# DataArcTech/RAG-ARC

Measured on AMD Instinct MI355X. Metric: queries/sec at fixed (N_corpus, d), exact top-k (ids bit-exact vs CPU oracle), higher is better.
Workload: dtype f16; 1 GPU; 100000000x768 fp16 corpus of N(0,1) directions resident in HBM, row-sharded over 1 GPU(s), batch 256 queries, cosine top-100, exact (canonical fp32 rescore); n_corpus=100000000, d=768, batch=256, k=100, rows_per_gpu=100000000, exchange=none (one shard), repaired_queries_last_step=0

## Files before the change

### include/rarc.h

```cpp
#ifndef RARC_H
#define RARC_H

#include <stddef.h>
#include <stdint.h>

#ifdef __cplusplus
extern "C" {
#endif

#define RARC_VERSION 600

#define RARC_OK 0
#define RARC_E_INVALID -1
#define RARC_E_HIP -2
#define RARC_E_WORKSPACE -3
#define RARC_E_UNSUPPORTED -4
#define RARC_E_IO -5

#define RARC_MAX_QUERIES 256
#define RARC_MAX_K 1024
#define RARC_DIM_ALIGN 128

#define RARC_Q_OK 0u
#define RARC_Q_UNCERTAIN 1u
#define RARC_Q_OVERFLOW 2u
#define RARC_Q_WHY_SEGMENT 0x100u
#define RARC_Q_WHY_G1 0x200u
#define RARC_Q_WHY_G2 0x400u
#define RARC_Q_WHY_BAND_TIES 0x800u
#define RARC_Q_WHY_BAND_GUARD 0x1000u

int rarc_version(void);
const char* rarc_last_error(void);

int rarc_padded_dim(int d);

int rarc_l2norm_rows_f32(const float* d_in, int64_t ld_in, float* d_out, int64_t ld_out,
                         int64_t n_rows, int d, void* stream);

int rarc_cosine_matrix_f32(const float* d_x, int64_t ld_x, int nx, const float* d_y, int64_t ld_y, int ny, int d,
                           double* d_out, void* stream);
int rarc_adjacent_cosine_distance_f32(const float* d_x, int64_t ld_x, int n_rows, int d, double* d_out, void* stream);

int rarc_ingest_f16(const float* d_in, int64_t ld_in, uint16_t* d_corpus_f16, int d_pad,
                    float* d_row_norm2, int64_t n_rows, int d, int normalize, void* stream);

size_t rarc_quant_meta_floats(int64_t n_rows);
int rarc_quant_meta_f16(const uint16_t* d_corpus_f16, int64_t n_rows, int d_pad, int64_t first_row,
                        float* d_qmeta, void* stream);

int rarc_debug_q8_scores(const uint16_t* d_corpus_f16, int64_t n_rows, int d_pad, const float* d_qmeta,
                         const void* d_qblock, int nq, float* d_out, void* stream);
int rarc_debug_q8_scores_f8(const uint8_t* d_corpus_f8, int64_t n_rows, int d_pad, const float* d_qmeta,
                            const void* d_qblock, int nq, float* d_out, void* stream);

size_t rarc_query_block_bytes(int d_pad);
int rarc_prep_queries(const float* d_in, int64_t ld_in, int nq, int d, int d_pad, int normalize,
                      float corpus_max_norm, const float* d_qmeta, void* d_qblock, void* stream);

int rarc_qblock_set_floor(void* d_qblock, int d_pad, const int64_t* d_prev_ids, const float* d_prev_scores, int k,
                          int nq, void* stream);

#define RARC_WS_ANYFLAG_OFFSET 5124
size_t rarc_search_workspace_bytes(int cand_cap);

int rarc_search_f16(const uint16_t* d_corpus_f16, int64_t n_rows, int d_pad, const float* d_qmeta,
                    const void* d_qblock, int nq, int k, int kprime, int64_t id_base, float bin_lo,
                    float bin_hi, int64_t* d_out_ids, float* d_out_scores, uint32_t* d_status,
                    void* d_workspace, size_t workspace_bytes, int cand_cap, void* stream);

int rarc_repair_f16(const uint16_t* d_corpus_f16, int64_t n_rows, int d_pad, const void* d_qblock,
                    int q, int k, int64_t id_base, int64_t* d_out_ids, float* d_out_scores,
                    uint32_t* d_found, void* d_workspace, size_t workspace_bytes, void* stream);

int rarc_verify_batch(const void* d_rows, const float* d_row_scale, int row_format, int64_t n_rows, int d_pad,
                      const void* d_qblock, int q_first, int nq, int k, int64_t id_base, const int64_t* d_ids,
                      const float* d_scores, uint32_t* d_counts, void* stream);

int rarc_quant_shadow_f16(const uint16_t* d_corpus_f16, int64_t n_rows, int d_pad, int64_t first_row,
                          float* d_qmeta, int8_t* d_shadow8, void* stream);
int rarc_search_f16_shadow(const uint16_t* d_corpus_f16, const int8_t* d_shadow8, int64_t n_rows, int d_pad,
                           const float* d_qmeta, const void* d_qblock, int nq, int k, int kprime,
                           int64_t id_base, float bin_lo, float bin_hi, int64_t* d_out_ids,
                           float* d_out_scores, uint32_t* d_status, void* d_workspace, size_t workspace_bytes,
                           int cand_cap, void* stream);

int rarc_padded_dim_f8(int d);
int rarc_ingest_f8(const float* d_in, int64_t ld_in, uint8_t* d_corpus_f8, int d_pad, float* d_row_scale,
                   float* d_row_norm2, int64_t n_rows, int d, int normalize, void* stream);
size_t rarc_quant_meta_floats_f8(int64_t n_rows);
int rarc_quant_meta_f8(const uint8_t* d_corpus_f8, const float* d_row_scale, int64_t n_rows, int d_pad,
                       int64_t first_row, float* d_qmeta, void* stream);
int rarc_search_f8(const uint8_t* d_corpus_f8, const float* d_row_scale, int64_t n_rows, int d_pad,
                   const float* d_qmeta, const void* d_qblock, int nq, int k, int kprime, int64_t id_base,
                   float bin_lo, float bin_hi, int64_t* d_out_ids, float* d_out_scores, uint32_t* d_status,
                   void* d_workspace, size_t workspace_bytes, int cand_cap, void* stream);
int rarc_repair_f8(const uint8_t* d_corpus_f8, const float* d_row_scale, int64_t n_rows, int d_pad,
                   const void* d_qblock, int q, int k, int64_t id_base, int64_t* d_out_ids, float* d_out_scores,
                   uint32_t* d_found, void* d_workspace, size_t workspace_bytes, void* stream);

int rarc_ingest_f32(const float* d_in, int64_t ld_in, float* d_corpus_f32, uint16_t* d_image_f16, int d_pad,
                    float* d_row_norm2, int64_t n_rows, int d, int normalize, void* stream);
int rarc_search_f32(const float* d_corpus_f32, const uint16_t* d_image_f16, int64_t n_rows, int d_pad,
                    const float* d_qmeta, const void* d_qblock, int nq, int k, int kprime, int64_t id_base,
                    float bin_lo, float bin_hi, int64_t* d_out_ids, float* d_out_scores, uint32_t* d_status,
                    void* d_workspace, size_t workspace_bytes, int cand_cap, void* stream);
typedef struct RarcSearchBatch {
  const void* d_rows; const void* d_aux; int row_format; int64_t n_rows; int d_pad; const float* d_qmeta;
  const float* d_queries; int64_t ld_queries; int nq; int d; int normalize; float corpus_max_norm; void* d_qblock;
  int k, kprime; int64_t id_base; float bin_lo, bin_hi;
  int64_t* d_out_ids; float* d_out_scores; uint32_t* d_status; uint32_t* flag_host;
  void* d_workspace; size_t workspace_bytes; int cand_cap;
  void* gate_event;
} RarcSearchBatch;
int rarc_search_batch(const RarcSearchBatch* batch, void* stream);

int rarc_stream_read(const void* d_src, size_t n_bytes, void* d_sink, void* stream);

size_t rarc_bm25_workspace_bytes(int nq, int64_t n_query_tokens, int64_t n_docs, int k);
int rarc_bm25_topk(const int64_t* d_post_off, const int32_t* d_post_doc, const double* d_post_w, int64_t n_terms,
                   int64_t n_docs, const int32_t* d_q_off, const int32_t* d_q_term, const double* d_q_idf, int nq,
                   int64_t n_query_tokens, int k, void* d_workspace, size_t workspace_bytes, int64_t* d_out_ids,
                   double* d_out_scores, void* stream);
int rarc_bm25_scores(const int64_t* d_post_off, const int32_t* d_post_doc, const double* d_post_w, int64_t n_terms,
                     int64_t n_docs, const int32_t* d_q_off, const int32_t* d_q_term, const double* d_q_idf, int nq,
                     int64_t n_query_tokens, void* d_workspace, size_t workspace_bytes, double* d_out_scores,
                     void* stream);

int rarc_repair_f32(const float* d_corpus_f32, int64_t n_rows, int d_pad, const void* d_qblock, int q, int k,
                    int64_t id_base, int64_t* d_out_ids, float* d_out_scores, uint32_t* d_found, void* d_workspace,
                    size_t workspace_bytes, void* stream);

int rarc_topk_merge(const int64_t* d_ids, const float* d_scores, int n_lists, int nq, int k,
                    int64_t* d_out_ids, float* d_out_scores, void* stream);
int rarc_pack_results(const int64_t* d_ids, const float* d_scores, int nq, int k, int32_t* d_packed, void* stream);
int rarc_topk_merge_packed(const int32_t* d_packed, int n_lists, int nq, int k, int64_t* d_out_ids,
                           float* d_out_scores, void* stream);

int rarc_rrf_fuse(const int64_t* d_keys, const int32_t* d_len, int nq, int n_lists, int max_len,
                  double rrf_k, int top_k, int64_t* d_out_keys, double* d_out_scores,
                  int32_t* d_out_n, void* stream);

int rarc_rerank_order(const uint16_t* d_z_no, const uint16_t* d_z_yes, int nq, int n,
                      uint16_t* d_out_scores_f16, int32_t* d_out_perm, void* stream);

size_t rarc_mmr_workspace_doubles(int n, int d);
int rarc_mmr_select(const float* d_cand, int64_t ld, const double* d_query, int n, int d, int normalize, int k,
                    double lambda, double* d_work, int32_t* d_out, void* stream);

size_t rarc_mmr_rows_workspace_bytes(int nq, int n, int d);
int rarc_mmr_select_rows(const void* d_rows, int fmt, const float* d_rowscale, int64_t n_rows, int d_pad, int d,
                         const double* d_queries, int64_t ldq, int nq, const int64_t* d_cand_ids, int n, int64_t id_base,
                         int normalize, int k, double lambda, int64_t* d_out_ids, void* d_ws, size_t ws_bytes, void* stream);

int rarc_synth_rows_f16(uint16_t* d_out_f16, int d_pad, int d, int64_t first_row, int64_t n_rows,
                        uint64_t seed, void* stream);
int rarc_synth_rows_f32(float* d_out_f32, int64_t ld_out, int d, int64_t first_row,
                        int64_t n_rows, uint64_t seed, void* stream);

int rarc_enc_embed_ln(const int32_t* d_ids, const uint16_t* d_word, const uint16_t* d_pos,
                      const uint16_t* d_type0, const uint16_t* d_gamma, const uint16_t* d_beta, float eps,
                      int n_tokens, int seq_len, int hidden, int vocab, uint16_t* d_out, void* stream);
int rarc_enc_gemm(const uint16_t* d_a, const uint16_t* d_w, const uint16_t* d_bias, uint16_t* d_c, int m,
                  int n, int k, int act, void* stream);
int rarc_enc_gemm_zero_bias(const uint16_t* d_a, const uint16_t* d_w, const uint16_t* d_zero_bias, uint16_t* d_c, int m,
                            int n, int k, int act, void* stream);
int rarc_enc_attention(const uint16_t* d_qkv, const int32_t* d_lens, int n_seq, int seq_len, int hidden,
                       int n_heads, uint16_t* d_ctx, void* stream);
int rarc_enc_add_ln(const uint16_t* d_x, const uint16_t* d_resid, const uint16_t* d_gamma,
                    const uint16_t* d_beta, float eps, int n_rows, int hidden, uint16_t* d_out, void* stream);
int rarc_enc_pool(const uint16_t* d_hidden, int n_seq, int seq_len, int hidden, int normalize,
                  float* d_out, void* stream);
int rarc_enc_pool_mean(const uint16_t* d_hidden, const int32_t* d_lens, int n_seq, int seq_len, int hidden,
                       int normalize, float* d_out, void* stream);

typedef struct RarcEncLayer {
  const uint16_t *qkv_w, *qkv_b;
  const uint16_t *o_w, *o_b, *ln1_g, *ln1_b;
  const uint16_t *f1_w, *f1_b, *f2_w, *f2_b, *ln2_g, *ln2_b;
} RarcEncLayer;
typedef struct RarcEncModel {
  int hidden, heads, inter, n_layers;
  float ln_eps;
  const uint16_t *word, *pos, *type0, *emb_g, *emb_b;
  const RarcEncLayer* layers;
  int vocab;
  int max_pos;
  const float* rel_bias;
  int rel_span;
} RarcEncModel;
size_t rarc_enc_workspace_bytes(int hidden, int inter, int n_tokens);
int rarc_enc_forward(const RarcEncModel* model, const int32_t* d_ids, const int32_t* d_lens, int n_seq,
                     int seq_len, int normalize, void* d_ws, size_t ws_bytes, float* d_out, void* stream);

typedef struct RarcEnc32Layer {
  const uint16_t* qkv_w3; const float *qkv_rw, *qkv_b;
  const uint16_t* o_w3;   const float *o_rw, *o_b, *ln1_g, *ln1_b;
  const uint16_t* f1_w3;  const float *f1_rw, *f1_b;
  const uint16_t* f2_w3;  const float *f2_rw, *f2_b, *ln2_g, *ln2_b;
  const float* f1_colmax;
  const uint16_t *qkv_wq, *o_wq, *f1_wq, *f2_wq;
} RarcEnc32Layer;
typedef struct RarcEnc32Model {
  int hidden, heads, inter, n_layers;
  float ln_eps;
  const float *word, *pos, *type0, *emb_g, *emb_b;
  const RarcEnc32Layer* layers;
  int vocab, max_pos;
  const float* rel_bias;
  int rel_span;
} RarcEnc32Model;
int rarc_enc32_split_weight(const float* d_w, int n, int k, uint16_t* d_w3, float* d_rw, void* stream);
int rarc_enc32_pack_query_weight(const uint16_t* d_w3, int n, int k, uint16_t* d_wq, void* stream);
int rarc_enc32_split_rows(const float* d_x, int m, int k, uint16_t* d_a3, float* d_ra, void* stream);
int rarc_enc32_gemm(const uint16_t* d_a3, const float* d_ra, const uint16_t* d_w3, const float* d_rw,
                    const float* d_bias, float* d_c, int m, int n, int k, void* stream);
size_t rarc_enc32_workspace_bytes(int hidden, int inter, int n_tokens);
int rarc_enc32_forward(const RarcEnc32Model* model, const int32_t* d_ids, const int32_t* d_lens, int n_seq,
                       int seq_len, int normalize, void* d_ws, size_t ws_bytes, float* d_out, void* stream);

typedef struct RarcLmLayer {
  const uint16_t *in_norm, *qkv_w, *q_norm, *k_norm, *o_w, *post_norm, *gate_up_w, *down_w;
  const uint16_t *qkv_w_folded, *gate_up_w_folded;
} RarcLmLayer;
typedef struct RarcLmModel {
  int hidden, n_layers, n_q_heads, n_kv_heads, head_dim, inter, vocab;
  float rms_eps, rope_theta;
  const uint16_t *embed, *lm_head, *final_norm, *zero_bias;
  const RarcLmLayer* layers;
} RarcLmModel;
size_t rarc_lm_workspace_bytes(const RarcLmModel* model, int n_tokens);
int rarc_lm_yes_no_logits(const RarcLmModel* model, const int32_t* d_ids, const int32_t* d_start, int n_seq,
                          int seq_len, int no_id, int yes_id, void* d_ws, size_t ws_bytes, uint16_t* d_out_f16,
                          void* stream);

size_t rarc_lm_prefix_cache_bytes(const RarcLmModel* model, int n_prefix_tokens);
int rarc_lm_prefix_kv(const RarcLmModel* model, const int32_t* d_ids, const int32_t* d_start, int n_prefix, int prefix_len,
                      void* d_ws, size_t ws_bytes, void* d_cache, size_t cache_bytes, void* stream);
int rarc_lm_yes_no_logits_prefixed(const RarcLmModel* model, const int32_t* d_ids, const int32_t* d_start, int n_seq,
                                   int seq_len, const int32_t* d_prefix_of, const void* d_cache, int n_prefix,
                                   int prefix_len, const int32_t* d_prefix_start, int no_id, int yes_id, void* d_ws,
                                   size_t ws_bytes, uint16_t* d_out_f16, void* stream);

int rarc_lm_embed_last(const RarcLmModel* model, const int32_t* d_ids, const int32_t* d_start, int n_seq, int seq_len,
                       int out_dim, int normalize, void* d_ws, size_t ws_bytes, float* d_out, int64_t ld_out, void* stream);
int rarc_lm_embed_last_prefixed(const RarcLmModel* model, const int32_t* d_ids, const int32_t* d_start, int n_seq,
                                int seq_len, const int32_t* d_prefix_of, const void* d_cache, int n_prefix,
                                int prefix_len, const int32_t* d_prefix_start, int out_dim, int normalize, void* d_ws,
                                size_t ws_bytes, float* d_out, int64_t ld_out, void* stream);

int rarc_lm_rope_table(int n_rows, int head_dim, float theta, uint16_t* d_table, void* stream);
int rarc_lm_rmsnorm(uint16_t* d_x, const uint16_t* d_delta, const uint16_t* d_w, float eps, int n_rows, int hidden, uint16_t* d_y,
                    void* stream);
int rarc_lm_rowscale_parts(const float* d_ssq, int n_parts, float eps, int n_rows, int hidden, float* d_r, void* stream);
int rarc_lm_swiglu(const uint16_t* d_gate_up, int n_rows, int inter, uint16_t* d_out, void* stream);
int rarc_lm_attention(const uint16_t* d_qkv, const int32_t* d_start, int n_seq, int seq_len, int n_q, int n_kv, int head_dim,
                      const uint16_t* d_q_norm, const uint16_t* d_k_norm, float eps, const uint16_t* d_rope, int rope_rows,
                      const uint16_t* d_prefix_kv, const int32_t* d_prefix_of, const int32_t* d_prefix_start, int n_prefix,
                      int prefix_len, int kernel, uint16_t* d_ctx, void* stream);
int rarc_lm_last_logits(const uint16_t* d_x, const uint16_t* d_final_norm, const uint16_t* d_lm_head, float eps, int n_seq,
                        int row_stride, int row_off, int hidden, int vocab, int no_id, int yes_id, uint16_t* d_out, void* stream);
int rarc_lm_last_embed(const uint16_t* d_x, const uint16_t* d_final_norm, float eps, int n_seq, int row_stride, int row_off,
                       int hidden, int out_dim, int normalize, float* d_out, int64_t ld_out, void* stream);
int rarc_lm_gather_last(const uint16_t* d_src, int seq_len, int width, int n_seq, int n_rows, uint16_t* d_dst, void* stream);

typedef struct RarcWordPiece RarcWordPiece;
int rarc_wordpiece_create(const char* vocab_blob, size_t blob_bytes, int do_lower_case, const char* unk_token,
                          const char* cls_token, const char* sep_token, const char* pad_token, const char* never_split_blob,
                          size_t never_split_bytes, int max_input_chars_per_word, RarcWordPiece** out);
void rarc_wordpiece_destroy(RarcWordPiece* wp);
int rarc_wordpiece_encode(const RarcWordPiece* wp, const char* text_blob, const int64_t* text_offsets, int n_texts,
                          int max_length, int32_t* h_ids, int64_t ld_ids, int32_t* h_lens, int n_threads);

#define RARC_IO_DIRECT 1
#define RARC_IO_FSYNC 2
#define RARC_IO_TRUNCATE 4
typedef struct RarcIoStats {
  int64_t bytes;
  double seconds;
  double file_seconds;
  double copy_wait_seconds;
  int64_t direct_bytes;
  int64_t n_chunks, slot_bytes;
  int n_threads, direct;
} RarcIoStats;
int rarc_file_to_device(const char* path, int n_seg, const int64_t* h_file_off, const int64_t* h_bytes,
                        const int64_t* h_dev_off, void* d_base, int64_t d_capacity_bytes, void* h_staging,
                        size_t staging_bytes, int n_threads, int flags, void* stream, RarcIoStats* stats);
int rarc_device_to_file(const char* path, int n_seg, const int64_t* h_file_off, const int64_t* h_bytes,
                        const int64_t* h_dev_off, const void* d_base, int64_t d_capacity_bytes, void* h_staging,
                        size_t staging_bytes, int n_threads, int flags, void* stream, RarcIoStats* stats);

size_t rarc_wide_workspace_bytes(int d_pad, int cand_cap);
int rarc_search_wide(const void* d_rows, const uint16_t* d_image16, int fmt, int64_t n_rows, int d_pad, float max_norm,
                     float rho, const void* d_qblock, int nq, int k, int64_t id_base, int64_t* d_out_ids,
                     float* d_out_scores, uint32_t* d_status, void* d_ws, size_t ws_bytes, int cand_cap, void* stream);

int rarc_row_sqnorms(const void* d_rows, int fmt, int64_t n_rows, int d_pad, int64_t first_row, float* d_xn, void* stream);
int rarc_search_wide_l2(const void* d_rows, const uint16_t* d_image16, int fmt, int64_t n_rows, int d_pad, float max_norm,
                        float rho, const float* d_xn, const void* d_qblock, int nq, int k, int64_t id_base, int64_t* d_out_ids,
                        float* d_out_scores, uint32_t* d_status, void* d_ws, size_t ws_bytes, int cand_cap, void* stream);
int rarc_debug_wide_bounds(const void* d_ws, size_t ws_bytes, int d_pad, int cand_cap, float* d_out, void* stream);
int rarc_debug_query_scale8(float mx, float* sq, float* qi);
int rarc_debug_q8_tail_plan(uint32_t t_begin, uint32_t n_tiles, uint32_t grid, int d_pad, int fmt, int pct, int min_mib,
                            uint32_t* t_dyn, uint32_t* r0, uint32_t* unit);
int rarc_debug_q8_tail_chunks(uint32_t k_first, uint32_t n, uint32_t stride, uint32_t unit, uint32_t t_dyn, uint32_t r0,
                              uint32_t n_tiles, uint32_t* t0, uint32_t* t_end);
int64_t rarc_debug_q8_tail_counter_offset(int launch);

size_t rarc_search_rows_workspace_bytes(int nq, int k);
int rarc_search_rows(const void* d_rows, int fmt, int64_t n_rows, int d_pad, const void* d_qblock, int nq, const int64_t* d_list,
                     int64_t m, int k, int64_t id_base, const float* d_xn, int l2, int64_t* d_out_ids, float* d_out_scores,
                     uint32_t* d_status, void* d_ws, size_t ws_bytes, void* stream);
int rarc_strike_rows(const int64_t* d_ids, const float* d_scores, int nq, int kprime, const uint32_t* d_bits, int64_t n_rows,
                     int64_t id_base, int k, int l2, int64_t* d_out_ids, float* d_out_scores, uint32_t* d_count, void* stream);

size_t rarc_search_rows_grouped_workspace_bytes(int nq, int k);
int rarc_search_rows_grouped(const void* d_rows, int fmt, int64_t n_rows, int d_pad, const void* d_qblock, int nq,
                             const int64_t* d_lists, const int64_t* d_tiles, int n_tiles, int64_t m_max, int k, int64_t id_base,
                             const float* d_xn, int l2, int64_t* d_out_ids, float* d_out_scores, uint32_t* d_status, void* d_ws,
                             size_t ws_bytes, void* stream);
int rarc_strike_rows_grouped(const int64_t* d_ids, const float* d_scores, int nq, int kprime, const uint32_t* d_bits,
                             const int64_t* d_bits_off, int64_t n_rows, int64_t id_base, int k, int l2, int64_t* d_out_ids,
                             float* d_out_scores, uint32_t* d_count, void* stream);

size_t rarc_similar_pairs_workspace_bytes(int64_t n_rows, int d, int cand_cap);
int rarc_similar_pairs(const float* d_rows, int64_t ld, int64_t n_rows, int d, double threshold, void* d_ws, size_t ws_bytes,
                       int cand_cap, int64_t* d_out_pairs, double* d_out_scores, int64_t out_cap,
                       unsigned long long* d_out_count, uint32_t* d_flags, void* stream);

size_t rarc_knn_graph_workspace_bytes(int64_t n_rows, int d, int top_k, int cand_cap);
int rarc_knn_graph(const float* d_rows, int64_t ld, int64_t n_rows, int d, int top_k, double cutoff, void* d_ws, size_t ws_bytes,
                   int cand_cap, int64_t* d_out_ids, double* d_out_scores, int32_t* d_out_count, uint32_t* d_flags, void* stream);

size_t rarc_graph_csr_workspace_bytes(int64_t n, int64_t m);
int rarc_graph_csr(const int64_t* d_pairs, const uint32_t* d_weights, const uint32_t* d_loops, int64_t n, int64_t m, void* d_graph,
                   size_t graph_bytes, void* stream);
size_t rarc_louvain_workspace_bytes(int64_t n, int64_t m);
int rarc_louvain_init(const void* d_graph, size_t graph_bytes, int64_t n, int64_t m, void* d_state, size_t state_bytes, int64_t* d_out3,
                      void* stream);
int rarc_louvain_sweep(const void* d_graph, size_t graph_bytes, int64_t n, int64_t m, void* d_state, size_t state_bytes, int cur, int sweep,
                       int64_t* d_out3, void* stream);
int rarc_louvain_aggregate(const void* d_graph, size_t graph_bytes, int64_t n, int64_t m, void* d_state, size_t state_bytes, int cur,
                           int64_t* d_labels, int64_t n0, int64_t* d_out_pairs, uint32_t* d_out_weights, uint32_t* d_out_loops,
                           int64_t* d_out_counts, void* stream);
size_t rarc_louvain_labels_workspace_bytes(int64_t n0);
int rarc_louvain_labels(int64_t* d_labels, int64_t n0, void* d_ws, size_t ws_bytes, void* stream);
int rarc_louvain_limits(int* out4);

size_t rarc_ppr_workspace_bytes(int64_t n, int64_t m, int nq);
int rarc_ppr_seed(const void* d_graph, size_t graph_bytes, int64_t n, int64_t m, const int64_t* d_seeds, const uint32_t* d_seed_weights,
                  int nq, int n_slots, void* d_ws, size_t ws_bytes, void* stream);
int rarc_ppr_step(const void* d_graph, size_t graph_bytes, int64_t n, int64_t m, int nq, int damping_q16, int64_t tolerance, int cur,
                  void* d_ws, size_t ws_bytes, uint32_t* d_done_out, void* stream);
int rarc_ppr_scores(int64_t n, int64_t m, int nq, const void* d_ws, size_t ws_bytes, double* d_out_scores, void* stream);
int rarc_ppr_topk(int64_t n, int64_t m, int nq, int top_k, int cur, void* d_ws, size_t ws_bytes, int64_t* d_out_ids,
                  double* d_out_scores, int32_t* d_out_count, void* stream);
int rarc_ppr_limits(int* out6);

size_t rarc_ppr_chunks_workspace_bytes(int64_t n_chunks, int nq);
int rarc_ppr_chunks(int64_t n, int64_t m, int nq, int cur, const void* d_ws, size_t ws_bytes, const int64_t* d_row_ptr,
                    const int32_t* d_ent, const uint32_t* d_w, int64_t n_chunks, int64_t nnz, const int32_t* d_split, int64_t n_split,
                    void* d_cws, size_t cws_bytes, void* stream);
int rarc_ppr_chunks_scores(int64_t n_chunks, int nq, const void* d_cws, size_t cws_bytes, double* d_out_scores, void* stream);
int rarc_ppr_chunks_topk(int64_t n_chunks, int nq, int top_k, void* d_cws, size_t cws_bytes, int64_t* d_out_ids, double* d_out_scores,
                         int32_t* d_out_count, void* stream);
int rarc_ppr_chunks_limits(int* out4);

size_t rarc_khop_workspace_bytes(int64_t n, int64_t m, int nq, int hops);
int rarc_khop_seed(int64_t n, int64_t m, const int64_t* d_seeds, int nq, int n_slots, int hops, void* d_ws, size_t ws_bytes, void* stream);
int rarc_khop_step(const void* d_graph, size_t graph_bytes, int64_t n, int64_t m, int nq, int hops, int hop, void* d_ws, size_t ws_bytes,
                   uint32_t* d_grew_out, void* stream);
int rarc_khop_counts(int64_t n, int64_t m, int nq, int hops, void* d_ws, size_t ws_bytes, int32_t* d_out_counts, void* stream);
int rarc_khop_levels(int64_t n, int64_t m, int nq, int hops, const void* d_ws, size_t ws_bytes, uint8_t* d_out_levels, void* stream);
int rarc_khop_list(int64_t n, int64_t m, int nq, int hops, int max_vertices, void* d_ws, size_t ws_bytes, int64_t* d_out_ids,
                   int32_t* d_out_hops, int32_t* d_out_count, void* stream);
int rarc_khop_chunks(int64_t n, int64_t m, int nq, int hops, const uint32_t* decay, const void* d_ws, size_t ws_bytes,
                     const int64_t* d_row_ptr, const int32_t* d_ent, const uint32_t* d_w, int64_t n_chunks, int64_t nnz,
                     const int32_t* d_split, int64_t n_split, void* d_cws, size_t cws_bytes, void* stream);
int rarc_khop_limits(int* out5);

size_t rarc_khop_edges_workspace_bytes(int64_t r, int nq, int hops);
int rarc_khop_edges(int64_t n, int64_t m, int nq, int hops, const void* d_ws, size_t ws_bytes, const int64_t* d_rel, int64_t r, int max_edges,
                    void* d_ews, size_t ews_bytes, int64_t* d_out_ids, int32_t* d_out_levels, int32_t* d_out_count,
                    int32_t* d_out_level_counts, void* stream);
int rarc_khop_edges_limits(int* out2);

int rarc_khop_paths(int64_t n, int64_t m, int ns, int np, int max_length, const void* d_ws, size_t ws_bytes, const int32_t* d_pairs,
                    void* d_pws, size_t pws_bytes, int32_t* d_out_dist, void* stream);
int rarc_khop_path_edges(int64_t n, int64_t m, int nq, int hops, const void* d_ws, size_t ws_bytes, const int64_t* d_rel, int64_t r,
                         int max_edges, void* d_ews, size_t ews_bytes, int64_t* d_out_ids, int32_t* d_out_levels, int32_t* d_out_count,
                         int32_t* d_out_level_counts, void* stream);
int rarc_khop_paths_limits(int* out3);

size_t rarc_graph_types_workspace_bytes(int64_t n, int64_t m);
int rarc_graph_types(const void* d_graph, size_t graph_bytes, int64_t n, int64_t m, const int64_t* d_pairs, const uint32_t* d_masks,
                     void* d_out, size_t out_bytes, void* stream);
int rarc_khop_step_typed(const void* d_graph, size_t graph_bytes, const void* d_types, size_t types_bytes, const uint32_t* d_filters,
                         int64_t n, int64_t m, int nq, int hops, int hop, void* d_ws, size_t ws_bytes, uint32_t* d_grew_out, void* stream);
int rarc_khop_edges_typed(int64_t n, int64_t m, int nq, int hops, const void* d_ws, size_t ws_bytes, const int64_t* d_rel, int64_t r,
                          const int32_t* d_rel_types, int rel_masks, const uint32_t* d_filters, int max_edges, void* d_ews, size_t ews_bytes,
                          int64_t* d_out_ids, int32_t* d_out_levels, int32_t* d_out_count, int32_t* d_out_level_counts, void* stream);
int rarc_khop_path_edges_typed(int64_t n, int64_t m, int nq, int hops, const void* d_ws, size_t ws_bytes, const int64_t* d_rel, int64_t r,
                               const int32_t* d_rel_types, int rel_masks, const uint32_t* d_filters, int max_edges, void* d_ews,
                               size_t ews_bytes, int64_t* d_out_ids, int32_t* d_out_levels, int32_t* d_out_count,
                               int32_t* d_out_level_counts, void* stream);

size_t rarc_graph_types_weighted_workspace_bytes(int64_t n, int64_t m);
int rarc_graph_types_weighted(const void* d_graph, size_t graph_bytes, int64_t n, int64_t m, const int64_t* d_pairs, const uint32_t* d_masks,
                              const uint32_t* d_weights, void* d_out, size_t out_bytes, void* stream);
int rarc_ppr_seed_typed(const void* d_graph, size_t graph_bytes, const void* d_types, size_t types_bytes, const uint32_t* d_filters, int64_t n,
                        int64_t m, const int64_t* d_seeds, const uint32_t* d_seed_weights, int nq, int n_slots, void* d_ws, size_t ws_bytes,
                        void* stream);
int rarc_ppr_step_typed(const void* d_graph, size_t graph_bytes, const void* d_types, size_t types_bytes, const uint32_t* d_filters, int64_t n,
                        int64_t m, int nq, int damping_q16, int64_t tolerance, int cur, void* d_ws, size_t ws_bytes, uint32_t* d_done_out,
                        void* stream);

size_t rarc_sort_reduce_workspace_bytes(int64_t count);
int rarc_sort_reduce(const uint64_t* d_keys, const uint32_t* d_values, int64_t count, int key_bits, void* d_ws, size_t ws_bytes,
                     uint64_t* d_out_keys, uint64_t* d_out_sums, int64_t* d_out2, void* stream);
int rarc_sort_reduce_limits(int* out4);
size_t rarc_merge_plan_workspace_bytes(int64_t n);
int rarc_merge_plan(const int64_t* d_labels, const uint32_t* d_richness, int64_t n, void* d_ws, size_t ws_bytes, int64_t* d_primary,
                    int64_t* d_new_id, int64_t* d_kept, int64_t* d_removed, int64_t* d_out_count, void* stream);
size_t rarc_merge_pairs_workspace_bytes(int64_t m);
int rarc_merge_pairs(const int64_t* d_pairs, const uint32_t* d_weights, int64_t m, const int64_t* d_new_id, int64_t n, void* d_ws,
                     size_t ws_bytes, int64_t* d_out_pairs, uint32_t* d_out_weights, int64_t* d_out5, void* stream);
size_t rarc_merge_mentions_workspace_bytes(int64_t n_chunks, int64_t nnz);
int rarc_merge_mentions(const int64_t* d_row_ptr, const int32_t* d_ent, const uint32_t* d_w, int64_t n_chunks, int64_t nnz,
                        const int64_t* d_new_id, int64_t n, void* d_ws, size_t ws_bytes, int64_t* d_out_row_ptr, int32_t* d_out_ent,
                        uint32_t* d_out_w, int32_t* d_out_split, int64_t* d_out6, void* stream);
size_t rarc_merge_relations_workspace_bytes(int64_t r);
int rarc_merge_relations(const int64_t* d_rel, int64_t r, const int64_t* d_new_id, int64_t n, void* d_ws, size_t ws_bytes,
                         int64_t* d_out_rel, int64_t* d_out_rows, int64_t* d_out3, void* stream);

size_t rarc_ingest_pairs_workspace_bytes(int64_t m0, int64_t r);
int rarc_ingest_pairs(const int64_t* d_rows, const uint32_t* d_row_weights, const int32_t* d_row_types, int64_t r,
                      const int64_t* d_base_pairs, const uint32_t* d_base_weights, const uint32_t* d_base_masks, int64_t m0, int64_t n,
                      void* d_ws, size_t ws_bytes, int64_t* d_out_pairs, uint32_t* d_out_weights, uint32_t* d_out_masks, int64_t* d_out8,
                      void* stream);
size_t rarc_ingest_mentions_workspace_bytes(int64_t n_chunks, int64_t nnz0, int64_t r);
int rarc_ingest_mentions(const int64_t* d_rows, const uint32_t* d_row_weights, int64_t r, const int64_t* d_base_row_ptr,
                         const int32_t* d_base_ent, const uint32_t* d_base_w, int64_t base_chunks, int64_t nnz0, int64_t n_chunks,
                         int64_t n_entities, void* d_ws, size_t ws_bytes, int64_t* d_out_row_ptr, int32_t* d_out_ent, uint32_t* d_out_w,
                         int32_t* d_out_split, int64_t* d_out8, void* stream);
int rarc_ingest_limits(int* out4);

size_t rarc_components_workspace_bytes(int64_t n, int64_t m);
int rarc_components_init(int64_t n, int64_t m, void* d_ws, size_t ws_bytes, void* stream);
int rarc_components_round(const void* d_graph, size_t graph_bytes, int64_t n, int64_t m, void* d_ws, size_t ws_bytes, int32_t* d_changed,
                          void* stream);
int rarc_components_finish(int64_t n, int64_t m, void* d_ws, size_t ws_bytes, int64_t* d_labels, int32_t* d_dense, int64_t* d_sizes,
                           int64_t* d_out3, void* stream);
int rarc_components_limits(int* out4);

size_t rarc_cooccur_workspace_bytes(int64_t n_chunks, int64_t nnz);
int rarc_cooccur_count(const int64_t* d_row_ptr, const int32_t* d_ent, const uint32_t* d_w, int64_t n_chunks, int64_t nnz, int64_t n,
                       int max_mentions, void* d_ws, size_t ws_bytes, int64_t* d_out4, void* stream);
int rarc_cooccur_emit(const int64_t* d_row_ptr, const int32_t* d_ent, const uint32_t* d_w, int64_t n_chunks, int64_t nnz, int64_t n,
                      int mode, const void* d_ws, size_t ws_bytes, uint64_t* d_keys, uint32_t* d_values, int64_t total, void* stream);
size_t rarc_cooccur_edges_workspace_bytes(int64_t distinct);
int rarc_cooccur_edges(const uint64_t* d_keys, const uint64_t* d_sums, int64_t distinct, int64_t n, int64_t min_weight, void* d_ws,
                       size_t ws_bytes, int64_t* d_out_pairs, uint32_t* d_out_weights, int64_t* d_out3, void* stream);
int rarc_cooccur_limits(int* out4);

int rarc_compact_rows(void* d_rows, int64_t row_bytes, int64_t n_rows, const int64_t* d_adj, int64_t n_holes,
                      int64_t first_hole, void* d_tmp, size_t tmp_bytes, void* stream);

#define RARC_VMEM_DEFAULT_SLAB (16u << 20)
typedef struct RarcVmem RarcVmem;
int rarc_vmem_create(int device, size_t reserve_bytes, size_t min_reserve_bytes, size_t slab_bytes, RarcVmem** out);
int rarc_vmem_grow(RarcVmem* arena, size_t min_bytes);
void* rarc_vmem_base(const RarcVmem* arena);
size_t rarc_vmem_mapped(const RarcVmem* arena);
size_t rarc_vmem_reserved(const RarcVmem* arena);
size_t rarc_vmem_slab(const RarcVmem* arena);
size_t rarc_vmem_granularity(const RarcVmem* arena);
int rarc_vmem_destroy(RarcVmem* arena);

int rarc_profile_begin(int max_launches);
int rarc_profile_end(double* total_scan_ms, int* n_launches);

#ifdef __cplusplus
}
#endif
#endif
```

### rag-arc_amd/csrc/finalize.hip

```cpp
#include "rarc_common.h"
#include <type_traits>

constexpr int FIN_THREADS = 256;

__device__ __forceinline__ float canon_dot_f16(const float* __restrict__ q,
                                               const half_t* __restrict__ row, int d) {
  float a[8] = {0.f, 0.f, 0.f, 0.f, 0.f, 0.f, 0.f, 0.f};
#pragma unroll 16
  for (int m = 0; m < d; m += 8) {
    const half8 x = *(const half8*)(row + m);
    const float4 q0 = *(const float4*)(q + m);
    const float4 q1 = *(const float4*)(q + m + 4);
    a[0] = __builtin_fmaf(q0.x, (float)x[0], a[0]);
    a[1] = __builtin_fmaf(q0.y, (float)x[1], a[1]);
    a[2] = __builtin_fmaf(q0.z, (float)x[2], a[2]);
    a[3] = __builtin_fmaf(q0.w, (float)x[3], a[3]);
    a[4] = __builtin_fmaf(q1.x, (float)x[4], a[4]);
    a[5] = __builtin_fmaf(q1.y, (float)x[5], a[5]);
    a[6] = __builtin_fmaf(q1.z, (float)x[6], a[6]);
    a[7] = __builtin_fmaf(q1.w, (float)x[7], a[7]);
  }
  return rarc_canon_tree(a);
}

__device__ __forceinline__ float canon_dot_f32(const float* __restrict__ q, const float* __restrict__ row, int d) {
  float a[8] = {0.f, 0.f, 0.f, 0.f, 0.f, 0.f, 0.f, 0.f};
#pragma unroll 8
  for (int m = 0; m < d; m += 8) {
    const float4 x0 = *(const float4*)(row + m), x1 = *(const float4*)(row + m + 4);
    const float4 q0 = *(const float4*)(q + m), q1 = *(const float4*)(q + m + 4);
    a[0] = __builtin_fmaf(q0.x, x0.x, a[0]);
    a[1] = __builtin_fmaf(q0.y, x0.y, a[1]);
    a[2] = __builtin_fmaf(q0.z, x0.z, a[2]);
    a[3] = __builtin_fmaf(q0.w, x0.w, a[3]);
    a[4] = __builtin_fmaf(q1.x, x1.x, a[4]);
    a[5] = __builtin_fmaf(q1.y, x1.y, a[5]);
    a[6] = __builtin_fmaf(q1.z, x1.z, a[6]);
    a[7] = __builtin_fmaf(q1.w, x1.w, a[7]);
  }
  return rarc_canon_tree(a);
}

__device__ __forceinline__ void bitonic_desc(uint64_t* a, int n) {
  for (int k = 2; k <= n; k <<= 1) {
    for (int j = k >> 1; j > 0; j >>= 1) {
      for (int i = threadIdx.x; i < n; i += blockDim.x) {
        const int ixj = i ^ j;
        if (ixj > i) {
          const uint64_t x = a[i], y = a[ixj];
          const bool up = ((i & k) == 0);
          if (up ? (x < y) : (x > y)) {
            a[i] = y;
            a[ixj] = x;
          }
        }
      }
      __syncthreads();
    }
  }
}

struct FinParams {
  const half_t* corpus;
  const float* q32;
  const float* eps;
  const uint32_t* cnt2;
  const uint64_t* cand;
  const uint32_t* hist;
  const float* binlo;
  const float* bininv;
  uint32_t* flags;
  uint32_t seg;
  uint32_t n_wg;
  int d;
  int k, kprime;
  int64_t id_base;
  int64_t* out_ids;
  float* out_scores;
  uint32_t* status;
  uint32_t* flag_host;
};

constexpr int FIN_SURV = 4096;

__global__ __launch_bounds__(FIN_THREADS) void rarc_finalize_kernel(const FinParams p) {
  __shared__ uint64_t keys[FIN_SURV];
  __shared__ uint64_t sel[RARC_MAX_K];
  __shared__ uint64_t fin[RARC_MAX_K];
  __shared__ uint32_t s_hist[RARC_NB];
  __shared__ __attribute__((aligned(16))) float s_q[768];
  __shared__ float s_thr;
  __shared__ uint32_t s_ns, s_total, s_over, s_maxn;
  const int q = blockIdx.x, tid = threadIdx.x;

  for (int i = tid; i < RARC_NB; i += blockDim.x) s_hist[i] = p.hist[(size_t)q * RARC_NB + i];
  for (int i = tid; i < p.d; i += blockDim.x) s_q[i] = p.q32[(size_t)q * p.d + i];
  if (tid == 0) { s_ns = 0; s_total = 0; s_over = 0; s_maxn = 0; }
  __syncthreads();
  if (tid < 64) {
    uint32_t above;
    const int b = rarc_wave_find_from_top(s_hist, RARC_NB, (uint32_t)p.kprime, &above);
    if (tid == 0) s_thr = rarc_bin_threshold(b, p.binlo[q], p.bininv[q]);
  }
  __syncthreads();
  const float thr = s_thr;

  {
    uint32_t n = 0;
    const uint64_t* src = p.cand;
    if ((uint32_t)tid < p.n_wg) {
      const uint32_t c = p.cnt2[(size_t)tid * RARC_MAX_QUERIES + q];
      n = c < p.seg ? c : p.seg;
      if (c > p.seg) atomicOr(&s_over, 1u);
      atomicAdd(&s_total, c);
      src = p.cand + ((size_t)q * RARC_MAX_WG + tid) * p.seg;
    }
    uint64_t first[16];
#pragma unroll
    for (int i = 0; i < 8; ++i) {
      const ulonglong2 v = ((const ulonglong2*)src)[i];
      first[2 * i] = v.x;
      first[2 * i + 1] = v.y;
    }
#pragma unroll
    for (uint32_t i = 0; i < 16; ++i) {
      if (i < n && rarc_candscore(first[i]) >= thr) {
        const uint32_t pos = atomicAdd(&s_ns, 1u);
        if (pos < FIN_SURV) keys[pos] = first[i];
      }
    }
    for (uint32_t i = 16; i < n; ++i) {
      const uint64_t key = src[i];
      if (rarc_candscore(key) >= thr) {
        const uint32_t pos = atomicAdd(&s_ns, 1u);
        if (pos < FIN_SURV) keys[pos] = key;
      }
    }
  }
  __syncthreads();
  const uint32_t ns_all = s_ns, total = s_total;
  const int ns = ns_all < FIN_SURV ? (int)ns_all : FIN_SURV;

  const int kp = ns < p.kprime ? ns : p.kprime;
  for (int i = tid; i < ns; i += blockDim.x) {
    const uint64_t mine = keys[i];
    int rank = 0;
    for (int j = 0; j < ns; ++j) rank += (keys[j] > mine);
    if (rank < kp) sel[rank] = mine;
  }
  __syncthreads();

  const float* qv = s_q;
  for (int i = tid; i < kp; i += blockDim.x) {
    const uint32_t row = rarc_candrow(sel[i]);
    fin[i] = rarc_candkey(canon_dot_f16(qv, p.corpus + (size_t)row * p.d, p.d), row);
  }
  __syncthreads();
  for (int i = tid; i < p.k; i += blockDim.x) {
    if (i >= kp) {
      p.out_ids[(size_t)q * p.k + i] = -1;
      p.out_scores[(size_t)q * p.k + i] = -INFINITY;
    }
  }
  __shared__ float s_sk;
  for (int i = tid; i < kp; i += blockDim.x) {
    const uint64_t mine = fin[i];
    int rank = 0;
    for (int j = 0; j < kp; ++j) rank += (fin[j] > mine);
    if (rank < p.k) {
      p.out_ids[(size_t)q * p.k + rank] = p.id_base + (int64_t)rarc_candrow(mine);
      p.out_scores[(size_t)q * p.k + rank] = rarc_candscore(mine);
    }
    if (rank == (p.k < kp ? p.k : kp) - 1) s_sk = rarc_candscore(mine);
  }
  __syncthreads();

  if (tid == 0) {
    uint32_t st = RARC_Q_OK;
    if (s_over || ns_all > (uint32_t)FIN_SURV) st |= RARC_Q_OVERFLOW;
    if (total >= (uint32_t)p.kprime && kp >= 1) {
      const float tmin = rarc_candscore(sel[kp - 1]);
      if (!(tmin + p.eps[q] < s_sk)) st |= RARC_Q_UNCERTAIN;
    }
    p.status[q] = st;
    if (st) {
      atomicOr(&p.flags[1], st);
      atomicOr(&p.status[RARC_MAX_QUERIES], st);
      if (p.flag_host) __hip_atomic_store(p.flag_host, 1u, __ATOMIC_RELAXED, __HIP_MEMORY_SCOPE_SYSTEM);
    }
  }
}

int rarc_finalize_launch(const uint16_t* corpus, int d_pad, const float* q32, const float* eps, int nq,
                         int k, int kprime, int64_t id_base, const RarcWs& ws, int cap, int n_wg,
                         int64_t* out_ids, float* out_scores, uint32_t* status, hipStream_t s) {
  FinParams p;
  p.corpus = (const half_t*)corpus;
  p.q32 = q32;
  p.eps = eps;
  p.cnt2 = ws.cnt2;
  p.cand = ws.cand;
  p.hist = ws.hist;
  p.binlo = ws.binlo;
  p.bininv = ws.bininv;
  p.flags = ws.flags;
  p.seg = (uint32_t)(cap / RARC_MAX_WG);
  p.n_wg = (uint32_t)n_wg;
  p.d = d_pad;
  p.k = k;
  p.kprime = kprime;
  p.id_base = id_base;
  p.out_ids = out_ids;
  p.out_scores = out_scores;
  p.status = status;
  p.flag_host = rarc_launch_extras().flag_host;
  hipLaunchKernelGGL(rarc_finalize_kernel, dim3(nq), dim3(FIN_THREADS), 0, s, p);
  RARC_HIP_CHECK(hipGetLastError());
  return RARC_OK;
}

constexpr int FIN8_THREADS = 512;
constexpr int FIN8_RS = 6144;
constexpr int FIN8_MAXD = 1024;
#ifndef FIN8_COLLECT_U
#define FIN8_COLLECT_U 8
#endif

struct Fin8Params {
  const void* corpus;
  const float* rowscale;
  int fmt;
  const float* q32;
  const float* eps8;
  const uint32_t* cnt2;
  const uint64_t* cand;
  const uint32_t* hist;
  const float* binlo;
  const float* bininv;
  uint32_t* flags;
  uint32_t seg;
  uint32_t n_wg;
  int d;
  int k;
  int64_t id_base;
  int64_t* out_ids;
  float* out_scores;
  uint32_t* status;
  const float* tmeta;
  int mstride;
  const float* hq;
  unsigned long long* dbg;
  uint32_t* tighten_thr;
  int tighten_mode;
  const float* eps16;
  uint32_t* flag_host;
};

__global__ __launch_bounds__(FIN8_THREADS) void rarc_finalize_q8_kernel(const Fin8Params p) {
  extern __shared__ __attribute__((aligned(16))) char fsm[];
  __shared__ uint64_t ex[FIN8_RS];
  __shared__ __attribute__((aligned(16))) float s_q[FIN8_MAXD];
  __shared__ uint32_t s_hist[RARC_NB];
  __shared__ uint32_t s_cnt[RARC_MAX_WG];
  __shared__ float s_t1, s_L;
  __shared__ uint32_t s_ne, s_over, s_cmp;
  __shared__ int s_selb;
  __shared__ uint32_t s_selabove;
  const int q = blockIdx.x, tid = threadIdx.x;
  const float eps = p.eps8[q];
#define FIN8_STAMP(i) if (p.dbg && q == 0 && tid == 0) p.dbg[i] = __builtin_amdgcn_s_memrealtime();
  FIN8_STAMP(0)

  for (int i = tid; i < RARC_NB; i += blockDim.x) s_hist[i] = p.hist[(size_t)q * RARC_NB + i];
  for (int i = tid; i < p.d; i += blockDim.x) s_q[i] = p.q32[(size_t)q * p.d + i];
  if (tid == 0) { s_ne = 0; s_over = 0; s_L = -INFINITY; }
  __syncthreads();
  for (int i = tid; i < RARC_MAX_WG; i += blockDim.x) {
    const uint32_t c = (uint32_t)i < p.n_wg ? p.cnt2[(size_t)i * RARC_MAX_QUERIES + q] : 0u;
    s_cnt[i] = c;
    if (c > p.seg) atomicOr(&s_over, 1u);
  }
  if (tid < 64) {
    uint32_t above;
    const int b = rarc_wave_find_from_top(s_hist, RARC_NB, (uint32_t)p.k, &above);
    if (tid == 0) s_t1 = rarc_bin_threshold(b, p.binlo[q], p.bininv[q]);
  }
  __syncthreads();
  float t1 = s_t1;

  auto collect = [&](auto want) {
    constexpr int U = FIN8_COLLECT_U;
    const int lane = tid & 63, wv = tid >> 6, nwv = blockDim.x >> 6;
    for (uint32_t wg0 = wv * U; wg0 < p.n_wg; wg0 += nwv * U) {
      uint32_t n[U];
      uint32_t nmax = 0;
#pragma unroll
      for (int u = 0; u < U; ++u) {
        const uint32_t wg = wg0 + u;
        const uint32_t c = wg < p.n_wg ? s_cnt[wg] : 0u;
        n[u] = c < p.seg ? c : p.seg;
        nmax = n[u] > nmax ? n[u] : nmax;
      }
      for (uint32_t base = 0; base < nmax; base += 64) {
        uint64_t key[U];
#pragma unroll
        for (int u = 0; u < U; ++u) {
          const uint32_t i = base + lane;
          key[u] = i < n[u] ? p.cand[((size_t)q * RARC_MAX_WG + wg0 + u) * p.seg + i] : 0ull;
        }
#pragma unroll
        for (int u = 0; u < U; ++u) {
          if (base + lane < n[u] && want(rarc_candscore(key[u]), rarc_candrow(key[u]))) {
            const uint32_t e = atomicAdd(&s_ne, 1u);
            if (e < FIN8_RS) ex[e] = key[u];
          }
        }
      }
    }
  };
  auto rescore_n = [&](auto nt_c, int from, int to) __attribute__((always_inline)) {
    constexpr int NT = decltype(nt_c)::value;
    const int lane = tid & 63, wv = tid >> 6, j = lane & 7, rr = lane >> 3;
    constexpr int rbytes = NT * 128;
    constexpr int rstride = rbytes + 16;
    char* stage = fsm + (size_t)wv * 8 * rstride;
    typedef uint32_t u32x4 __attribute__((ext_vector_type(4)));
    u32x4 pre[NT];
    auto issue = [&](int i) {
      if (i < to) {
        const u32x4* src = (const u32x4*)((const char*)p.corpus + (size_t)rarc_candrow(ex[i]) * rbytes) + j;
#pragma unroll
        for (int t = 0; t < NT; ++t) pre[t] = src[t * 8];
      }
    };
    int i = from + wv * 8 + rr;
    issue(i);
    for (; i - rr - wv * 8 < to; i += (blockDim.x >> 6) * 8) {
#pragma unroll
      for (int t = 0; t < NT; ++t) *(u32x4*)(stage + rr * rstride + (t * 8 + j) * 16) = pre[t];
      const int cur = i;
      issue(i + (blockDim.x >> 6) * 8);
      __builtin_amdgcn_wave_barrier();
      float acc = 0.f;
      if (cur < to) {
        if (p.fmt == 2) {
          const char* rowp = stage + rr * rstride + 4 * j;
          for (int m0 = 0; m0 < NT * 4; m0 += 16) {
            float xs[16], qs[16];
#pragma unroll
            for (int u = 0; u < 16; ++u) {
              xs[u] = *(const float*)(rowp + 32 * (m0 + u));
              qs[u] = s_q[8 * (m0 + u) + j];
            }
#pragma unroll
            for (int u = 0; u < 16; ++u) acc = __builtin_fmaf(qs[u], xs[u], acc);
          }
        } else if (p.fmt) {
          const char* rowp = stage + rr * rstride + j;
          for (int m0 = 0; m0 < NT * 16; m0 += 16) {
            float xs[16], qs[16];
#pragma unroll
            for (int u = 0; u < 16; ++u) {
              xs[u] = __builtin_amdgcn_cvt_f32_fp8((uint32_t) * (const uint8_t*)(rowp + 8 * (m0 + u)), 0);
              qs[u] = s_q[8 * (m0 + u) + j];
            }
#pragma unroll
            for (int u = 0; u < 16; ++u) acc = __builtin_fmaf(qs[u], xs[u], acc);
          }
        } else {
          const char* rowp = stage + rr * rstride + 2 * j;
          for (int m0 = 0; m0 < NT * 8; m0 += 16) {
            float xs[16], qs[16];
#pragma unroll
            for (int u = 0; u < 16; ++u) {
              xs[u] = (float)*(const half_t*)(rowp + 16 * (m0 + u));
              qs[u] = s_q[8 * (m0 + u) + j];
            }
#pragma unroll
            for (int u = 0; u < 16; ++u) acc = __builtin_fmaf(qs[u], xs[u], acc);
          }
        }
      }
      float a8[8];
#pragma unroll
      for (int u = 0; u < 8; ++u) a8[u] = __shfl(acc, (lane & ~7) + u, 64);
      if (cur < to && j == 0) {
        const uint32_t row = rarc_candrow(ex[cur]);
        float sc = rarc_canon_tree(a8);
        if (p.fmt == 1) sc = p.rowscale[row] * sc;
        ex[cur] = rarc_candkey(sc, row);
      }
      __builtin_amdgcn_wave_barrier();
    }
  };
  auto rescore = [&](int from, int to) __attribute__((always_inline)) {
    switch ((p.fmt == 2 ? p.d * 4 : (p.fmt ? p.d : p.d * 2)) / 128) {
#define FIN8_NT(N) case N: rescore_n(std::integral_constant<int, N>{}, from, to); break;
      FIN8_NT(2) FIN8_NT(4) FIN8_NT(6) FIN8_NT(8) FIN8_NT(10) FIN8_NT(12) FIN8_NT(14) FIN8_NT(16)
      FIN8_NT(20) FIN8_NT(24) FIN8_NT(28) FIN8_NT(32)
#undef FIN8_NT
      default: break;
    }
  };

  constexpr int FIN8_SMALL = 1024;
  auto select_kth = [&](int n, int kth) __attribute__((always_inline)) -> uint64_t {
    if (n <= FIN8_SMALL) {
      __syncthreads();
      for (int i = tid; i < n; i += blockDim.x) {
        const uint64_t mine = ex[i];
        int rank = 0;
        for (int j = 0; j < n; ++j) rank += (ex[j] > mine);
        if (rank == kth - 1) { s_selb = (int)(mine >> 32); s_selabove = (uint32_t)mine; }
      }
      __syncthreads();
      const uint64_t r = ((uint64_t)(uint32_t)s_selb << 32) | s_selabove;
      __syncthreads();
      return r;
    }
    uint64_t prefix = 0, mask = 0;
    uint32_t need = (uint32_t)kth;
    for (int shift = 56; shift >= 0; shift -= 8) {
      __syncthreads();
      for (int i = tid; i < RARC_NB; i += blockDim.x) s_hist[i] = 0;
      __syncthreads();
      for (int i = tid; i < n; i += blockDim.x) {
        const uint64_t key = ex[i];
        if ((key & mask) == prefix) atomicAdd(&s_hist[(uint32_t)(key >> shift) & 255u], 1u);
      }
      __syncthreads();
      if (tid < 64) {
        uint32_t above = 0;
        const int b = rarc_wave_find_from_top(s_hist, RARC_NB, need, &above);
        if (tid == 0) { s_selb = b; s_selabove = above; }
      }
      __syncthreads();
      prefix |= (uint64_t)(uint32_t)s_selb << shift;
      mask |= 0xFFull << shift;
      need -= s_selabove;
    }
    __syncthreads();
    return prefix;
  };
  static_assert(RARC_NB == 256, "the radix select counts one byte per pass in s_hist");

  FIN8_STAMP(1)
  collect([&](float a, uint32_t) { return a >= t1; });
  __syncthreads();
  if (s_ne > (uint32_t)FIN8_RS && t1 > -INFINITY) {
    __syncthreads();
    if (tid == 0) s_cmp = 0;
    __syncthreads();
    collect([&](float a, uint32_t) { atomicMax(&s_cmp, rarc_ordkey(a)); return false; });
    __syncthreads();
    float a_lo = t1, a_hi = rarc_unordkey(s_cmp + 1u);
    __syncthreads();
    for (int probe = 0; probe < 40 && a_hi > a_lo; ++probe) {
      const float mid = a_lo + 0.5f * (a_hi - a_lo);
      if (!(mid > a_lo && mid < a_hi)) break;
      __syncthreads();
      if (tid == 0) s_ne = 0;
      __syncthreads();
      collect([&](float a, uint32_t) { return a >= mid; });
      __syncthreads();
      const uint32_t c = s_ne;
      if (c > (uint32_t)FIN8_RS) a_lo = mid;
      else if (c < (uint32_t)p.k) a_hi = mid;
      else { t1 = mid; break; }
    }
    if (s_ne > (uint32_t)FIN8_RS || s_ne < (uint32_t)p.k) {
      __syncthreads();
      if (tid == 0) s_ne = 0;
      __syncthreads();
      collect([&](float a, uint32_t) { return a >= t1; });
      __syncthreads();
    }
  }
  FIN8_STAMP(2)
  const uint32_t ne1_all = s_ne;
  const int ne1 = ne1_all < FIN8_RS ? (int)ne1_all : FIN8_RS;
  rescore(0, ne1);
  __syncthreads();
  FIN8_STAMP(3)
  if (ne1 >= p.k) {
    const uint64_t kth = select_kth(ne1, p.k);
    if (tid == 0) s_L = rarc_candscore(kth);
  }
  __syncthreads();
  const float L = s_L;
  FIN8_STAMP(4)
  if (p.tighten_thr) {
    if (tid == 0 && L > -INFINITY) {
      const float t = L - (1.0002f * eps + 1e-7f);
      if (p.tighten_mode == 2 || t > __uint_as_float(p.tighten_thr[q])) p.tighten_thr[q] = __float_as_uint(t);
    } else if (tid == 0 && p.tighten_mode == 2) {
      const float e16 = p.eps16 ? p.eps16[q] : 0.f;
      const float cur = __uint_as_float(p.tighten_thr[q]);
      if (cur > -INFINITY && cur < INFINITY) p.tighten_thr[q] = __float_as_uint(cur - (1.0002f * fmaxf(eps - e16, 0.f) + 1e-7f));
    }
    return;
  }

  const float hqv = p.hq ? p.hq[q] : 0.f;
  const float e16 = p.eps16 ? p.eps16[q] : 0.f;
  const float r_max = p.tmeta ? p.tmeta[0 - RARC_QMETA_HDR] : 0.f;
  auto reaches = [&](float a, uint32_t row, float ref) {
    if (!(a + eps * 1.0001f >= ref)) return false;
    if (!p.tmeta) return true;
    const uint32_t w = __float_as_uint(p.tmeta[(size_t)(row >> 5) * p.mstride]);
    const float rt = (float)__builtin_bit_cast(half_t, (uint16_t)(w >> 16));
    return a + fmaxf(eps - hqv * fmaxf(r_max - rt, 0.f), e16) * 1.0001f >= ref;
  };
  if (ne1_all <= (uint32_t)FIN8_RS && t1 > -INFINITY) collect([&](float a, uint32_t row) { return a < t1 && reaches(a, row, L); });
  __syncthreads();
  FIN8_STAMP(5)
  uint32_t ne_all = s_ne;
  int ne = ne_all < FIN8_RS ? (int)ne_all : FIN8_RS;
  bool band_fail = false;
  uint32_t why = 0;
  if (ne1_all > (uint32_t)FIN8_RS) why |= RARC_Q_WHY_G1;
  if (ne_all > (uint32_t)FIN8_RS && ne1_all <= (uint32_t)FIN8_RS && ne1 >= p.k && L > -INFINITY) {
    uint64_t* tmp = (uint64_t*)fsm;
    auto keep_top_k = [&](int n) {
      const uint64_t kth = select_kth(n, p.k);
      if (tid == 0) { s_cmp = 0; s_L = rarc_candscore(kth); }
      __syncthreads();
      for (int i = tid; i < n; i += blockDim.x) {
        const uint64_t mine = ex[i];
        if (mine >= kth) tmp[atomicAdd(&s_cmp, 1u)] = mine;
      }
      __syncthreads();
      for (int i = tid; i < p.k; i += blockDim.x) ex[i] = tmp[i];
      __syncthreads();
    };
    keep_top_k(ne1);
    float hi = t1, lo_try = -INFINITY;
    bool reached_floor = false;
    for (int guard = 0; guard < 512; ++guard) {
      const float floor_a = s_L - eps * 1.0001f;
      if (!(hi > floor_a)) { reached_floor = true; break; }
      const float lo = lo_try > floor_a ? lo_try : floor_a;
      __syncthreads();
      if (tid == 0) s_ne = (uint32_t)p.k;
      __syncthreads();
      const float lc = s_L;
      collect([&](float a, uint32_t row) { return a >= lo && a < hi && reaches(a, row, lc); });
      __syncthreads();
      const uint32_t cnt = s_ne;
      if (cnt > (uint32_t)FIN8_RS) {
        const float mid = lo + 0.5f * (hi - lo);
        if (!(mid > lo && mid < hi)) { band_fail = true; why |= RARC_Q_WHY_BAND_TIES; break; }
        lo_try = mid;
        continue;
      }
      rescore(p.k, (int)cnt);
      __syncthreads();
      keep_top_k((int)cnt);
      const float width = hi - lo;
      hi = lo;
      lo_try = (cnt > (uint32_t)(FIN8_RS / 2)) ? hi - width : hi - 2.0f * width;
    }
    if (!reached_floor && !band_fail) why |= RARC_Q_WHY_BAND_GUARD;
    if (!reached_floor) band_fail = true;
    ne = p.k;
    ne_all = band_fail ? (uint32_t)FIN8_RS + 1u : (uint32_t)p.k;
  } else {
    rescore(ne1, ne);
    __syncthreads();
  }
  FIN8_STAMP(6)

  const int kk = ne < p.k ? ne : p.k;
  for (int i = tid; i < p.k; i += blockDim.x) {
    if (i >= kk) {
      p.out_ids[(size_t)q * p.k + i] = -1;
      p.out_scores[(size_t)q * p.k + i] = -INFINITY;
    }
  }
  if (ne <= FIN8_SMALL) {
    for (int i = tid; i < ne; i += blockDim.x) {
      const uint64_t mine = ex[i];
      if (rarc_candscore(mine) < L) continue;
      int rank = 0;
      for (int j = 0; j < ne; ++j) rank += (ex[j] > mine);
      if (rank < p.k) {
        p.out_ids[(size_t)q * p.k + rank] = p.id_base + (int64_t)rarc_candrow(mine);
        p.out_scores[(size_t)q * p.k + rank] = rarc_candscore(mine);
      }
    }
  } else {
    uint64_t* top = (uint64_t*)fsm;
    const uint64_t kth = select_kth(ne, kk);
    if (tid == 0) s_cmp = 0;
    __syncthreads();
    for (int i = tid; i < ne; i += blockDim.x) {
      const uint64_t mine = ex[i];
      if (mine >= kth) top[atomicAdd(&s_cmp, 1u)] = mine;
    }
    __syncthreads();
    for (int i = tid; i < kk; i += blockDim.x) {
      const uint64_t mine = top[i];
      int rank = 0;
      for (int j = 0; j < kk; ++j) rank += (top[j] > mine);
      p.out_ids[(size_t)q * p.k + rank] = p.id_base + (int64_t)rarc_candrow(mine);
      p.out_scores[(size_t)q * p.k + rank] = rarc_candscore(mine);
    }
  }
  FIN8_STAMP(7)
  if (p.dbg && q == 0 && tid == 0) { p.dbg[8] = ne1_all; p.dbg[9] = ne_all; }
  if (p.dbg && tid == 0) { p.dbg[16 + 4 * q] = ne1_all; p.dbg[17 + 4 * q] = ne_all; p.dbg[18 + 4 * q] = __builtin_amdgcn_s_memrealtime(); p.dbg[19 + 4 * q] = ((unsigned long long)__float_as_uint(t1) << 32) | __float_as_uint(L); }
  if (tid == 0) {
    uint32_t st = RARC_Q_OK;
    if (s_over || ne_all > (uint32_t)FIN8_RS) st |= RARC_Q_OVERFLOW;
    if (st) st |= why | (s_over ? RARC_Q_WHY_SEGMENT : 0u) | ((ne_all > (uint32_t)FIN8_RS && !why) ? RARC_Q_WHY_G2 : 0u);
    p.status[q] = st;
    if (st) {
      atomicOr(&p.flags[1], st);
      atomicOr(&p.status[RARC_MAX_QUERIES], st);
      if (p.flag_host) __hip_atomic_store(p.flag_host, 1u, __ATOMIC_RELAXED, __HIP_MEMORY_SCOPE_SYSTEM);
    }
  }
}

unsigned long long* g_fin8_dbg = nullptr;
int rarc_finalize_q8_launch(const void* corpus, const float* rowscale, int fmt, int d_pad, const float* q32,
                            const float* eps8, int nq, int k, int64_t id_base, const RarcWs& ws, int cap, int n_wg,
                            int64_t* out_ids, float* out_scores, uint32_t* status, hipStream_t s, int tighten,
                            const float* qmeta, const float* hq, const float* eps16) {
  RARC_REQUIRE(d_pad <= FIN8_MAXD, RARC_E_UNSUPPORTED, "rarc_finalize_q8: d_pad %d > %d", d_pad, FIN8_MAXD);
  Fin8Params p;
  p.corpus = corpus;
  p.rowscale = rowscale;
  p.fmt = fmt;
  p.q32 = q32;
  p.eps8 = eps8;
  p.cnt2 = ws.cnt2;
  p.cand = ws.cand;
  p.hist = ws.hist;
  p.binlo = ws.binlo;
  p.bininv = ws.bininv;
  p.flags = ws.flags;
  p.seg = (uint32_t)(cap / RARC_MAX_WG);
  p.n_wg = (uint32_t)n_wg;
  p.d = d_pad;
  p.k = k;
  p.id_base = id_base;
  p.out_ids = out_ids;
  p.out_scores = out_scores;
  p.status = status;
  p.tmeta = qmeta ? qmeta + RARC_QMETA_HDR : nullptr;
  p.mstride = fmt == 1 ? RARC_QMETA_F8_STRIDE : RARC_QMETA_STRIDE;
  p.hq = hq;
  p.dbg = tighten ? nullptr : g_fin8_dbg;
  p.tighten_thr = tighten ? (uint32_t*)ws.thr : nullptr;
  p.tighten_mode = tighten;
  p.eps16 = eps16;
  p.flag_host = tighten ? nullptr : rarc_launch_extras().flag_host;
  const size_t rbytes = (size_t)d_pad * (fmt == 2 ? 4 : (fmt ? 1 : 2));
  const int threads = rbytes <= 1536 ? FIN8_THREADS : (rbytes <= 3072 ? FIN8_THREADS / 2 : FIN8_THREADS / 4);
  const size_t lds = (size_t)(threads / 64) * 8 * (rbytes + 16);
  static RarcPerDevice lds_attr_dev;
  size_t& lds_attr = lds_attr_dev.cur();
  if (lds > lds_attr) {
    RARC_HIP_CHECK(hipFuncSetAttribute((const void*)rarc_finalize_q8_kernel,
                                       hipFuncAttributeMaxDynamicSharedMemorySize, (int)lds));
    lds_attr = lds;
  }
  hipLaunchKernelGGL(rarc_finalize_q8_kernel, dim3(nq), dim3(threads), lds, s, p);
  RARC_HIP_CHECK(hipGetLastError());
  return RARC_OK;
}

__device__ __forceinline__ float canon_dot_f8(const float* __restrict__ q, const uint8_t* __restrict__ row, int d,
                                              float scale) {
  float a[8] = {0.f, 0.f, 0.f, 0.f, 0.f, 0.f, 0.f, 0.f};
#pragma unroll 8
  for (int m = 0; m < d; m += 16) {
    const uint4 v = *(const uint4*)(row + m);
    const uint32_t w[4] = {v.x, v.y, v.z, v.w};
#pragma unroll
    for (int i = 0; i < 4; ++i) {
      float f[4];
      rarc_f8x4_to_f32(w[i], f);
      const int e0 = 4 * i;
#pragma unroll
      for (int e = 0; e < 4; ++e) a[(e0 + e) & 7] = __builtin_fmaf(q[m + e0 + e], f[e], a[(e0 + e) & 7]);
    }
  }
  return scale * rarc_canon_tree(a);
}

struct RepairParams {
  const half_t* corpus;
  const uint8_t* corpus8;
  const float* corpus32;
  const float* rowscale;
  const float* qv;
  uint32_t n_rows;
  int d, k;
  int64_t id_base;
  int64_t* ids;
  float* scores;
  uint64_t* list;
  uint32_t* count;
  uint32_t cap;
};

__global__ __launch_bounds__(256) void rarc_repair_scan_kernel(const RepairParams p) {
  const int64_t kid = p.ids[p.k - 1];
  const float ks = p.scores[p.k - 1];
  const uint64_t kth = (kid < 0) ? 0ull : rarc_candkey(ks, (uint32_t)(kid - p.id_base));
  for (uint32_t r = blockIdx.x * blockDim.x + threadIdx.x; r < p.n_rows; r += gridDim.x * blockDim.x) {
    const float c = p.corpus32 ? canon_dot_f32(p.qv, p.corpus32 + (size_t)r * p.d, p.d)
                  : p.corpus8 ? canon_dot_f8(p.qv, p.corpus8 + (size_t)r * p.d, p.d, p.rowscale[r])
                              : canon_dot_f16(p.qv, p.corpus + (size_t)r * p.d, p.d);
    const uint64_t key = rarc_candkey(c, r);
    if (key > kth) {
      const uint32_t pos = atomicAdd(p.count, 1u);
      if (pos < p.cap) p.list[pos] = key;
    }
  }
}

__global__ __launch_bounds__(256) void rarc_repair_merge_kernel(const RepairParams p, uint32_t* found) {
  extern __shared__ __attribute__((aligned(16))) char smem[];
  uint64_t* keys = (uint64_t*)smem;
  const uint32_t total = *p.count;
  const uint32_t n = total < p.cap ? total : p.cap;
  int np2 = 2;
  while (np2 < (int)n + 1) np2 <<= 1;
  const int64_t kid = p.ids[p.k - 1];
  const uint64_t kth = (kid < 0) ? 0ull : rarc_candkey(p.scores[p.k - 1], (uint32_t)(kid - p.id_base));
  for (int i = threadIdx.x; i < np2; i += blockDim.x)
    keys[i] = (i < (int)n) ? p.list[i] : (i == (int)n ? kth : 0ull);
  __syncthreads();
  bitonic_desc(keys, np2);
  if (threadIdx.x == 0) {
    uint32_t old_better = 0;
    for (int i = 0; i < p.k - 1; ++i) old_better += (p.ids[i] >= 0);
    *found = (total > old_better) ? (total - old_better) : 0u;
    if (total > p.cap) *found |= 0x80000000u;
  }
  __syncthreads();
  for (int i = threadIdx.x; i < p.k; i += blockDim.x) {
    const uint64_t key = keys[i];
    if (key != 0ull) {
      p.ids[i] = p.id_base + (int64_t)rarc_candrow(key);
      p.scores[i] = rarc_candscore(key);
    } else {
      p.ids[i] = -1;
      p.scores[i] = -INFINITY;
    }
  }
}

constexpr int VERIFY_NQ = 8;
struct VerifyParams {
  const void* corpus;
  const float* rowscale;
  int fmt;
  const float* q32;
  int q_first, nq;
  uint32_t n_rows;
  int d, k;
  int64_t id_base;
  const int64_t* ids;
  const float* scores;
  uint32_t* counts;
};

__global__ __launch_bounds__(256) void rarc_verify_kernel(const VerifyParams p) {
  __shared__ __attribute__((aligned(16))) float s_q[VERIFY_NQ][1024];
  __shared__ uint64_t s_kth[VERIFY_NQ];
  __shared__ uint32_t s_cnt[3 * VERIFY_NQ];
  const int tid = threadIdx.x;
  for (int i = tid; i < VERIFY_NQ * p.d; i += blockDim.x) {
    const int qi = i / p.d, m = i % p.d;
    s_q[qi][m] = qi < p.nq ? p.q32[(size_t)(p.q_first + qi) * p.d + m] : 0.f;
  }
  if (tid < VERIFY_NQ) {
    uint64_t kth = ~0ull;
    if (tid < p.nq) {
      const int64_t kid = p.ids[(size_t)(p.q_first + tid) * p.k + p.k - 1];
      kth = kid < 0 ? 0ull : rarc_candkey(p.scores[(size_t)(p.q_first + tid) * p.k + p.k - 1], (uint32_t)(kid - p.id_base));
    }
    s_kth[tid] = kth;
    s_cnt[tid] = 0;
    s_cnt[VERIFY_NQ + tid] = 0;
    s_cnt[2 * VERIFY_NQ + tid] = 0;
  }
  __syncthreads();
  uint32_t mine[VERIFY_NQ];
#pragma unroll
  for (int qi = 0; qi < VERIFY_NQ; ++qi) mine[qi] = 0;
  uint8_t lookups[VERIFY_NQ];
#pragma unroll
  for (int qi = 0; qi < VERIFY_NQ; ++qi) lookups[qi] = 0;
  for (uint32_t r = blockIdx.x * blockDim.x + tid; r < p.n_rows; r += gridDim.x * blockDim.x) {
    float a[VERIFY_NQ][8];
#pragma unroll
    for (int qi = 0; qi < VERIFY_NQ; ++qi)
#pragma unroll
      for (int j = 0; j < 8; ++j) a[qi][j] = 0.f;
    float scale = 1.f;
    if (p.fmt == 0) {
      const half_t* row = (const half_t*)p.corpus + (size_t)r * p.d;
      for (int m = 0; m < p.d; m += 8) {
        const half8 x = *(const half8*)(row + m);
#pragma unroll
        for (int qi = 0; qi < VERIFY_NQ; ++qi) {
          const float4 q0 = *(const float4*)(&s_q[qi][m]), q1 = *(const float4*)(&s_q[qi][m + 4]);
          a[qi][0] = __builtin_fmaf(q0.x, (float)x[0], a[qi][0]);
          a[qi][1] = __builtin_fmaf(q0.y, (float)x[1], a[qi][1]);
          a[qi][2] = __builtin_fmaf(q0.z, (float)x[2], a[qi][2]);
          a[qi][3] = __builtin_fmaf(q0.w, (float)x[3], a[qi][3]);
          a[qi][4] = __builtin_fmaf(q1.x, (float)x[4], a[qi][4]);
          a[qi][5] = __builtin_fmaf(q1.y, (float)x[5], a[qi][5]);
          a[qi][6] = __builtin_fmaf(q1.z, (float)x[6], a[qi][6]);
          a[qi][7] = __builtin_fmaf(q1.w, (float)x[7], a[qi][7]);
        }
      }
    } else if (p.fmt == 2) {
      const float* row = (const float*)p.corpus + (size_t)r * p.d;
      for (int m = 0; m < p.d; m += 8) {
        const float4 x0 = *(const float4*)(row + m), x1 = *(const float4*)(row + m + 4);
#pragma unroll
        for (int qi = 0; qi < VERIFY_NQ; ++qi) {
          const float4 q0 = *(const float4*)(&s_q[qi][m]), q1 = *(const float4*)(&s_q[qi][m + 4]);
          a[qi][0] = __builtin_fmaf(q0.x, x0.x, a[qi][0]);
          a[qi][1] = __builtin_fmaf(q0.y, x0.y, a[qi][1]);
          a[qi][2] = __builtin_fmaf(q0.z, x0.z, a[qi][2]);
          a[qi][3] = __builtin_fmaf(q0.w, x0.w, a[qi][3]);
          a[qi][4] = __builtin_fmaf(q1.x, x1.x, a[qi][4]);
          a[qi][5] = __builtin_fmaf(q1.y, x1.y, a[qi][5]);
          a[qi][6] = __builtin_fmaf(q1.z, x1.z, a[qi][6]);
          a[qi][7] = __builtin_fmaf(q1.w, x1.w, a[qi][7]);
        }
      }
    } else {
      const uint8_t* row = (const uint8_t*)p.corpus + (size_t)r * p.d;
      scale = p.rowscale[r];
      for (int m = 0; m < p.d; m += 8) {
        const uint2 v = *(const uint2*)(row + m);
        float xa[4], xb[4];
        rarc_f8x4_to_f32(v.x, xa);
        rarc_f8x4_to_f32(v.y, xb);
        const float x[8] = {xa[0], xa[1], xa[2], xa[3], xb[0], xb[1], xb[2], xb[3]};
#pragma unroll
        for (int qi = 0; qi < VERIFY_NQ; ++qi) {
          const float4 q0 = *(const float4*)(&s_q[qi][m]), q1 = *(const float4*)(&s_q[qi][m + 4]);
          a[qi][0] = __builtin_fmaf(q0.x, x[0], a[qi][0]);
          a[qi][1] = __builtin_fmaf(q0.y, x[1], a[qi][1]);
          a[qi][2] = __builtin_fmaf(q0.z, x[2], a[qi][2]);
          a[qi][3] = __builtin_fmaf(q0.w, x[3], a[qi][3]);
          a[qi][4] = __builtin_fmaf(q1.x, x[4], a[qi][4]);
          a[qi][5] = __builtin_fmaf(q1.y, x[5], a[qi][5]);
          a[qi][6] = __builtin_fmaf(q1.z, x[6], a[qi][6]);
          a[qi][7] = __builtin_fmaf(q1.w, x[7], a[qi][7]);
        }
      }
    }
#pragma unroll
    for (int qi = 0; qi < VERIFY_NQ; ++qi) {
      float c = rarc_canon_tree(a[qi]);
      if (p.fmt == 1) c = scale * c;
      const uint64_t key = rarc_candkey(c, r);
      mine[qi] += key > s_kth[qi] ? 1u : 0u;
      if (qi < p.nq && key >= s_kth[qi] && s_kth[qi] != 0ull && lookups[qi] >= 64) atomicAdd(&s_cnt[2 * VERIFY_NQ + qi], 1u);
      if (qi < p.nq && key >= s_kth[qi] && s_kth[qi] != 0ull && lookups[qi] < 64) {
        ++lookups[qi];
        const int64_t* ai = p.ids + (size_t)(p.q_first + qi) * p.k;
        const float* as = p.scores + (size_t)(p.q_first + qi) * p.k;
        const int64_t want = (int64_t)r + p.id_base;
        for (int j = 0; j < p.k; ++j)
          if (ai[j] == want) {
            if (__builtin_bit_cast(uint32_t, as[j]) == __builtin_bit_cast(uint32_t, c)) atomicAdd(&s_cnt[VERIFY_NQ + qi], 1u);
            break;
          }
      }
    }
  }
#pragma unroll
  for (int qi = 0; qi < VERIFY_NQ; ++qi)
    if (mine[qi]) atomicAdd(&s_cnt[qi], mine[qi]);
  __syncthreads();
  if (tid < p.nq && s_cnt[tid]) atomicAdd(&p.counts[tid], s_cnt[tid]);
  if (tid < p.nq && s_cnt[VERIFY_NQ + tid]) atomicAdd(&p.counts[VERIFY_NQ + tid], s_cnt[VERIFY_NQ + tid]);
  if (tid < p.nq && s_cnt[2 * VERIFY_NQ + tid]) atomicAdd(&p.counts[2 * VERIFY_NQ + tid], s_cnt[2 * VERIFY_NQ + tid]);
}

int rarc_verify_launch(const void* corpus, const float* rowscale, int fmt, int64_t n_rows, int d_pad, const float* q32,
                       int q_first, int nq, int k, int64_t id_base, const int64_t* ids, const float* scores,
                       uint32_t* counts, hipStream_t s) {
  VerifyParams p{corpus, rowscale, fmt, q32, q_first, nq, (uint32_t)n_rows, d_pad, k, id_base, ids, scores, counts};
  RARC_HIP_CHECK(hipMemsetAsync(counts, 0, sizeof(uint32_t) * 3 * VERIFY_NQ, s));
  hipLaunchKernelGGL(rarc_verify_kernel, dim3(2048), dim3(256), 0, s, p);
  RARC_HIP_CHECK(hipGetLastError());
  return RARC_OK;
}

int rarc_repair_launch(const void* corpus, const float* rowscale, int fmt, int64_t n_rows, int d_pad,
                       const float* qv, int k, int64_t id_base, int64_t* ids, float* scores, uint32_t* found,
                       const RarcWs& ws, int cap, hipStream_t s) {
  RepairParams p;
  p.corpus = fmt ? nullptr : (const half_t*)corpus;
  p.corpus8 = fmt == 1 ? (const uint8_t*)corpus : nullptr;
  p.corpus32 = fmt == 2 ? (const float*)corpus : nullptr;
  p.rowscale = rowscale;
  p.qv = qv;
  p.n_rows = (uint32_t)n_rows;
  p.d = d_pad;
  p.k = k;
  p.id_base = id_base;
  p.ids = ids;
  p.scores = scores;
  p.list = ws.cand;
  p.count = ws.cnt;
  p.cap = (uint32_t)(cap < 8192 ? cap : 8192);
  RARC_HIP_CHECK(hipMemsetAsync(p.count, 0, 4, s));
  const int grid = 2048;
  hipLaunchKernelGGL(rarc_repair_scan_kernel, dim3(grid), dim3(256), 0, s, p);
  RARC_HIP_CHECK(hipGetLastError());
  int np2 = 2;
  while (np2 < (int)p.cap + 1) np2 <<= 1;
  const size_t lds = (size_t)np2 * 8;
  static RarcPerDevice lds_attr_dev;
  size_t& lds_attr = lds_attr_dev.cur();
  if (lds > lds_attr) {
    RARC_HIP_CHECK(hipFuncSetAttribute((const void*)rarc_repair_merge_kernel,
                                       hipFuncAttributeMaxDynamicSharedMemorySize, (int)lds));
    lds_attr = lds;
  }
  hipLaunchKernelGGL(rarc_repair_merge_kernel, dim3(1), dim3(256), lds, s, p, found);
  RARC_HIP_CHECK(hipGetLastError());
  return RARC_OK;
}

template <bool PACKED>
__global__ __launch_bounds__(256) void rarc_merge_kernel(const int64_t* ids, const float* scores, int G,
                                                         int nq, int k, int64_t* out_ids,
                                                         float* out_scores) {
  extern __shared__ __attribute__((aligned(16))) char smem[];
  uint32_t* sk = (uint32_t*)smem;
  const int q = blockIdx.x;
  const int n = G * k;
  int np2 = 2;
  while (np2 < n) np2 <<= 1;
  int64_t* sid = (int64_t*)(smem + (size_t)np2 * 4);
  for (int i = threadIdx.x; i < np2; i += blockDim.x) {
    uint32_t key = 0;
    int64_t id = INT64_MAX;
    if (i < n) {
      const int g = i / k, j = i % k;
      const size_t o = ((size_t)g * nq + q) * k + j;
      float sc;
      if (PACKED) {
        const uint32_t* pk = (const uint32_t*)ids + o * 3;
        id = (int64_t)((uint64_t)pk[0] | ((uint64_t)pk[1] << 32));
        sc = __uint_as_float(pk[2]);
      } else {
        id = ids[o];
        sc = scores[o];
      }
      if (id >= 0) key = rarc_ordkey(sc);
      else id = INT64_MAX;
    }
    sk[i] = key;
    sid[i] = id;
  }
  __syncthreads();
  for (int kk = 2; kk <= np2; kk <<= 1) {
    for (int j = kk >> 1; j > 0; j >>= 1) {
      for (int i = threadIdx.x; i < np2; i += blockDim.x) {
        const int ixj = i ^ j;
        if (ixj > i) {
          const uint32_t ka = sk[i], kb = sk[ixj];
          const int64_t ia = sid[i], ib = sid[ixj];
          const bool a_better = (ka > kb) || (ka == kb && ia < ib);
          const bool b_better = (kb > ka) || (ka == kb && ib < ia);
          const bool up = ((i & kk) == 0);
          if (up ? b_better : a_better) {
            sk[i] = kb; sk[ixj] = ka;
            sid[i] = ib; sid[ixj] = ia;
          }
        }
      }
      __syncthreads();
    }
  }
  for (int i = threadIdx.x; i < k; i += blockDim.x) {
    const bool valid = (i < n) && sid[i] != INT64_MAX;
    out_ids[(size_t)q * k + i] = valid ? sid[i] : -1;
    out_scores[(size_t)q * k + i] = valid ? rarc_unordkey(sk[i]) : -INFINITY;
  }
}

int rarc_merge_launch(const int64_t* ids, const float* scores, int G, int nq, int k, int64_t* out_ids,
                      float* out_scores, hipStream_t s, bool packed) {
  int np2 = 2;
  while (np2 < G * k) np2 <<= 1;
  const size_t lds = (size_t)np2 * 12;
  RARC_REQUIRE(lds <= 160 * 1024, RARC_E_UNSUPPORTED, "rarc_topk_merge: %d lists x k=%d too large", G, k);
  static RarcPerDevice lds_attr_dev;
  size_t& lds_attr = lds_attr_dev.cur();
  if (lds > lds_attr) {
    RARC_HIP_CHECK(hipFuncSetAttribute((const void*)rarc_merge_kernel<false>,
                                       hipFuncAttributeMaxDynamicSharedMemorySize, (int)lds));
    RARC_HIP_CHECK(hipFuncSetAttribute((const void*)rarc_merge_kernel<true>,
                                       hipFuncAttributeMaxDynamicSharedMemorySize, (int)lds));
    lds_attr = lds;
  }
  if (packed)
    hipLaunchKernelGGL(rarc_merge_kernel<true>, dim3(nq), dim3(256), lds, s, ids, scores, G, nq, k, out_ids, out_scores);
  else
    hipLaunchKernelGGL(rarc_merge_kernel<false>, dim3(nq), dim3(256), lds, s, ids, scores, G, nq, k, out_ids, out_scores);
  RARC_HIP_CHECK(hipGetLastError());
  return RARC_OK;
}

__global__ __launch_bounds__(256) void rarc_pack_kernel(const int64_t* ids, const float* scores, int n, uint32_t* out) {
  const int i = blockIdx.x * 256 + threadIdx.x;
  if (i >= n) return;
  const uint64_t id = (uint64_t)ids[i];
  out[3 * i] = (uint32_t)id;
  out[3 * i + 1] = (uint32_t)(id >> 32);
  out[3 * i + 2] = __float_as_uint(scores[i]);
}

int rarc_pack_launch(const int64_t* ids, const float* scores, int n, uint32_t* out, hipStream_t s) {
  hipLaunchKernelGGL(rarc_pack_kernel, dim3((n + 255) / 256), dim3(256), 0, s, ids, scores, n, out);
  RARC_HIP_CHECK(hipGetLastError());
  return RARC_OK;
}
```

### rag-arc_amd/csrc/rarc_api.hip

```cpp
#include <stdarg.h>
#include <stdio.h>
#include "rarc_common.h"

int rarc_scan_f16_launch(const uint16_t* corpus, int64_t n_rows, int d_pad, const uint16_t* q16, int nq,
                         int kprime, float bin_lo, float bin_hi, const RarcWs& ws, int cap, int* grid_out,
                         hipStream_t s, const float* floor, const float* floor_eps);
int rarc_finalize_launch(const uint16_t* corpus, int d_pad, const float* q32, const float* eps, int nq,
                         int k, int kprime, int64_t id_base, const RarcWs& ws, int cap, int n_wg,
                         int64_t* out_ids, float* out_scores, uint32_t* status, hipStream_t s);
int rarc_scan_q8_launch(const void* corpus, const float* rowscale, int fmt, int64_t n_rows, int d_pad,
                        const float* qmeta, const uint16_t* q16, const int8_t* q8, const float* qinv,
                        const float* eps16, const float* eps8, int nq, int kprime, float bin_lo, float bin_hi,
                        const RarcWs& ws, int cap, int* grid_out, hipStream_t s, const int8_t* shadow8,
                        int (*tighten)(void* ctx, int n_wg, int mode), void* tighten_ctx, const float* hq, const float* floor,
                        int* hybrid_out);
int rarc_finalize_q8_launch(const void* corpus, const float* rowscale, int fmt, int d_pad, const float* q32,
                            const float* eps8, int nq, int k, int64_t id_base, const RarcWs& ws, int cap, int n_wg,
                            int64_t* out_ids, float* out_scores, uint32_t* status, hipStream_t s, int tighten,
                            const float* qmeta, const float* hq, const float* eps16);

struct Q8Search {
  const void* rows;
  const float* rowscale;
  int fin_fmt;
  int d_pad, nq, k, cap;
  int64_t id_base;
  const float *q32, *eps8;
  const float *qmeta, *hq;
  const float* eps16;
  const RarcWs* ws;
  int64_t* out_ids;
  float* out_scores;
  uint32_t* status;
  hipStream_t s;
};
static int q8_tighten(void* ctx, int n_wg, int mode) {
  const Q8Search& a = *(const Q8Search*)ctx;
  return rarc_finalize_q8_launch(a.rows, a.rowscale, a.fin_fmt, a.d_pad, a.q32, a.eps8, a.nq, a.k, a.id_base, *a.ws, a.cap,
                                 n_wg, a.out_ids, a.out_scores, a.status, a.s, mode, a.qmeta, a.hq, a.eps16);
}
int rarc_repair_launch(const void* corpus, const float* rowscale, int fmt, int64_t n_rows, int d_pad,
                       const float* qv, int k, int64_t id_base, int64_t* ids, float* scores, uint32_t* found,
                       const RarcWs& ws, int cap, hipStream_t s);
int rarc_verify_launch(const void* corpus, const float* rowscale, int fmt, int64_t n_rows, int d_pad, const float* q32,
                       int q_first, int nq, int k, int64_t id_base, const int64_t* ids, const float* scores,
                       uint32_t* counts, hipStream_t s);
int rarc_merge_launch(const int64_t* ids, const float* scores, int G, int nq, int k, int64_t* out_ids,
                      float* out_scores, hipStream_t s, bool packed);
int rarc_pack_launch(const int64_t* ids, const float* scores, int n, uint32_t* out, hipStream_t s);

static thread_local char g_err[512] = "";

#include <atomic>
#include <mutex>
#include <vector>
static std::mutex g_prof_mu;
static std::vector<hipEvent_t> g_prof_ev;
static int g_prof_n = 0;
static std::atomic<bool> g_prof_on{false};
bool rarc_prof_next(hipEvent_t* start, hipEvent_t* stop) {
  if (!g_prof_on.load(std::memory_order_acquire)) return false;
  std::lock_guard<std::mutex> lk(g_prof_mu);
  if (!g_prof_on || (size_t)(2 * g_prof_n + 1) >= g_prof_ev.size()) return false;
  *start = g_prof_ev[2 * g_prof_n];
  *stop = g_prof_ev[2 * g_prof_n + 1];
  ++g_prof_n;
  return true;
}
extern "C" int rarc_profile_begin(int max_launches) {
  std::lock_guard<std::mutex> lk(g_prof_mu);
  RARC_REQUIRE(max_launches > 0 && max_launches <= 65536 && !g_prof_on, RARC_E_INVALID, "rarc_profile_begin: bad state");
  g_prof_ev.resize((size_t)2 * max_launches);
  for (auto& e : g_prof_ev) RARC_HIP_CHECK(hipEventCreate(&e));
  g_prof_n = 0;
  g_prof_on = true;
  return RARC_OK;
}
extern "C" int rarc_profile_end(double* total_scan_ms, int* n_launches) {
  std::lock_guard<std::mutex> lk(g_prof_mu);
  RARC_REQUIRE(g_prof_on && total_scan_ms && n_launches, RARC_E_INVALID, "rarc_profile_end: not profiling");
  double tot = 0;
  for (int i = 0; i < g_prof_n; ++i) {
    RARC_HIP_CHECK(hipEventSynchronize(g_prof_ev[2 * i + 1]));
    float ms = 0;
    RARC_HIP_CHECK(hipEventElapsedTime(&ms, g_prof_ev[2 * i], g_prof_ev[2 * i + 1]));
    tot += ms;
  }
  *total_scan_ms = tot;
  *n_launches = g_prof_n;
  for (auto& e : g_prof_ev) (void)hipEventDestroy(e);
  g_prof_ev.clear();
  g_prof_on = false;
  return RARC_OK;
}

void rarc_set_error(const char* fmt, ...) {
  va_list ap;
  va_start(ap, fmt);
  vsnprintf(g_err, sizeof(g_err), fmt, ap);
  va_end(ap);
}

#include <dlfcn.h>
static int (*g_roctx_push)(const char*) = nullptr;
static int (*g_roctx_pop)() = nullptr;
static bool roctx_ready() {
  static const bool ok = [] {
    const char* e = getenv("RARC_ROCTX");
    if (!e || atoi(e) == 0) return false;
    void* h = dlopen("librocprofiler-sdk-roctx.so", RTLD_NOW | RTLD_GLOBAL);
    if (!h) h = dlopen("libroctx64.so", RTLD_NOW | RTLD_GLOBAL);
    if (!h) return false;
    g_roctx_push = (int (*)(const char*))dlsym(h, "roctxRangePushA");
    g_roctx_pop = (int (*)())dlsym(h, "roctxRangePop");
    return g_roctx_push && g_roctx_pop;
  }();
  return ok;
}
void rarc_roctx_push(const char* name) { if (roctx_ready()) g_roctx_push(name); }
void rarc_roctx_pop() { if (roctx_ready()) g_roctx_pop(); }

RarcLaunchExtras& rarc_launch_extras() {
  static thread_local RarcLaunchExtras x;
  return x;
}

extern "C" int rarc_version(void) { return RARC_BUILD_VERSION; }
extern "C" const char* rarc_last_error(void) { return g_err; }
extern "C" int rarc_padded_dim(int d) {
  return d <= 0 ? 0 : ((d + RARC_DIM_ALIGN - 1) / RARC_DIM_ALIGN) * RARC_DIM_ALIGN;
}

extern "C" size_t rarc_search_workspace_bytes(int cand_cap) {
  if (cand_cap < 4096) cand_cap = 4096;
  return RARC_WS_CAND + (size_t)RARC_MAX_QUERIES * (size_t)cand_cap * 8;
}

static int check_ws(void* ws, size_t bytes, int cap, const char* who) {
  RARC_REQUIRE(ws != nullptr && ((uintptr_t)ws % 256) == 0, RARC_E_WORKSPACE,
               "%s: workspace must be a 256-byte aligned device pointer", who);
  RARC_REQUIRE(cap >= 4096 && cap % RARC_MAX_WG == 0 && bytes >= rarc_search_workspace_bytes(cap), RARC_E_WORKSPACE,
               "%s: workspace of %zu bytes too small for cand_cap=%d (need %zu)", who, bytes, cap,
               rarc_search_workspace_bytes(cap));
  return RARC_OK;
}

extern "C" int rarc_search_f16(const uint16_t* d_corpus_f16, int64_t n_rows, int d_pad, const float* d_qmeta,
                               const void* d_qblock, int nq, int k, int kprime, int64_t id_base, float bin_lo,
                               float bin_hi, int64_t* d_out_ids, float* d_out_scores, uint32_t* d_status,
                               void* d_workspace, size_t workspace_bytes, int cand_cap, void* stream) {
  RARC_RANGE();
  RARC_REQUIRE(d_qblock && d_out_ids && d_out_scores && d_status, RARC_E_INVALID, "rarc_search_f16: null pointer");
  RARC_REQUIRE(n_rows >= 0 && n_rows < (int64_t)0xffffffe0ll, RARC_E_INVALID,
               "rarc_search_f16: n_rows=%lld outside [0, 2^32-32)", (long long)n_rows);
  RARC_REQUIRE(d_corpus_f16 || n_rows == 0, RARC_E_INVALID, "rarc_search_f16: null corpus");
  RARC_REQUIRE(d_pad > 0 && d_pad % RARC_DIM_ALIGN == 0, RARC_E_INVALID, "rarc_search_f16: d_pad=%d", d_pad);
  RARC_REQUIRE(nq >= 0 && nq <= RARC_MAX_QUERIES, RARC_E_INVALID, "rarc_search_f16: nq=%d outside [0,%d]", nq,
               RARC_MAX_QUERIES);
  RARC_REQUIRE(k >= 1 && k <= kprime && kprime <= RARC_MAX_K, RARC_E_INVALID,
               "rarc_search_f16: need 1 <= k (%d) <= kprime (%d) <= %d", k, kprime, RARC_MAX_K);
  RARC_REQUIRE(bin_hi > bin_lo, RARC_E_INVALID, "rarc_search_f16: empty histogram range");
  int rc = check_ws(d_workspace, workspace_bytes, cand_cap, "rarc_search_f16");
  if (rc) return rc;
  if (nq == 0) return RARC_OK;
  const RarcWs ws = rarc_ws_carve(d_workspace);
  const RarcQb qb = rarc_qb_carve(d_qblock, d_pad);
  hipStream_t s = (hipStream_t)stream;
  int n_wg = 0, hybrid = 0;
  if (d_qmeta) {
    Q8Search a{d_corpus_f16, nullptr, 0, d_pad, nq, k, cand_cap, id_base, qb.q32, qb.eps8, d_qmeta, qb.hq, qb.eps16, &ws, d_out_ids, d_out_scores,
               d_status, s};
    rc = rarc_scan_q8_launch(d_corpus_f16, nullptr, 0, n_rows, d_pad, d_qmeta, qb.q16, qb.q8, qb.qinv, qb.eps16,
                             qb.eps8, nq, kprime, bin_lo, bin_hi, ws, cand_cap, &n_wg, s, nullptr, q8_tighten, &a, qb.hq, qb.floor, &hybrid);
    if (rc) return rc;
    return rarc_finalize_q8_launch(d_corpus_f16, nullptr, 0, d_pad, qb.q32, qb.eps8, nq, k, id_base, ws, cand_cap,
                                   n_wg, d_out_ids, d_out_scores, d_status, s, 0, d_qmeta, qb.hq, hybrid ? qb.eps16 : nullptr);
  }
  rc = rarc_scan_f16_launch(d_corpus_f16, n_rows, d_pad, qb.q16, nq, kprime, bin_lo, bin_hi, ws, cand_cap, &n_wg, s,
                            qb.floor, qb.eps16);
  if (rc) return rc;
  return rarc_finalize_launch(d_corpus_f16, d_pad, qb.q32, qb.eps16, nq, k, kprime, id_base, ws, cand_cap, n_wg,
                              d_out_ids, d_out_scores, d_status, s);
}

extern "C" int rarc_repair_f16(const uint16_t* d_corpus_f16, int64_t n_rows, int d_pad, const void* d_qblock,
                               int q, int k, int64_t id_base, int64_t* d_out_ids, float* d_out_scores,
                               uint32_t* d_found, void* d_workspace, size_t workspace_bytes, void* stream) {
  RARC_RANGE();
  RARC_REQUIRE(d_corpus_f16 && d_qblock && d_out_ids && d_out_scores && d_found, RARC_E_INVALID,
               "rarc_repair_f16: null pointer");
  RARC_REQUIRE(q >= 0 && q < RARC_MAX_QUERIES && k >= 1 && k <= RARC_MAX_K && d_pad > 0 &&
                   d_pad % RARC_DIM_ALIGN == 0 && n_rows >= 0 && n_rows < (int64_t)0xffffffe0ll,
               RARC_E_INVALID, "rarc_repair_f16: bad arguments (q=%d k=%d)", q, k);
  int rc = check_ws(d_workspace, workspace_bytes, 4096, "rarc_repair_f16");
  if (rc) return rc;
  const int cap = (int)((workspace_bytes - RARC_WS_CAND) / 8);
  const RarcWs ws = rarc_ws_carve(d_workspace);
  const RarcQb qb = rarc_qb_carve(d_qblock, d_pad);
  return rarc_repair_launch(d_corpus_f16, nullptr, 0, n_rows, d_pad, qb.q32 + (size_t)q * d_pad, k, id_base,
                            d_out_ids + (size_t)q * k, d_out_scores + (size_t)q * k, d_found, ws, cap,
                            (hipStream_t)stream);
}

extern "C" int rarc_search_f16_shadow(const uint16_t* d_corpus_f16, const int8_t* d_shadow8, int64_t n_rows,
                                      int d_pad, const float* d_qmeta, const void* d_qblock, int nq, int k,
                                      int kprime, int64_t id_base, float bin_lo, float bin_hi, int64_t* d_out_ids,
                                      float* d_out_scores, uint32_t* d_status, void* d_workspace,
                                      size_t workspace_bytes, int cand_cap, void* stream) {
  RARC_RANGE();
  RARC_REQUIRE(d_qblock && d_qmeta && d_out_ids && d_out_scores && d_status, RARC_E_INVALID,
               "rarc_search_f16_shadow: null pointer");
  RARC_REQUIRE(n_rows >= 0 && n_rows < (int64_t)0xffffffe0ll, RARC_E_INVALID,
               "rarc_search_f16_shadow: n_rows=%lld outside [0, 2^32-32)", (long long)n_rows);
  RARC_REQUIRE((d_corpus_f16 && d_shadow8) || n_rows == 0, RARC_E_INVALID, "rarc_search_f16_shadow: null corpus");
  RARC_REQUIRE(d_pad > 0 && d_pad % 256 == 0, RARC_E_INVALID, "rarc_search_f16_shadow: d_pad=%d (multiple of 256)", d_pad);
  RARC_REQUIRE(nq >= 0 && nq <= RARC_MAX_QUERIES, RARC_E_INVALID, "rarc_search_f16_shadow: nq=%d outside [0,%d]", nq,
               RARC_MAX_QUERIES);
  RARC_REQUIRE(k >= 1 && k <= kprime && kprime <= RARC_MAX_K, RARC_E_INVALID,
               "rarc_search_f16_shadow: need 1 <= k (%d) <= kprime (%d) <= %d", k, kprime, RARC_MAX_K);
  RARC_REQUIRE(bin_hi > bin_lo, RARC_E_INVALID, "rarc_search_f16_shadow: empty histogram range");
  int rc = check_ws(d_workspace, workspace_bytes, cand_cap, "rarc_search_f16_shadow");
  if (rc) return rc;
  if (nq == 0) return RARC_OK;
  const RarcWs ws = rarc_ws_carve(d_workspace);
  const RarcQb qb = rarc_qb_carve(d_qblock, d_pad);
  hipStream_t s = (hipStream_t)stream;
  int n_wg = 0, hybrid = 0;
  Q8Search a{d_corpus_f16, nullptr, 0, d_pad, nq, k, cand_cap, id_base, qb.q32, qb.eps8, d_qmeta, qb.hq, qb.eps16, &ws, d_out_ids, d_out_scores,
             d_status, s};
  rc = rarc_scan_q8_launch(d_corpus_f16, nullptr, 2, n_rows, d_pad, d_qmeta, qb.q16, qb.q8, qb.qinv, qb.eps16, qb.eps8,
                           nq, kprime, bin_lo, bin_hi, ws, cand_cap, &n_wg, s, d_shadow8, q8_tighten, &a, qb.hq, qb.floor, nullptr);
  if (rc) return rc;
  return rarc_finalize_q8_launch(d_corpus_f16, nullptr, 0, d_pad, qb.q32, qb.eps8, nq, k, id_base, ws, cand_cap,
                                 n_wg, d_out_ids, d_out_scores, d_status, s, 0, d_qmeta, qb.hq, hybrid ? qb.eps16 : nullptr);
}

extern "C" int rarc_search_f32(const float* d_corpus_f32, const uint16_t* d_image_f16, int64_t n_rows, int d_pad,
                               const float* d_qmeta, const void* d_qblock, int nq, int k, int kprime, int64_t id_base,
                               float bin_lo, float bin_hi, int64_t* d_out_ids, float* d_out_scores,
                               uint32_t* d_status, void* d_workspace, size_t workspace_bytes, int cand_cap,
                               void* stream) {
  RARC_RANGE();
  RARC_REQUIRE(d_qblock && d_qmeta && d_out_ids && d_out_scores && d_status, RARC_E_INVALID,
               "rarc_search_f32: null pointer");
  RARC_REQUIRE(n_rows >= 0 && n_rows < (int64_t)0xffffffe0ll, RARC_E_INVALID,
               "rarc_search_f32: n_rows=%lld outside [0, 2^32-32)", (long long)n_rows);
  RARC_REQUIRE((d_corpus_f32 && d_image_f16) || n_rows == 0, RARC_E_INVALID, "rarc_search_f32: null corpus");
  RARC_REQUIRE(d_pad > 0 && d_pad % RARC_DIM_ALIGN == 0, RARC_E_INVALID, "rarc_search_f32: d_pad=%d", d_pad);
  RARC_REQUIRE(nq >= 0 && nq <= RARC_MAX_QUERIES, RARC_E_INVALID, "rarc_search_f32: nq=%d outside [0,%d]", nq,
               RARC_MAX_QUERIES);
  RARC_REQUIRE(k >= 1 && k <= kprime && kprime <= RARC_MAX_K, RARC_E_INVALID,
               "rarc_search_f32: need 1 <= k (%d) <= kprime (%d) <= %d", k, kprime, RARC_MAX_K);
  RARC_REQUIRE(bin_hi > bin_lo, RARC_E_INVALID, "rarc_search_f32: empty histogram range");
  int rc = check_ws(d_workspace, workspace_bytes, cand_cap, "rarc_search_f32");
  if (rc) return rc;
  if (nq == 0) return RARC_OK;
  const RarcWs ws = rarc_ws_carve(d_workspace);
  const RarcQb qb = rarc_qb_carve(d_qblock, d_pad);
  hipStream_t s = (hipStream_t)stream;
  int n_wg = 0, hybrid = 0;
  Q8Search a{d_corpus_f32, nullptr, 2, d_pad, nq, k, cand_cap, id_base, qb.q32, qb.eps8, d_qmeta, qb.hq, qb.eps16, &ws, d_out_ids, d_out_scores,
             d_status, s};
  rc = rarc_scan_q8_launch(d_image_f16, nullptr, 0, n_rows, d_pad, d_qmeta, qb.q16, qb.q8, qb.qinv, qb.eps16, qb.eps8,
                           nq, kprime, bin_lo, bin_hi, ws, cand_cap, &n_wg, s, nullptr, q8_tighten, &a, qb.hq, qb.floor, nullptr);
  if (rc) return rc;
  return rarc_finalize_q8_launch(d_corpus_f32, nullptr, 2, d_pad, qb.q32, qb.eps8, nq, k, id_base, ws, cand_cap, n_wg,
                                 d_out_ids, d_out_scores, d_status, s, 0, d_qmeta, qb.hq, hybrid ? qb.eps16 : nullptr);
}

extern "C" int rarc_repair_f32(const float* d_corpus_f32, int64_t n_rows, int d_pad, const void* d_qblock, int q, int k,
                               int64_t id_base, int64_t* d_out_ids, float* d_out_scores, uint32_t* d_found,
                               void* d_workspace, size_t workspace_bytes, void* stream) {
  RARC_RANGE();
  RARC_REQUIRE(d_corpus_f32 && d_qblock && d_out_ids && d_out_scores && d_found, RARC_E_INVALID,
               "rarc_repair_f32: null pointer");
  RARC_REQUIRE(q >= 0 && q < RARC_MAX_QUERIES && k >= 1 && k <= RARC_MAX_K && d_pad > 0 &&
                   d_pad % RARC_DIM_ALIGN == 0 && n_rows >= 0 && n_rows < (int64_t)0xffffffe0ll,
               RARC_E_INVALID, "rarc_repair_f32: bad arguments (q=%d k=%d)", q, k);
  int rc = check_ws(d_workspace, workspace_bytes, 4096, "rarc_repair_f32");
  if (rc) return rc;
  const int cap = (int)((workspace_bytes - RARC_WS_CAND) / 8);
  const RarcWs ws = rarc_ws_carve(d_workspace);
  const RarcQb qb = rarc_qb_carve(d_qblock, d_pad);
  return rarc_repair_launch(d_corpus_f32, nullptr, 2, n_rows, d_pad, qb.q32 + (size_t)q * d_pad, k, id_base,
                            d_out_ids + (size_t)q * k, d_out_scores + (size_t)q * k, d_found, ws, cap,
                            (hipStream_t)stream);
}

extern "C" int rarc_search_f8(const uint8_t* d_corpus_f8, const float* d_row_scale, int64_t n_rows, int d_pad,
                              const float* d_qmeta, const void* d_qblock, int nq, int k, int kprime,
                              int64_t id_base, float bin_lo, float bin_hi, int64_t* d_out_ids,
                              float* d_out_scores, uint32_t* d_status, void* d_workspace, size_t workspace_bytes,
                              int cand_cap, void* stream) {
  RARC_RANGE();
  RARC_REQUIRE(d_qblock && d_qmeta && d_out_ids && d_out_scores && d_status, RARC_E_INVALID,
               "rarc_search_f8: null pointer");
  RARC_REQUIRE(n_rows >= 0 && n_rows < (int64_t)0xffffffe0ll, RARC_E_INVALID,
               "rarc_search_f8: n_rows=%lld outside [0, 2^32-32)", (long long)n_rows);
  RARC_REQUIRE((d_corpus_f8 && d_row_scale) || n_rows == 0, RARC_E_INVALID, "rarc_search_f8: null corpus");
  RARC_REQUIRE(d_pad > 0 && d_pad % RARC_DIM_ALIGN_F8 == 0, RARC_E_INVALID, "rarc_search_f8: d_pad=%d", d_pad);
  RARC_REQUIRE(nq >= 0 && nq <= RARC_MAX_QUERIES, RARC_E_INVALID, "rarc_search_f8: nq=%d outside [0,%d]", nq,
               RARC_MAX_QUERIES);
  RARC_REQUIRE(k >= 1 && k <= kprime && kprime <= RARC_MAX_K, RARC_E_INVALID,
               "rarc_search_f8: need 1 <= k (%d) <= kprime (%d) <= %d", k, kprime, RARC_MAX_K);
  RARC_REQUIRE(bin_hi > bin_lo, RARC_E_INVALID, "rarc_search_f8: empty histogram range");
  int rc = check_ws(d_workspace, workspace_bytes, cand_cap, "rarc_search_f8");
  if (rc) return rc;
  if (nq == 0) return RARC_OK;
  const RarcWs ws = rarc_ws_carve(d_workspace);
  const RarcQb qb = rarc_qb_carve(d_qblock, d_pad);
  hipStream_t s = (hipStream_t)stream;
  int n_wg = 0, hybrid = 0;
  Q8Search a{d_corpus_f8, d_row_scale, 1, d_pad, nq, k, cand_cap, id_base, qb.q32, qb.eps8, d_qmeta, qb.hq, qb.eps16, &ws, d_out_ids, d_out_scores,
             d_status, s};
  rc = rarc_scan_q8_launch(d_corpus_f8, d_row_scale, 1, n_rows, d_pad, d_qmeta, qb.q16, qb.q8, qb.qinv, qb.eps16,
                           qb.eps8, nq, kprime, bin_lo, bin_hi, ws, cand_cap, &n_wg, s, nullptr, q8_tighten, &a, qb.hq, qb.floor, nullptr);
  if (rc) return rc;
  return rarc_finalize_q8_launch(d_corpus_f8, d_row_scale, 1, d_pad, qb.q32, qb.eps8, nq, k, id_base, ws, cand_cap,
                                 n_wg, d_out_ids, d_out_scores, d_status, s, 0, d_qmeta, qb.hq, hybrid ? qb.eps16 : nullptr);
}

extern "C" int rarc_repair_f8(const uint8_t* d_corpus_f8, const float* d_row_scale, int64_t n_rows, int d_pad,
                              const void* d_qblock, int q, int k, int64_t id_base, int64_t* d_out_ids,
                              float* d_out_scores, uint32_t* d_found, void* d_workspace, size_t workspace_bytes,
                              void* stream) {
  RARC_RANGE();
  RARC_REQUIRE(d_corpus_f8 && d_row_scale && d_qblock && d_out_ids && d_out_scores && d_found, RARC_E_INVALID,
               "rarc_repair_f8: null pointer");
  RARC_REQUIRE(q >= 0 && q < RARC_MAX_QUERIES && k >= 1 && k <= RARC_MAX_K && d_pad > 0 &&
                   d_pad % RARC_DIM_ALIGN_F8 == 0 && n_rows >= 0 && n_rows < (int64_t)0xffffffe0ll,
               RARC_E_INVALID, "rarc_repair_f8: bad arguments (q=%d k=%d)", q, k);
  int rc = check_ws(d_workspace, workspace_bytes, 4096, "rarc_repair_f8");
  if (rc) return rc;
  const int cap = (int)((workspace_bytes - RARC_WS_CAND) / 8);
  const RarcWs ws = rarc_ws_carve(d_workspace);
  const RarcQb qb = rarc_qb_carve(d_qblock, d_pad);
  return rarc_repair_launch(d_corpus_f8, d_row_scale, 1, n_rows, d_pad, qb.q32 + (size_t)q * d_pad, k, id_base,
                            d_out_ids + (size_t)q * k, d_out_scores + (size_t)q * k, d_found, ws, cap,
                            (hipStream_t)stream);
}

extern "C" int rarc_verify_batch(const void* d_rows, const float* d_row_scale, int row_format, int64_t n_rows, int d_pad,
                                 const void* d_qblock, int q_first, int nq, int k, int64_t id_base, const int64_t* d_ids,
                                 const float* d_scores, uint32_t* d_counts, void* stream) {
  RARC_RANGE();
  RARC_REQUIRE(d_rows && d_qblock && d_ids && d_scores && d_counts, RARC_E_INVALID, "rarc_verify_batch: null pointer");
  RARC_REQUIRE(row_format >= 0 && row_format <= 2 && (row_format != 1 || d_row_scale), RARC_E_INVALID,
               "rarc_verify_batch: row_format %d (0 fp16, 1 fp8 + scales, 2 fp32)", row_format);
  RARC_REQUIRE(nq >= 1 && nq <= 8 && q_first >= 0 && q_first + nq <= RARC_MAX_QUERIES && k >= 1 && k <= RARC_MAX_K &&
                   d_pad > 0 && d_pad % RARC_DIM_ALIGN == 0 && d_pad <= 1024 && n_rows >= 0 && n_rows < (int64_t)0xffffffe0ll,
               RARC_E_INVALID, "rarc_verify_batch: bad arguments (q_first=%d nq=%d k=%d d_pad=%d)", q_first, nq, k, d_pad);
  const RarcQb qb = rarc_qb_carve(d_qblock, d_pad);
  return rarc_verify_launch(d_rows, d_row_scale, row_format, n_rows, d_pad, qb.q32, q_first, nq, k, id_base, d_ids,
                            d_scores, d_counts, (hipStream_t)stream);
}

extern "C" int rarc_topk_merge(const int64_t* d_ids, const float* d_scores, int n_lists, int nq, int k,
                               int64_t* d_out_ids, float* d_out_scores, void* stream) {
  RARC_RANGE();
  RARC_REQUIRE(d_ids && d_scores && d_out_ids && d_out_scores, RARC_E_INVALID, "rarc_topk_merge: null pointer");
  RARC_REQUIRE(n_lists >= 1 && nq >= 0 && k >= 1, RARC_E_INVALID, "rarc_topk_merge: bad sizes");
  if (nq == 0) return RARC_OK;
  return rarc_merge_launch(d_ids, d_scores, n_lists, nq, k, d_out_ids, d_out_scores, (hipStream_t)stream, false);
}

extern "C" int rarc_pack_results(const int64_t* d_ids, const float* d_scores, int nq, int k, int32_t* d_packed, void* stream) {
  RARC_REQUIRE(d_ids && d_scores && d_packed && nq >= 0 && k >= 1, RARC_E_INVALID, "rarc_pack_results: bad arguments");
  if (nq == 0) return RARC_OK;
  return rarc_pack_launch(d_ids, d_scores, nq * k, (uint32_t*)d_packed, (hipStream_t)stream);
}

extern "C" int rarc_topk_merge_packed(const int32_t* d_packed, int n_lists, int nq, int k, int64_t* d_out_ids,
                                      float* d_out_scores, void* stream) {
  RARC_RANGE();
  RARC_REQUIRE(d_packed && d_out_ids && d_out_scores, RARC_E_INVALID, "rarc_topk_merge_packed: null pointer");
  RARC_REQUIRE(n_lists >= 1 && nq >= 0 && k >= 1, RARC_E_INVALID, "rarc_topk_merge_packed: bad sizes");
  if (nq == 0) return RARC_OK;
  return rarc_merge_launch((const int64_t*)d_packed, nullptr, n_lists, nq, k, d_out_ids, d_out_scores, (hipStream_t)stream, true);
}


extern "C" int rarc_search_batch(const RarcSearchBatch* b, void* stream) {
  RARC_RANGE();
  RARC_REQUIRE(b != nullptr, RARC_E_INVALID, "rarc_search_batch: null descriptor");
  RARC_REQUIRE(b->row_format >= 0 && b->row_format <= 3, RARC_E_INVALID, "rarc_search_batch: row_format %d", b->row_format);
  RARC_REQUIRE(b->d_status != nullptr, RARC_E_INVALID, "rarc_search_batch: null status");
  RarcLaunchExtras& x = rarc_launch_extras();
  struct Clear {
    RarcLaunchExtras& x;
    ~Clear() { x = RarcLaunchExtras(); }
  } clear{x};
  x.status_zero = b->d_status;
  x.flag_host = b->flag_host;
  x.gate = (hipEvent_t)b->gate_event;
  int rc = rarc_prep_queries(b->d_queries, b->ld_queries, b->nq, b->d, b->d_pad, b->normalize, b->corpus_max_norm, b->d_qmeta,
                             b->d_qblock, stream);
  if (rc) return rc;
  switch (b->row_format) {
    case 0:
      return rarc_search_f16((const uint16_t*)b->d_rows, b->n_rows, b->d_pad, b->d_qmeta, b->d_qblock, b->nq, b->k, b->kprime,
                             b->id_base, b->bin_lo, b->bin_hi, b->d_out_ids, b->d_out_scores, b->d_status, b->d_workspace,
                             b->workspace_bytes, b->cand_cap, stream);
    case 1:
      return rarc_search_f8((const uint8_t*)b->d_rows, (const float*)b->d_aux, b->n_rows, b->d_pad, b->d_qmeta, b->d_qblock, b->nq,
                            b->k, b->kprime, b->id_base, b->bin_lo, b->bin_hi, b->d_out_ids, b->d_out_scores, b->d_status,
                            b->d_workspace, b->workspace_bytes, b->cand_cap, stream);
    case 2:
      return rarc_search_f32((const float*)b->d_rows, (const uint16_t*)b->d_aux, b->n_rows, b->d_pad, b->d_qmeta, b->d_qblock, b->nq,
                             b->k, b->kprime, b->id_base, b->bin_lo, b->bin_hi, b->d_out_ids, b->d_out_scores, b->d_status,
                             b->d_workspace, b->workspace_bytes, b->cand_cap, stream);
    default:
      return rarc_search_f16_shadow((const uint16_t*)b->d_rows, (const int8_t*)b->d_aux, b->n_rows, b->d_pad, b->d_qmeta, b->d_qblock,
                                    b->nq, b->k, b->kprime, b->id_base, b->bin_lo, b->bin_hi, b->d_out_ids, b->d_out_scores,
                                    b->d_status, b->d_workspace, b->workspace_bytes, b->cand_cap, stream);
  }
}
```

### rag-arc_amd/csrc/rarc_common.h

```cpp
#pragma once
#include <hip/hip_runtime.h>
#include <stdint.h>
#include <stddef.h>
#include "../../include/rarc.h"

#if (defined(SCAN_HALFREAD) || defined(RARC_Q8_ABLATIONS) || defined(G256_SKIP_A1)) && !defined(RARC_EXPERIMENT)
#error "SCAN_HALFREAD / RARC_Q8_ABLATIONS / G256_SKIP_A1 build kernels with wrong results: measurement builds only, add -DRARC_EXPERIMENT"
#endif
#ifdef RARC_EXPERIMENT
#define RARC_BUILD_VERSION (RARC_VERSION + 100000)
#else
#define RARC_BUILD_VERSION RARC_VERSION
#endif

typedef _Float16 half_t;
typedef _Float16 half8 __attribute__((ext_vector_type(8)));
typedef float f32x16 __attribute__((ext_vector_type(16)));

#define RARC_GPTR(p) ((const __attribute__((address_space(1))) void*)(p))
#define RARC_LPTR(p) ((__attribute__((address_space(3))) void*)(p))

constexpr int RARC_NB = 256;
constexpr int RARC_MAX_WG = 256;
constexpr int RARC_SEED_TILES = 128;
constexpr int RARC_SEED_MAX_TILES = 2048;
constexpr size_t RARC_WS_THR = 0;
constexpr size_t RARC_WS_BINLO = 1024;
constexpr size_t RARC_WS_BINSCALE = 2048;
constexpr size_t RARC_WS_BININV = 3072;
constexpr size_t RARC_WS_CNT = 4096;
constexpr size_t RARC_WS_FLAGS = 5120;
constexpr int RARC_WS_TAIL_FLAG = 32;
static_assert(RARC_WS_FLAGS + 4 == RARC_WS_ANYFLAG_OFFSET, "include/rarc.h out of sync");
constexpr size_t RARC_WS_HIST = 8192;
constexpr size_t RARC_WS_CNT2 = RARC_WS_HIST + (size_t)RARC_MAX_QUERIES * RARC_NB * 4;
constexpr size_t RARC_WS_SEED = RARC_WS_CNT2 + (size_t)RARC_MAX_WG * RARC_MAX_QUERIES * 4;
constexpr size_t RARC_WS_CAND = RARC_WS_SEED + (size_t)RARC_MAX_QUERIES * RARC_SEED_MAX_TILES * 32 * 4;

struct RarcWs {
  float* thr;
  float* binlo;
  float* binscale;
  float* bininv;
  uint32_t* cnt;
  uint32_t* flags;
  uint32_t* hist;
  uint32_t* cnt2;
  float* seed;
  uint64_t* cand;
};
static inline RarcWs rarc_ws_carve(void* base) {
  char* b = (char*)base;
  RarcWs w;
  w.thr = (float*)(b + RARC_WS_THR);
  w.binlo = (float*)(b + RARC_WS_BINLO);
  w.binscale = (float*)(b + RARC_WS_BINSCALE);
  w.bininv = (float*)(b + RARC_WS_BININV);
  w.cnt = (uint32_t*)(b + RARC_WS_CNT);
  w.flags = (uint32_t*)(b + RARC_WS_FLAGS);
  w.hist = (uint32_t*)(b + RARC_WS_HIST);
  w.cnt2 = (uint32_t*)(b + RARC_WS_CNT2);
  w.seed = (float*)(b + RARC_WS_SEED);
  w.cand = (uint64_t*)(b + RARC_WS_CAND);
  return w;
}


struct RarcQb {
  float* q32;
  uint16_t* q16;
  int8_t* q8;
  float* eps16;
  float* eps8;
  float* qinv;
  float* hq;
  float* floor;
};
static inline size_t rarc_qb_bytes(int d_pad) { return (size_t)RARC_MAX_QUERIES * (size_t)d_pad * 7 + 5 * 1024; }
static inline RarcQb rarc_qb_carve(const void* base, int d_pad) {
  char* b = (char*)base;
  const size_t n = (size_t)RARC_MAX_QUERIES * (size_t)d_pad;
  RarcQb q;
  q.q32 = (float*)b;
  q.q16 = (uint16_t*)(b + n * 4);
  q.q8 = (int8_t*)(b + n * 6);
  q.eps16 = (float*)(b + n * 7);
  q.eps8 = (float*)(b + n * 7 + 1024);
  q.qinv = (float*)(b + n * 7 + 2048);
  q.hq = (float*)(b + n * 7 + 3072);
  q.floor = (float*)(b + n * 7 + 4096);
  return q;
}

__host__ __device__ static inline float rarc_bin_threshold(int b, float lo, float width) {
  return (b >= 2) ? lo + (float)(b - 1) * width : -__builtin_inff();
}
__host__ __device__ static inline int rarc_bin_of(float s, float lo, float scale) {
  const float x = (s - lo) * scale;
  int b = (x >= (float)(RARC_NB - 1)) ? RARC_NB - 1 : (x > 0.f ? (int)x : 0);
  return b;
}

#ifdef __HIPCC__
__device__ __forceinline__ int rarc_fresh_lane() {
  int l;
  asm volatile("v_mbcnt_lo_u32_b32 %0, -1, 0\n\tv_mbcnt_hi_u32_b32 %0, -1, %0" : "=v"(l));
  return l;
}
__device__ __forceinline__ uint32_t rarc_lds_add_rtn(uint32_t byte_addr, uint32_t v) {
  uint32_t old;
  asm volatile("ds_add_rtn_u32 %0, %1, %2\n\ts_waitcnt lgkmcnt(0)" : "=v"(old) : "v"(byte_addr), "v"(v) : "memory");
  return old;
}
__device__ __forceinline__ float rarc_lds_read_f32(uint32_t byte_addr) {
  float x;
  asm volatile("ds_read_b32 %0, %1\n\ts_waitcnt lgkmcnt(0)" : "=v"(x) : "v"(byte_addr) : "memory");
  return x;
}
__device__ __forceinline__ void rarc_lds_read_u32x4(uint32_t byte_addr, uint32_t& a, uint32_t& b, uint32_t& c,
                                                    uint32_t& d) {
  typedef uint32_t u32x4 __attribute__((ext_vector_type(4)));
  u32x4 v;
  asm volatile("ds_read_b128 %0, %1\n\ts_waitcnt lgkmcnt(0)" : "=v"(v) : "v"(byte_addr) : "memory");
  a = v[0]; b = v[1]; c = v[2]; d = v[3];
}
__device__ static inline int rarc_wave_find_from_top_256(uint32_t c0, uint32_t c1, uint32_t c2, uint32_t c3,
                                                         uint32_t need) {
  const int lane = rarc_fresh_lane();
  const uint32_t mine = c0 + c1 + c2 + c3;
  uint32_t suf = mine;
#pragma unroll
  for (int d = 1; d < 64; d <<= 1) {
    const uint32_t o = (uint32_t)__builtin_amdgcn_ds_bpermute(((lane + d) & 63) << 2, (int)suf);
    if (lane + d < 64) suf += o;
  }
  const unsigned long long ge = __builtin_amdgcn_ballot_w64(suf >= need);
  if (!ge) return -1;
  const int hl = 63 - __builtin_clzll(ge);
  const uint32_t above = __shfl(suf - mine, hl, 64);
  const uint32_t h3 = __shfl(c3, hl, 64), h2 = __shfl(c2, hl, 64), h1 = __shfl(c1, hl, 64);
  int b = 4 * hl;
  if (above + h3 >= need) b += 3;
  else if (above + h3 + h2 >= need) b += 2;
  else if (above + h3 + h2 + h1 >= need) b += 1;
  return b;
}
__device__ static inline int rarc_wave_find_from_top(const uint32_t* cnt, int nbins, uint32_t need,
                                                     uint32_t* above_out) {
  const int lane = rarc_fresh_lane();
  const int per = nbins / 64;
  const uint32_t* mine = cnt + lane * per;
  uint32_t tot = 0;
  for (int i = 0; i < per; ++i) tot += mine[i];
  uint32_t suf = tot;
#pragma unroll
  for (int d = 1; d < 64; d <<= 1) {
    const uint32_t o = __shfl_down(suf, d, 64);
    if (lane + d < 64) suf += o;
  }
  const unsigned long long ge = __builtin_amdgcn_ballot_w64(suf >= need);
  if (!ge) return -1;
  const int hl = 63 - __builtin_clzll(ge);
  uint32_t above = __shfl(suf - tot, hl, 64);
  int b = -1;
  if (lane == hl) {
    for (int i = per - 1; i >= 0; --i) {
      const uint32_t c = mine[i];
      if (above + c >= need) { b = lane * per + i; break; }
      above += c;
    }
  }
  b = __shfl(b, hl, 64);
  *above_out = __shfl(above, hl, 64);
  return b;
}
#endif

__host__ __device__ static inline uint32_t rarc_ordkey(float f) {
  union { float f; uint32_t u; } x; x.f = f;
  return (x.u & 0x80000000u) ? ~x.u : (x.u | 0x80000000u);
}
__host__ __device__ static inline float rarc_unordkey(uint32_t k) {
  union { float f; uint32_t u; } x;
  x.u = (k & 0x80000000u) ? (k & 0x7fffffffu) : ~k;
  return x.f;
}
__host__ __device__ static inline uint64_t rarc_candkey(float score, uint32_t row) {
  return ((uint64_t)rarc_ordkey(score) << 32) | (uint64_t)(~row);
}
__host__ __device__ static inline uint32_t rarc_candrow(uint64_t key) { return ~(uint32_t)key; }
__host__ __device__ static inline float rarc_candscore(uint64_t key) {
  return rarc_unordkey((uint32_t)(key >> 32));
}

__host__ __device__ static inline float rarc_canon_tree(const float a[8]) {
  return ((a[0] + a[4]) + (a[2] + a[6])) + ((a[1] + a[5]) + (a[3] + a[7]));
}


#define RARC_MFMA_SETTLE(acc)                  \
  do {                                         \
    __builtin_amdgcn_sched_barrier(0);         \
    asm volatile("s_nop 4");                   \
    __builtin_amdgcn_sched_barrier(0);         \
  } while (0)

struct RarcLaunchExtras {
  uint32_t* status_zero = nullptr;
  uint32_t* flag_host = nullptr;
  hipEvent_t gate = nullptr;
};
RarcLaunchExtras& rarc_launch_extras();
inline int rarc_gate_scan(hipStream_t s) {
  RarcLaunchExtras& x = rarc_launch_extras();
  if (x.gate) {
    hipEvent_t g = x.gate;
    x.gate = nullptr;
    if (hipStreamWaitEvent(s, g, 0) != hipSuccess) return -2;
  }
  return 0;
}

typedef _Float16 half2_t __attribute__((ext_vector_type(2)));
typedef int i32x4 __attribute__((ext_vector_type(4)));
typedef int i32x16 __attribute__((ext_vector_type(16)));
#ifdef __HIPCC__
__device__ __forceinline__ uint2 rarc_quant8_chunk(const uint4 v, const half_t s) {
  const half2_t s2 = {s, s}, c2 = {(half_t)1536.f, (half_t)1536.f};
  const half2_t y0 = __builtin_elementwise_fma(__builtin_bit_cast(half2_t, v.x), s2, c2);
  const half2_t y1 = __builtin_elementwise_fma(__builtin_bit_cast(half2_t, v.y), s2, c2);
  const half2_t y2 = __builtin_elementwise_fma(__builtin_bit_cast(half2_t, v.z), s2, c2);
  const half2_t y3 = __builtin_elementwise_fma(__builtin_bit_cast(half2_t, v.w), s2, c2);
  uint2 o;
  o.x = __builtin_amdgcn_perm(__builtin_bit_cast(uint32_t, y1), __builtin_bit_cast(uint32_t, y0), 0x06040200u);
  o.y = __builtin_amdgcn_perm(__builtin_bit_cast(uint32_t, y3), __builtin_bit_cast(uint32_t, y2), 0x06040200u);
  return o;
}
#endif
__host__ __device__ static inline uint8_t rarc_f8_encode(float x) {
  union { float f; uint32_t u; } c; c.f = x;
  uint32_t u = c.u;
  const uint8_t sign = (uint8_t)((u >> 24) & 0x80);
  u &= 0x7fffffffu;
  c.u = u;
  const float a = c.f;
  if (!(a == a)) return sign;
  if (a >= 448.0f) return sign | 0x7e;
  if (a < 0.015625f) return sign | (uint8_t)(int)__builtin_rintf(a * 512.0f);
  uint32_t r = u + 0x0007ffffu + ((u >> 20) & 1u);
  r >>= 20;
  uint32_t code = r - ((127u - 7u) << 3);
  if (code > 0x7eu) code = 0x7eu;
  return sign | (uint8_t)code;
}
#ifdef __HIPCC__
typedef float float2_t __attribute__((ext_vector_type(2)));
__device__ __forceinline__ void rarc_f8x4_to_f32(uint32_t w, float (&o)[4]) {
  const float2_t lo = __builtin_amdgcn_cvt_pk_f32_fp8(w, false), hi = __builtin_amdgcn_cvt_pk_f32_fp8(w, true);
  o[0] = lo.x; o[1] = lo.y; o[2] = hi.x; o[3] = hi.y;
}
__device__ __forceinline__ uint4 rarc_quant8_chunk_f8(const uint4 v, const half_t mul) {
  const half2_t m2 = {mul, mul}, c2 = {(half_t)1536.f, (half_t)1536.f};
  const uint32_t w[4] = {v.x, v.y, v.z, v.w};
  uint32_t o[4];
#pragma unroll
  for (int i = 0; i < 4; ++i) {
    const half2_t lo = __builtin_amdgcn_cvt_scalef32_pk_f16_fp8(w[i], 1.0f, false);
    const half2_t hi = __builtin_amdgcn_cvt_scalef32_pk_f16_fp8(w[i], 1.0f, true);
    const half2_t ylo = __builtin_elementwise_fma(lo, m2, c2), yhi = __builtin_elementwise_fma(hi, m2, c2);
    o[i] = __builtin_amdgcn_perm(__builtin_bit_cast(uint32_t, yhi), __builtin_bit_cast(uint32_t, ylo), 0x06040200u);
  }
  return make_uint4(o[0], o[1], o[2], o[3]);
}
#endif
constexpr int RARC_DIM_ALIGN_F8 = 256;
constexpr int RARC_QMETA_F8_STRIDE = 34;

constexpr int RARC_QMETA_HDR = 4;
constexpr int RARC_QMETA_STRIDE = 2;
static inline __host__ __device__ float rarc_tmeta_pack(uint16_t s_half_bits, uint16_t rt_half_bits) {
  const uint32_t w = ((uint32_t)rt_half_bits << 16) | (uint32_t)s_half_bits;
  return __builtin_bit_cast(float, w);
}

__host__ __device__ static inline void rarc_query_scale8(float mx, float* sq_out, float* qi_out) {
  float sq = (mx > 0.f && mx < __builtin_inff()) ? 127.f / mx : 1.f;
  if (!(sq < __builtin_inff())) sq = 1.f;
  *sq_out = sq;
  *qi_out = 1.0f / sq;
}

void rarc_set_error(const char* fmt, ...);
#define RARC_HIP_CHECK(expr)                                                              \
  do {                                                                                    \
    hipError_t _e = (expr);                                                               \
    if (_e != hipSuccess) {                                                               \
      rarc_set_error("%s failed: %s (%s:%d)", #expr, hipGetErrorString(_e), __FILE__,     \
                     __LINE__);                                                           \
      return RARC_E_HIP;                                                                  \
    }                                                                                     \
  } while (0)
struct RarcPerDevice {
  size_t v[64] = {};
  size_t& cur() {
    int d = 0;
    (void)hipGetDevice(&d);
    return v[(d < 0 ? 0 : d) & 63];
  }
};

#define RARC_REQUIRE(cond, code, ...)  \
  do {                                 \
    if (!(cond)) {                     \
      rarc_set_error(__VA_ARGS__);     \
      return (code);                   \
    }                                  \
  } while (0)

void rarc_roctx_push(const char* name);
void rarc_roctx_pop();
struct RarcRange {
  explicit RarcRange(const char* name) { rarc_roctx_push(name); }
  ~RarcRange() { rarc_roctx_pop(); }
  RarcRange(const RarcRange&) = delete;
  RarcRange& operator=(const RarcRange&) = delete;
};
#define RARC_RANGE() RarcRange rarc_range_guard_(__func__)
```

### rag-arc_amd/hip/binding.py

```python
from __future__ import annotations

import ctypes
import os
import threading
from ctypes import c_double, c_float, c_int, c_int64, c_size_t, c_uint64, c_void_p

_PKG = os.path.dirname(os.path.dirname(os.path.abspath(__file__)))
_LIB = os.environ.get("RARC_LIBRARY") or os.path.join(_PKG, "lib", "librarc_hip.so")

MAX_QUERIES = 256
MAX_K = 1024
WIDE_MAX_K = 8192
WIDE_MAX_DPAD = 4096
DIM_ALIGN = 128
Q_UNCERTAIN = 1
Q_OVERFLOW = 2
WS_ANYFLAG_OFFSET = 5124


class RarcError(RuntimeError):
    """Raised for every non-zero status returned by librarc_hip.so."""


class RarcUnsupported(RarcError, NotImplementedError):
    """A search the reference's `IndexFlatIP.search` would answer (any d, any k: VectorStore_Faiss.py:262) that this backend
    REFUSES — the storage x path matrix in INTEGRATION.md ("What the backend refuses").  A refusal is loud and happens before
    anything is launched; the message names the configuration that does answer the call.  Also a NotImplementedError, the
    type the reference's VectorStore base raises for what a store does not implement (VectorStoreBase.py:145-176)."""


class EncLayer(ctypes.Structure):
    _fields_ = [(n, c_void_p) for n in ("qkv_w", "qkv_b", "o_w", "o_b", "ln1_g", "ln1_b", "f1_w", "f1_b", "f2_w",
                                        "f2_b", "ln2_g", "ln2_b")]


class EncModel(ctypes.Structure):
    _fields_ = [("hidden", c_int), ("heads", c_int), ("inter", c_int), ("n_layers", c_int), ("ln_eps", c_float),
                ("word", c_void_p), ("pos", c_void_p), ("type0", c_void_p), ("emb_g", c_void_p), ("emb_b", c_void_p),
                ("layers", ctypes.POINTER(EncLayer)), ("vocab", c_int), ("max_pos", c_int),
                ("rel_bias", c_void_p), ("rel_span", c_int)]


class Enc32Layer(ctypes.Structure):
    _fields_ = [(n, c_void_p) for n in ("qkv_w3", "qkv_rw", "qkv_b", "o_w3", "o_rw", "o_b", "ln1_g", "ln1_b", "f1_w3", "f1_rw",
                                        "f1_b", "f2_w3", "f2_rw", "f2_b", "ln2_g", "ln2_b", "f1_colmax",
                                        "qkv_wq", "o_wq", "f1_wq", "f2_wq")]


class Enc32Model(ctypes.Structure):
    _fields_ = [("hidden", c_int), ("heads", c_int), ("inter", c_int), ("n_layers", c_int), ("ln_eps", c_float),
                ("word", c_void_p), ("pos", c_void_p), ("type0", c_void_p), ("emb_g", c_void_p), ("emb_b", c_void_p),
                ("layers", ctypes.POINTER(Enc32Layer)), ("vocab", c_int), ("max_pos", c_int),
                ("rel_bias", c_void_p), ("rel_span", c_int)]


class SearchBatch(ctypes.Structure):
    _fields_ = [("d_rows", c_void_p), ("d_aux", c_void_p), ("row_format", c_int), ("n_rows", c_int64), ("d_pad", c_int),
                ("d_qmeta", c_void_p),
                ("d_queries", c_void_p), ("ld_queries", c_int64), ("nq", c_int), ("d", c_int), ("normalize", c_int),
                ("corpus_max_norm", c_float), ("d_qblock", c_void_p),
                ("k", c_int), ("kprime", c_int), ("id_base", c_int64), ("bin_lo", c_float), ("bin_hi", c_float),
                ("d_out_ids", c_void_p), ("d_out_scores", c_void_p), ("d_status", c_void_p), ("flag_host", c_void_p),
                ("d_workspace", c_void_p), ("workspace_bytes", c_size_t), ("cand_cap", c_int),
                ("gate_event", c_void_p)]


class IoStats(ctypes.Structure):
    _fields_ = [("bytes", c_int64), ("seconds", c_double), ("file_seconds", c_double), ("copy_wait_seconds", c_double),
                ("direct_bytes", c_int64), ("n_chunks", c_int64), ("slot_bytes", c_int64), ("n_threads", c_int),
                ("direct", c_int)]


IO_DIRECT = 1
IO_FSYNC = 2
IO_TRUNCATE = 4


class LmLayer(ctypes.Structure):
    _fields_ = [(n, c_void_p) for n in ("in_norm", "qkv_w", "q_norm", "k_norm", "o_w", "post_norm", "gate_up_w", "down_w",
                                        "qkv_w_folded", "gate_up_w_folded")]


class LmModel(ctypes.Structure):
    _fields_ = [("hidden", c_int), ("n_layers", c_int), ("n_q_heads", c_int), ("n_kv_heads", c_int), ("head_dim", c_int),
                ("inter", c_int), ("vocab", c_int), ("rms_eps", c_float), ("rope_theta", c_float), ("embed", c_void_p),
                ("lm_head", c_void_p), ("final_norm", c_void_p), ("zero_bias", c_void_p), ("layers", ctypes.POINTER(LmLayer))]


_lock = threading.Lock()
_lib = None

SIGNATURES = {
    "rarc_version": (c_int, []),
    "rarc_last_error": (ctypes.c_char_p, []),
    "rarc_padded_dim": (c_int, [c_int]),
    "rarc_l2norm_rows_f32": (c_int, [c_void_p, c_int64, c_void_p, c_int64, c_int64, c_int, c_void_p]),
    "rarc_cosine_matrix_f32": (c_int, [c_void_p, c_int64, c_int, c_void_p, c_int64, c_int, c_int, c_void_p, c_void_p]),
    "rarc_adjacent_cosine_distance_f32": (c_int, [c_void_p, c_int64, c_int, c_int, c_void_p, c_void_p]),
    "rarc_ingest_f16": (c_int, [c_void_p, c_int64, c_void_p, c_int, c_void_p, c_int64, c_int, c_int, c_void_p]),
    "rarc_quant_meta_floats": (c_size_t, [c_int64]),
    "rarc_quant_meta_f16": (c_int, [c_void_p, c_int64, c_int, c_int64, c_void_p, c_void_p]),
    "rarc_debug_q8_scores": (c_int, [c_void_p, c_int64, c_int, c_void_p, c_void_p, c_int, c_void_p, c_void_p]),
    "rarc_debug_q8_scores_f8": (c_int, [c_void_p, c_int64, c_int, c_void_p, c_void_p, c_int, c_void_p, c_void_p]),
    "rarc_query_block_bytes": (c_size_t, [c_int]),
    "rarc_prep_queries": (c_int, [c_void_p, c_int64, c_int, c_int, c_int, c_int, c_float, c_void_p, c_void_p,
                                  c_void_p]),
    "rarc_qblock_set_floor": (c_int, [c_void_p, c_int, c_void_p, c_void_p, c_int, c_int, c_void_p]),
    "rarc_search_workspace_bytes": (c_size_t, [c_int]),
    "rarc_search_f16": (c_int, [c_void_p, c_int64, c_int, c_void_p, c_void_p, c_int, c_int, c_int,
                                c_int64, c_float, c_float, c_void_p, c_void_p, c_void_p, c_void_p, c_size_t,
                                c_int, c_void_p]),
    "rarc_repair_f16": (c_int, [c_void_p, c_int64, c_int, c_void_p, c_int, c_int, c_int64, c_void_p, c_void_p,
                                c_void_p, c_void_p, c_size_t, c_void_p]),
    "rarc_verify_batch": (c_int, [c_void_p, c_void_p, c_int, c_int64, c_int, c_void_p, c_int, c_int, c_int, c_int64, c_void_p,
                                  c_void_p, c_void_p, c_void_p]),
    "rarc_quant_shadow_f16": (c_int, [c_void_p, c_int64, c_int, c_int64, c_void_p, c_void_p, c_void_p]),
    "rarc_search_f16_shadow": (c_int, [c_void_p, c_void_p, c_int64, c_int, c_void_p, c_void_p, c_int, c_int, c_int,
                                       c_int64, c_float, c_float, c_void_p, c_void_p, c_void_p, c_void_p, c_size_t,
                                       c_int, c_void_p]),
    "rarc_ingest_f32": (c_int, [c_void_p, c_int64, c_void_p, c_void_p, c_int, c_void_p, c_int64, c_int, c_int, c_void_p]),
    "rarc_search_f32": (c_int, [c_void_p, c_void_p, c_int64, c_int, c_void_p, c_void_p, c_int, c_int, c_int,
                                c_int64, c_float, c_float, c_void_p, c_void_p, c_void_p, c_void_p, c_size_t,
                                c_int, c_void_p]),
    "rarc_repair_f32": (c_int, [c_void_p, c_int64, c_int, c_void_p, c_int, c_int, c_int64, c_void_p, c_void_p,
                                c_void_p, c_void_p, c_size_t, c_void_p]),
    "rarc_padded_dim_f8": (c_int, [c_int]),
    "rarc_ingest_f8": (c_int, [c_void_p, c_int64, c_void_p, c_int, c_void_p, c_void_p, c_int64, c_int, c_int, c_void_p]),
    "rarc_quant_meta_floats_f8": (c_size_t, [c_int64]),
    "rarc_quant_meta_f8": (c_int, [c_void_p, c_void_p, c_int64, c_int, c_int64, c_void_p, c_void_p]),
    "rarc_search_f8": (c_int, [c_void_p, c_void_p, c_int64, c_int, c_void_p, c_void_p, c_int, c_int, c_int,
                               c_int64, c_float, c_float, c_void_p, c_void_p, c_void_p, c_void_p, c_size_t,
                               c_int, c_void_p]),
    "rarc_repair_f8": (c_int, [c_void_p, c_void_p, c_int64, c_int, c_void_p, c_int, c_int, c_int64, c_void_p,
                               c_void_p, c_void_p, c_void_p, c_size_t, c_void_p]),
    "rarc_topk_merge": (c_int, [c_void_p, c_void_p, c_int, c_int, c_int, c_void_p, c_void_p, c_void_p]),
    "rarc_pack_results": (c_int, [c_void_p, c_void_p, c_int, c_int, c_void_p, c_void_p]),
    "rarc_topk_merge_packed": (c_int, [c_void_p, c_int, c_int, c_int, c_void_p, c_void_p, c_void_p]),
    "rarc_rrf_fuse": (c_int, [c_void_p, c_void_p, c_int, c_int, c_int, c_double, c_int, c_void_p, c_void_p,
                              c_void_p, c_void_p]),
    "rarc_rerank_order": (c_int, [c_void_p, c_void_p, c_int, c_int, c_void_p, c_void_p, c_void_p]),
    "rarc_mmr_workspace_doubles": (c_size_t, [c_int, c_int]),
    "rarc_mmr_select": (c_int, [c_void_p, c_int64, c_void_p, c_int, c_int, c_int, c_int, c_double, c_void_p, c_void_p,
                                c_void_p]),
    "rarc_mmr_rows_workspace_bytes": (c_size_t, [c_int, c_int, c_int]),
    "rarc_mmr_select_rows": (c_int, [c_void_p, c_int, c_void_p, c_int64, c_int, c_int, c_void_p, c_int64, c_int, c_void_p, c_int,
                                     c_int64, c_int, c_int, c_double, c_void_p, c_void_p, c_size_t, c_void_p]),
    "rarc_synth_rows_f16": (c_int, [c_void_p, c_int, c_int, c_int64, c_int64, c_uint64, c_void_p]),
    "rarc_synth_rows_f32": (c_int, [c_void_p, c_int64, c_int, c_int64, c_int64, c_uint64, c_void_p]),
    "rarc_enc_embed_ln": (c_int, [c_void_p, c_void_p, c_void_p, c_void_p, c_void_p, c_void_p, c_float, c_int, c_int,
                                  c_int, c_int, c_void_p, c_void_p]),
    "rarc_enc_gemm": (c_int, [c_void_p, c_void_p, c_void_p, c_void_p, c_int, c_int, c_int, c_int, c_void_p]),
    "rarc_enc_gemm_zero_bias": (c_int, [c_void_p, c_void_p, c_void_p, c_void_p, c_int, c_int, c_int, c_int, c_void_p]),
    "rarc_enc_attention": (c_int, [c_void_p, c_void_p, c_int, c_int, c_int, c_int, c_void_p, c_void_p]),
    "rarc_enc_add_ln": (c_int, [c_void_p, c_void_p, c_void_p, c_void_p, c_float, c_int, c_int, c_void_p, c_void_p]),
    "rarc_enc_pool": (c_int, [c_void_p, c_int, c_int, c_int, c_int, c_void_p, c_void_p]),
    "rarc_enc_pool_mean": (c_int, [c_void_p, c_void_p, c_int, c_int, c_int, c_int, c_void_p, c_void_p]),
    "rarc_enc_workspace_bytes": (c_size_t, [c_int, c_int, c_int]),
    "rarc_enc_forward": (c_int, [c_void_p, c_void_p, c_void_p, c_int, c_int, c_int, c_void_p, c_size_t, c_void_p,
                                 c_void_p]),
    "rarc_enc32_split_weight": (c_int, [c_void_p, c_int, c_int, c_void_p, c_void_p, c_void_p]),
    "rarc_search_batch": (c_int, [c_void_p, c_void_p]),
    "rarc_stream_read": (c_int, [c_void_p, c_size_t, c_void_p, c_void_p]),
    "rarc_enc32_pack_query_weight": (c_int, [c_void_p, c_int, c_int, c_void_p, c_void_p]),
    "rarc_enc32_split_rows": (c_int, [c_void_p, c_int, c_int, c_void_p, c_void_p, c_void_p]),
    "rarc_enc32_gemm": (c_int, [c_void_p, c_void_p, c_void_p, c_void_p, c_void_p, c_void_p, c_int, c_int, c_int, c_void_p]),
    "rarc_enc32_workspace_bytes": (c_size_t, [c_int, c_int, c_int]),
    "rarc_enc32_forward": (c_int, [c_void_p, c_void_p, c_void_p, c_int, c_int, c_int, c_void_p, c_size_t, c_void_p,
                                   c_void_p]),
    "rarc_lm_workspace_bytes": (c_size_t, [c_void_p, c_int]),
    "rarc_lm_yes_no_logits": (c_int, [c_void_p, c_void_p, c_void_p, c_int, c_int, c_int, c_int, c_void_p, c_size_t, c_void_p,
                                      c_void_p]),
    "rarc_lm_prefix_cache_bytes": (c_size_t, [c_void_p, c_int]),
    "rarc_lm_prefix_kv": (c_int, [c_void_p, c_void_p, c_void_p, c_int, c_int, c_void_p, c_size_t, c_void_p, c_size_t, c_void_p]),
    "rarc_lm_yes_no_logits_prefixed": (c_int, [c_void_p, c_void_p, c_void_p, c_int, c_int, c_void_p, c_void_p, c_int, c_int,
                                                c_void_p, c_int, c_int, c_void_p, c_size_t, c_void_p, c_void_p]),
    "rarc_lm_embed_last": (c_int, [c_void_p, c_void_p, c_void_p, c_int, c_int, c_int, c_int, c_void_p, c_size_t, c_void_p, c_int64,
                                   c_void_p]),
    "rarc_lm_embed_last_prefixed": (c_int, [c_void_p, c_void_p, c_void_p, c_int, c_int, c_void_p, c_void_p, c_int, c_int, c_void_p,
                                            c_int, c_int, c_void_p, c_size_t, c_void_p, c_int64, c_void_p]),
    "rarc_lm_rope_table": (c_int, [c_int, c_int, c_float, c_void_p, c_void_p]),
    "rarc_lm_rmsnorm": (c_int, [c_void_p, c_void_p, c_void_p, c_float, c_int, c_int, c_void_p, c_void_p]),
    "rarc_lm_rowscale_parts": (c_int, [c_void_p, c_int, c_float, c_int, c_int, c_void_p, c_void_p]),
    "rarc_lm_swiglu": (c_int, [c_void_p, c_int, c_int, c_void_p, c_void_p]),
    "rarc_lm_attention": (c_int, [c_void_p, c_void_p, c_int, c_int, c_int, c_int, c_int, c_void_p, c_void_p, c_float, c_void_p, c_int,
                                  c_void_p, c_void_p, c_void_p, c_int, c_int, c_int, c_void_p, c_void_p]),
    "rarc_lm_last_logits": (c_int, [c_void_p, c_void_p, c_void_p, c_float, c_int, c_int, c_int, c_int, c_int, c_int, c_int, c_void_p,
                                    c_void_p]),
    "rarc_lm_last_embed": (c_int, [c_void_p, c_void_p, c_float, c_int, c_int, c_int, c_int, c_int, c_int, c_void_p, c_int64,
                                   c_void_p]),
    "rarc_lm_gather_last": (c_int, [c_void_p, c_int, c_int, c_int, c_int, c_void_p, c_void_p]),
    "rarc_wordpiece_create": (c_int, [ctypes.c_char_p, c_size_t, c_int, ctypes.c_char_p, ctypes.c_char_p, ctypes.c_char_p,
                                      ctypes.c_char_p, ctypes.c_char_p, c_size_t, c_int, ctypes.POINTER(c_void_p)]),
    "rarc_wordpiece_destroy": (None, [c_void_p]),
    "rarc_wordpiece_encode": (c_int, [c_void_p, ctypes.c_char_p, c_void_p, c_int, c_int, c_void_p, c_int64, c_void_p, c_int]),
    "rarc_file_to_device": (c_int, [ctypes.c_char_p, c_int, ctypes.POINTER(c_int64), ctypes.POINTER(c_int64),
                                    ctypes.POINTER(c_int64), c_void_p, c_int64, c_void_p, c_size_t, c_int, c_int, c_void_p,
                                    ctypes.POINTER(IoStats)]),
    "rarc_device_to_file": (c_int, [ctypes.c_char_p, c_int, ctypes.POINTER(c_int64), ctypes.POINTER(c_int64),
                                    ctypes.POINTER(c_int64), c_void_p, c_int64, c_void_p, c_size_t, c_int, c_int, c_void_p,
                                    ctypes.POINTER(IoStats)]),
    "rarc_wide_workspace_bytes": (c_size_t, [c_int, c_int]),
    "rarc_search_wide": (c_int, [c_void_p, c_void_p, c_int, c_int64, c_int, c_float, c_float, c_void_p, c_int, c_int, c_int64,
                                 c_void_p, c_void_p, c_void_p, c_void_p, c_size_t, c_int, c_void_p]),
    "rarc_row_sqnorms": (c_int, [c_void_p, c_int, c_int64, c_int, c_int64, c_void_p, c_void_p]),
    "rarc_search_wide_l2": (c_int, [c_void_p, c_void_p, c_int, c_int64, c_int, c_float, c_float, c_void_p, c_void_p, c_int, c_int,
                                    c_int64, c_void_p, c_void_p, c_void_p, c_void_p, c_size_t, c_int, c_void_p]),
    "rarc_debug_wide_bounds": (c_int, [c_void_p, c_size_t, c_int, c_int, c_void_p, c_void_p]),
    "rarc_debug_query_scale8": (c_int, [c_float, ctypes.POINTER(c_float), ctypes.POINTER(c_float)]),
    "rarc_debug_q8_tail_plan": (c_int, [ctypes.c_uint32, ctypes.c_uint32, ctypes.c_uint32, c_int, c_int, c_int, c_int,
                                        ctypes.POINTER(ctypes.c_uint32), ctypes.POINTER(ctypes.c_uint32), ctypes.POINTER(ctypes.c_uint32)]),
    "rarc_debug_q8_tail_chunks": (c_int, [ctypes.c_uint32] * 7 + [c_void_p, c_void_p]),
    "rarc_debug_q8_tail_counter_offset": (c_int64, [c_int]),
    "rarc_search_rows_workspace_bytes": (c_size_t, [c_int, c_int]),
    "rarc_search_rows": (c_int, [c_void_p, c_int, c_int64, c_int, c_void_p, c_int, c_void_p, c_int64, c_int, c_int64, c_void_p, c_int,
                                 c_void_p, c_void_p, c_void_p, c_void_p, c_size_t, c_void_p]),
    "rarc_strike_rows": (c_int, [c_void_p, c_void_p, c_int, c_int, c_void_p, c_int64, c_int64, c_int, c_int, c_void_p, c_void_p,
                                 c_void_p, c_void_p]),
    "rarc_search_rows_grouped_workspace_bytes": (c_size_t, [c_int, c_int]),
    "rarc_search_rows_grouped": (c_int, [c_void_p, c_int, c_int64, c_int, c_void_p, c_int, c_void_p, c_void_p, c_int, c_int64, c_int,
                                         c_int64, c_void_p, c_int, c_void_p, c_void_p, c_void_p, c_void_p, c_size_t, c_void_p]),
    "rarc_strike_rows_grouped": (c_int, [c_void_p, c_void_p, c_int, c_int, c_void_p, c_void_p, c_int64, c_int64, c_int, c_int,
                                         c_void_p, c_void_p, c_void_p, c_void_p]),
    "rarc_similar_pairs_workspace_bytes": (c_size_t, [c_int64, c_int, c_int]),
    "rarc_similar_pairs": (c_int, [c_void_p, c_int64, c_int64, c_int, ctypes.c_double, c_void_p, c_size_t, c_int, c_void_p, c_void_p,
                                   c_int64, c_void_p, c_void_p, c_void_p]),
    "rarc_knn_graph_workspace_bytes": (c_size_t, [c_int64, c_int, c_int, c_int]),
    "rarc_knn_graph": (c_int, [c_void_p, c_int64, c_int64, c_int, c_int, ctypes.c_double, c_void_p, c_size_t, c_int, c_void_p, c_void_p,
                               c_void_p, c_void_p, c_void_p]),
    "rarc_graph_csr_workspace_bytes": (c_size_t, [c_int64, c_int64]),
    "rarc_graph_csr": (c_int, [c_void_p, c_void_p, c_void_p, c_int64, c_int64, c_void_p, c_size_t, c_void_p]),
    "rarc_louvain_workspace_bytes": (c_size_t, [c_int64, c_int64]),
    "rarc_louvain_init": (c_int, [c_void_p, c_size_t, c_int64, c_int64, c_void_p, c_size_t, c_void_p, c_void_p]),
    "rarc_louvain_sweep": (c_int, [c_void_p, c_size_t, c_int64, c_int64, c_void_p, c_size_t, c_int, c_int, c_void_p, c_void_p]),
    "rarc_louvain_aggregate": (c_int, [c_void_p, c_size_t, c_int64, c_int64, c_void_p, c_size_t, c_int, c_void_p, c_int64, c_void_p,
                                       c_void_p, c_void_p, c_void_p, c_void_p]),
    "rarc_louvain_labels_workspace_bytes": (c_size_t, [c_int64]),
    "rarc_louvain_labels": (c_int, [c_void_p, c_int64, c_void_p, c_size_t, c_void_p]),
    "rarc_louvain_limits": (c_int, [ctypes.POINTER(c_int)]),
    "rarc_ppr_workspace_bytes": (c_size_t, [c_int64, c_int64, c_int]),
    "rarc_ppr_seed": (c_int, [c_void_p, c_size_t, c_int64, c_int64, c_void_p, c_void_p, c_int, c_int, c_void_p, c_size_t, c_void_p]),
    "rarc_ppr_step": (c_int, [c_void_p, c_size_t, c_int64, c_int64, c_int, c_int, c_int64, c_int, c_void_p, c_size_t, c_void_p,
                              c_void_p]),
    "rarc_ppr_scores": (c_int, [c_int64, c_int64, c_int, c_void_p, c_size_t, c_void_p, c_void_p]),
    "rarc_ppr_topk": (c_int, [c_int64, c_int64, c_int, c_int, c_int, c_void_p, c_size_t, c_void_p, c_void_p, c_void_p, c_void_p]),
    "rarc_ppr_limits": (c_int, [ctypes.POINTER(c_int)]),
    "rarc_ppr_chunks_workspace_bytes": (c_size_t, [c_int64, c_int]),
    "rarc_ppr_chunks": (c_int, [c_int64, c_int64, c_int, c_int, c_void_p, c_size_t, c_void_p, c_void_p, c_void_p, c_int64, c_int64,
                                c_void_p, c_int64, c_void_p, c_size_t, c_void_p]),
    "rarc_ppr_chunks_scores": (c_int, [c_int64, c_int, c_void_p, c_size_t, c_void_p, c_void_p]),
    "rarc_ppr_chunks_topk": (c_int, [c_int64, c_int, c_int, c_void_p, c_size_t, c_void_p, c_void_p, c_void_p, c_void_p]),
    "rarc_ppr_chunks_limits": (c_int, [ctypes.POINTER(c_int)]),
    "rarc_khop_workspace_bytes": (c_size_t, [c_int64, c_int64, c_int, c_int]),
    "rarc_khop_seed": (c_int, [c_int64, c_int64, c_void_p, c_int, c_int, c_int, c_void_p, c_size_t, c_void_p]),
    "rarc_khop_step": (c_int, [c_void_p, c_size_t, c_int64, c_int64, c_int, c_int, c_int, c_void_p, c_size_t, c_void_p, c_void_p]),
    "rarc_khop_counts": (c_int, [c_int64, c_int64, c_int, c_int, c_void_p, c_size_t, c_void_p, c_void_p]),
    "rarc_khop_levels": (c_int, [c_int64, c_int64, c_int, c_int, c_void_p, c_size_t, c_void_p, c_void_p]),
    "rarc_khop_list": (c_int, [c_int64, c_int64, c_int, c_int, c_int, c_void_p, c_size_t, c_void_p, c_void_p, c_void_p, c_void_p]),
    "rarc_khop_chunks": (c_int, [c_int64, c_int64, c_int, c_int, c_void_p, c_void_p, c_size_t, c_void_p, c_void_p, c_void_p, c_int64,
                                 c_int64, c_void_p, c_int64, c_void_p, c_size_t, c_void_p]),
    "rarc_khop_limits": (c_int, [ctypes.POINTER(c_int)]),
    "rarc_khop_edges_workspace_bytes": (c_size_t, [c_int64, c_int, c_int]),
    "rarc_khop_edges": (c_int, [c_int64, c_int64, c_int, c_int, c_void_p, c_size_t, c_void_p, c_int64, c_int, c_void_p, c_size_t, c_void_p,
                                c_void_p, c_void_p, c_void_p, c_void_p]),
    "rarc_khop_edges_limits": (c_int, [ctypes.POINTER(c_int)]),
    "rarc_khop_paths": (c_int, [c_int64, c_int64, c_int, c_int, c_int, c_void_p, c_size_t, c_void_p, c_void_p, c_size_t, c_void_p, c_void_p]),
    "rarc_khop_path_edges": (c_int, [c_int64, c_int64, c_int, c_int, c_void_p, c_size_t, c_void_p, c_int64, c_int, c_void_p, c_size_t,
                                     c_void_p, c_void_p, c_void_p, c_void_p, c_void_p]),
    "rarc_khop_paths_limits": (c_int, [ctypes.POINTER(c_int)]),
    "rarc_graph_types_workspace_bytes": (c_size_t, [c_int64, c_int64]),
    "rarc_graph_types": (c_int, [c_void_p, c_size_t, c_int64, c_int64, c_void_p, c_void_p, c_void_p, c_size_t, c_void_p]),
    "rarc_khop_step_typed": (c_int, [c_void_p, c_size_t, c_void_p, c_size_t, c_void_p, c_int64, c_int64, c_int, c_int, c_int, c_void_p,
                                     c_size_t, c_void_p, c_void_p]),
    "rarc_khop_edges_typed": (c_int, [c_int64, c_int64, c_int, c_int, c_void_p, c_size_t, c_void_p, c_int64, c_void_p, c_int, c_void_p, c_int,
                                      c_void_p, c_size_t, c_void_p, c_void_p, c_void_p, c_void_p, c_void_p]),
    "rarc_khop_path_edges_typed": (c_int, [c_int64, c_int64, c_int, c_int, c_void_p, c_size_t, c_void_p, c_int64, c_void_p, c_int, c_void_p,
                                           c_int, c_void_p, c_size_t, c_void_p, c_void_p, c_void_p, c_void_p, c_void_p]),
    "rarc_graph_types_weighted_workspace_bytes": (c_size_t, [c_int64, c_int64]),
    "rarc_graph_types_weighted": (c_int, [c_void_p, c_size_t, c_int64, c_int64, c_void_p, c_void_p, c_void_p, c_void_p, c_size_t, c_void_p]),
    "rarc_ppr_seed_typed": (c_int, [c_void_p, c_size_t, c_void_p, c_size_t, c_void_p, c_int64, c_int64, c_void_p, c_void_p, c_int, c_int,
                                    c_void_p, c_size_t, c_void_p]),
    "rarc_ppr_step_typed": (c_int, [c_void_p, c_size_t, c_void_p, c_size_t, c_void_p, c_int64, c_int64, c_int, c_int, c_int64, c_int, c_void_p,
                                    c_size_t, c_void_p, c_void_p]),
    "rarc_ingest_pairs_workspace_bytes": (c_size_t, [c_int64, c_int64]),
    "rarc_ingest_pairs": (c_int, [c_void_p, c_void_p, c_void_p, c_int64, c_void_p, c_void_p, c_void_p, c_int64, c_int64, c_void_p, c_size_t,
                                  c_void_p, c_void_p, c_void_p, c_void_p, c_void_p]),
    "rarc_ingest_mentions_workspace_bytes": (c_size_t, [c_int64, c_int64, c_int64]),
    "rarc_ingest_mentions": (c_int, [c_void_p, c_void_p, c_int64, c_void_p, c_void_p, c_void_p, c_int64, c_int64, c_int64, c_int64, c_void_p,
                                     c_size_t, c_void_p, c_void_p, c_void_p, c_void_p, c_void_p, c_void_p]),
    "rarc_ingest_limits": (c_int, [ctypes.POINTER(c_int)]),
    "rarc_sort_reduce_workspace_bytes": (c_size_t, [c_int64]),
    "rarc_sort_reduce": (c_int, [c_void_p, c_void_p, c_int64, c_int, c_void_p, c_size_t, c_void_p, c_void_p, c_void_p, c_void_p]),
    "rarc_sort_reduce_limits": (c_int, [ctypes.POINTER(c_int)]),
    "rarc_merge_plan_workspace_bytes": (c_size_t, [c_int64]),
    "rarc_merge_plan": (c_int, [c_void_p, c_void_p, c_int64, c_void_p, c_size_t, c_void_p, c_void_p, c_void_p, c_void_p, c_void_p, c_void_p]),
    "rarc_merge_pairs_workspace_bytes": (c_size_t, [c_int64]),
    "rarc_merge_pairs": (c_int, [c_void_p, c_void_p, c_int64, c_void_p, c_int64, c_void_p, c_size_t, c_void_p, c_void_p, c_void_p, c_void_p]),
    "rarc_merge_mentions_workspace_bytes": (c_size_t, [c_int64, c_int64]),
    "rarc_merge_mentions": (c_int, [c_void_p, c_void_p, c_void_p, c_int64, c_int64, c_void_p, c_int64, c_void_p, c_size_t, c_void_p, c_void_p,
                                    c_void_p, c_void_p, c_void_p, c_void_p]),
    "rarc_merge_relations_workspace_bytes": (c_size_t, [c_int64]),
    "rarc_merge_relations": (c_int, [c_void_p, c_int64, c_void_p, c_int64, c_void_p, c_size_t, c_void_p, c_void_p, c_void_p, c_void_p]),
    "rarc_components_workspace_bytes": (c_size_t, [c_int64, c_int64]),
    "rarc_components_init": (c_int, [c_int64, c_int64, c_void_p, c_size_t, c_void_p]),
    "rarc_components_round": (c_int, [c_void_p, c_size_t, c_int64, c_int64, c_void_p, c_size_t, c_void_p, c_void_p]),
    "rarc_components_finish": (c_int, [c_int64, c_int64, c_void_p, c_size_t, c_void_p, c_void_p, c_void_p, c_void_p, c_void_p]),
    "rarc_components_limits": (c_int, [ctypes.POINTER(c_int)]),
    "rarc_cooccur_workspace_bytes": (c_size_t, [c_int64, c_int64]),
    "rarc_cooccur_count": (c_int, [c_void_p, c_void_p, c_void_p, c_int64, c_int64, c_int64, c_int, c_void_p, c_size_t, c_void_p, c_void_p]),
    "rarc_cooccur_emit": (c_int, [c_void_p, c_void_p, c_void_p, c_int64, c_int64, c_int64, c_int, c_void_p, c_size_t, c_void_p, c_void_p,
                                  c_int64, c_void_p]),
    "rarc_cooccur_edges_workspace_bytes": (c_size_t, [c_int64]),
    "rarc_cooccur_edges": (c_int, [c_void_p, c_void_p, c_int64, c_int64, c_int64, c_void_p, c_size_t, c_void_p, c_void_p, c_void_p, c_void_p]),
    "rarc_cooccur_limits": (c_int, [ctypes.POINTER(c_int)]),
    "rarc_compact_rows": (c_int, [c_void_p, c_int64, c_int64, c_void_p, c_int64, c_int64, c_void_p, c_size_t, c_void_p]),
    "rarc_vmem_create": (c_int, [c_int, c_size_t, c_size_t, c_size_t, ctypes.POINTER(c_void_p)]),
    "rarc_vmem_grow": (c_int, [c_void_p, c_size_t]),
    "rarc_vmem_base": (c_void_p, [c_void_p]),
    "rarc_vmem_mapped": (c_size_t, [c_void_p]),
    "rarc_vmem_reserved": (c_size_t, [c_void_p]),
    "rarc_vmem_slab": (c_size_t, [c_void_p]),
    "rarc_vmem_granularity": (c_size_t, [c_void_p]),
    "rarc_vmem_destroy": (c_int, [c_void_p]),
    "rarc_profile_begin": (c_int, [c_int]),
    "rarc_profile_end": (c_int, [ctypes.POINTER(c_double), ctypes.POINTER(c_int)]),
    "rarc_bm25_workspace_bytes": (c_size_t, [c_int, c_int64, c_int64, c_int]),
    "rarc_bm25_topk": (c_int, [c_void_p, c_void_p, c_void_p, c_int64, c_int64, c_void_p, c_void_p, c_void_p, c_int, c_int64,
                               c_int, c_void_p, c_size_t, c_void_p, c_void_p, c_void_p]),
    "rarc_bm25_scores": (c_int, [c_void_p, c_void_p, c_void_p, c_int64, c_int64, c_void_p, c_void_p, c_void_p, c_int, c_int64,
                                 c_void_p, c_size_t, c_void_p, c_void_p]),
}


def library_path() -> str:
    return _LIB


def load_library() -> ctypes.CDLL:
    global _lib
    with _lock:
        if _lib is None:
            if not os.path.exists(_LIB):
                raise RarcError(
                    f"{_LIB} not found: build it with `python -c 'import __graft_entry__ as g; g.build()'` "
                    "(there is no CPU fallback)")
            lib = ctypes.CDLL(_LIB)
            lib.rarc_version.restype = c_int
            if lib.rarc_version() >= 100000 and os.environ.get("RARC_ALLOW_EXPERIMENT") != "1":
                raise RarcError(f"{_LIB} is a MEASUREMENT build (-DRARC_EXPERIMENT: it may contain kernels that return wrong "
                                "results on purpose); set RARC_ALLOW_EXPERIMENT=1 to load it from a bench tool")
            for name, (res, args) in SIGNATURES.items():
                fn = getattr(lib, name)
                fn.restype = res
                fn.argtypes = args
            _lib = lib
    return _lib


def check(rc: int, what: str = "") -> None:
    if rc != 0:
        msg = load_library().rarc_last_error()
        raise RarcError(f"{what or 'librarc_hip'} failed ({rc}): {msg.decode() if msg else '?'}")


def padded_dim(d: int, align: int = DIM_ALIGN) -> int:
    return ((d + align - 1) // align) * align
```

Measured before the change: 9886 queries/s.

## Make q8 finalize incremental across tighten passes by carrying top-k and consumed counts

The finalize kernel gains an incremental mode. Each tighten pass saves its sorted top-k, per-workgroup consumed candidate counts and threshold into a new workspace region. Later passes and the final finalize then scan only the candidates appended since the previous pass, instead of re-walking and rescoring every candidate segment. If a candidate buffer overflows or bisection is needed, the kernel falls back to the full walk. This costs extra workspace, more complex control flow with gotos, and extra sorting work to store the carried top-k.

```diff
diff --git a/include/rarc.h b/include/rarc.h
--- a/include/rarc.h
+++ b/include/rarc.h
@@ -307,6 +307,10 @@
 int rarc_debug_q8_tail_chunks(uint32_t k_first, uint32_t n, uint32_t stride, uint32_t unit, uint32_t t_dyn, uint32_t r0,
                               uint32_t n_tiles, uint32_t* t0, uint32_t* t_end);
 int64_t rarc_debug_q8_tail_counter_offset(int launch);
+int rarc_debug_fin_inc_layout(int cand_cap, int64_t* out6);
+int rarc_debug_finalize_q8(const uint16_t* d_corpus_f16, int d_pad, const void* d_qblock, int nq, int k, int64_t id_base,
+                           int n_wg, int tighten, int inc_mode, int64_t* d_out_ids, float* d_out_scores, uint32_t* d_status,
+                           void* d_workspace, size_t workspace_bytes, int cand_cap, void* stream);
 
 size_t rarc_search_rows_workspace_bytes(int nq, int k);
 int rarc_search_rows(const void* d_rows, int fmt, int64_t n_rows, int d_pad, const void* d_qblock, int nq, const int64_t* d_list,
diff --git a/rag-arc_amd/csrc/finalize.hip b/rag-arc_amd/csrc/finalize.hip
--- a/rag-arc_amd/csrc/finalize.hip
+++ b/rag-arc_amd/csrc/finalize.hip
@@ -254,6 +254,8 @@
   int tighten_mode;
   const float* eps16;
   uint32_t* flag_host;
+  int inc_mode;
+  RarcFinInc inc;
 };
 
 __global__ __launch_bounds__(FIN8_THREADS) void rarc_finalize_q8_kernel(const Fin8Params p) {
@@ -287,30 +289,70 @@
   }
   __syncthreads();
   float t1 = s_t1;
-
-  auto collect = [&](auto want) {
+  uint32_t npass = 0, nk = 0;
+  bool inc = false;
+  bool clean = p.inc_mode == 1;
+  float tp0 = 0.f, tp1 = 0.f, tp2 = 0.f;
+  auto uni = [](uint32_t x) { return (uint32_t)__builtin_amdgcn_readfirstlane((int)x); };
+  auto unif = [&](float x) { return __uint_as_float(uni(__float_as_uint(x))); };
+  const bool over = uni(s_over) != 0u;
+  if (p.inc_mode == 2) {
+    const uint32_t st = uni(p.inc.state[q]);
+    if (st >= 1u && st <= (uint32_t)RARC_FIN_INC_PASSES && !over) {
+      npass = st;
+      nk = uni(p.inc.nk[q]);
+      nk = nk < (uint32_t)p.k ? nk : (uint32_t)p.k;
+      inc = clean = true;
+      tp0 = unif(p.inc.t1[q]);
+      tp1 = unif(p.inc.t1[RARC_MAX_QUERIES + q]);
+      tp2 = unif(p.inc.t1[2 * RARC_MAX_QUERIES + q]);
+    }
+  }
+  if (over) clean = false;
+
+  auto collect = [&](auto inc_c, bool new_only, auto want) {
+    constexpr bool INC = decltype(inc_c)::value;
+    typedef uint32_t u32x4 __attribute__((ext_vector_type(4)));
     constexpr int U = FIN8_COLLECT_U;
     const int lane = tid & 63, wv = tid >> 6, nwv = blockDim.x >> 6;
     for (uint32_t wg0 = wv * U; wg0 < p.n_wg; wg0 += nwv * U) {
-      uint32_t n[U];
-      uint32_t nmax = 0;
+      uint32_t n[U], lo[U];
+      uint32_t cs0[U], cs1[U], cs2[U];
+      uint32_t nmax = 0, lomin = 0xffffffffu;
 #pragma unroll
       for (int u = 0; u < U; ++u) {
         const uint32_t wg = wg0 + u;
         const uint32_t c = wg < p.n_wg ? s_cnt[wg] : 0u;
         n[u] = c < p.seg ? c : p.seg;
-        nmax = n[u] > nmax ? n[u] : nmax;
-      }
-      for (uint32_t base = 0; base < nmax; base += 64) {
+        lo[u] = 0;
+        if constexpr (INC) {
+          const u32x4 v = wg < p.n_wg ? *(const u32x4*)(p.inc.cons + ((size_t)q * RARC_MAX_WG + wg) * 4) : (u32x4){0u, 0u, 0u, 0u};
+          cs0[u] = __builtin_amdgcn_readfirstlane(v[0]);
+          cs1[u] = __builtin_amdgcn_readfirstlane(v[1]);
+          cs2[u] = __builtin_amdgcn_readfirstlane(v[2]);
+          const uint32_t last = npass == 1u ? cs0[u] : (npass == 2u ? cs1[u] : cs2[u]);
+          if (npass < 2u) cs1[u] = last;
+          if (npass < 3u) cs2[u] = last;
+          if (new_only) lo[u] = last < n[u] ? last : n[u];
+        }
+        if (lo[u] < n[u]) {
+          nmax = n[u] > nmax ? n[u] : nmax;
+          lomin = lo[u] < lomin ? lo[u] : lomin;
+        }
+      }
+      for (uint32_t base = lomin & ~63u; base < nmax; base += 64) {
         uint64_t key[U];
 #pragma unroll
         for (int u = 0; u < U; ++u) {
           const uint32_t i = base + lane;
-          key[u] = i < n[u] ? p.cand[((size_t)q * RARC_MAX_WG + wg0 + u) * p.seg + i] : 0ull;
+          key[u] = (i >= lo[u] && i < n[u]) ? p.cand[((size_t)q * RARC_MAX_WG + wg0 + u) * p.seg + i] : 0ull;
         }
 #pragma unroll
         for (int u = 0; u < U; ++u) {
-          if (base + lane < n[u] && want(rarc_candscore(key[u]), rarc_candrow(key[u]))) {
+          const uint32_t i = base + lane;
+          float tp = t1;
+          if constexpr (INC) tp = i < cs0[u] ? tp0 : (i < cs1[u] ? tp1 : (i < cs2[u] ? tp2 : t1));
+          if (i >= lo[u] && i < n[u] && want(rarc_candscore(key[u]), rarc_candrow(key[u]), tp)) {
             const uint32_t e = atomicAdd(&s_ne, 1u);
             if (e < FIN8_RS) ex[e] = key[u];
           }
@@ -404,7 +446,7 @@
   };
 
   constexpr int FIN8_SMALL = 1024;
-  auto select_kth = [&](int n, int kth) __attribute__((always_inline)) -> uint64_t {
+  auto select_kth = [&](int n, int kth, uint64_t* sorted) __attribute__((always_inline)) -> uint64_t {
     if (n <= FIN8_SMALL) {
       __syncthreads();
       for (int i = tid; i < n; i += blockDim.x) {
@@ -412,6 +454,7 @@
         int rank = 0;
         for (int j = 0; j < n; ++j) rank += (ex[j] > mine);
         if (rank == kth - 1) { s_selb = (int)(mine >> 32); s_selabove = (uint32_t)mine; }
+        if (sorted && rank < kth) sorted[rank] = mine;
       }
       __syncthreads();
       const uint64_t r = ((uint64_t)(uint32_t)s_selb << 32) | s_selabove;
@@ -440,18 +483,52 @@
       need -= s_selabove;
     }
     __syncthreads();
+    if (sorted) {
+      uint64_t* top = (uint64_t*)fsm;
+      if (tid == 0) s_cmp = 0;
+      __syncthreads();
+      for (int i = tid; i < n; i += blockDim.x) {
+        const uint64_t mine = ex[i];
+        if (mine >= prefix) top[atomicAdd(&s_cmp, 1u)] = mine;
+      }
+      __syncthreads();
+      for (int i = tid; i < kth; i += blockDim.x) {
+        const uint64_t mine = top[i];
+        int rank = 0;
+        for (int j = 0; j < kth; ++j) rank += (top[j] > mine);
+        sorted[rank] = mine;
+      }
+      __syncthreads();
+    }
     return prefix;
   };
   static_assert(RARC_NB == 256, "the radix select counts one byte per pass in s_hist");
 
   FIN8_STAMP(1)
-  collect([&](float a, uint32_t) { return a >= t1; });
-  __syncthreads();
-  if (s_ne > (uint32_t)FIN8_RS && t1 > -INFINITY) {
+  const std::false_type full_c{};
+  const std::true_type inc_c{};
+full_walk:
+  bool bisected = false;
+  if (inc) {
+    collect(inc_c, true, [&](float a, uint32_t, float) { return a >= t1; });
+    __syncthreads();
+    if (s_ne + nk > (uint32_t)FIN8_RS) {
+      inc = clean = false;
+      __syncthreads();
+      if (tid == 0) s_ne = 0;
+      __syncthreads();
+      goto full_walk;
+    }
+  } else {
+    collect(full_c, false, [&](float a, uint32_t, float) { return a >= t1; });
+    __syncthreads();
+  }
+  if (!inc && s_ne > (uint32_t)FIN8_RS && t1 > -INFINITY) {
+    bisected = true;
     __syncthreads();
     if (tid == 0) s_cmp = 0;
     __syncthreads();
-    collect([&](float a, uint32_t) { atomicMax(&s_cmp, rarc_ordkey(a)); return false; });
+    collect(full_c, false, [&](float a, uint32_t, float) { atomicMax(&s_cmp, rarc_ordkey(a)); return false; });
     __syncthreads();
     float a_lo = t1, a_hi = rarc_unordkey(s_cmp + 1u);
     __syncthreads();
@@ -461,7 +538,7 @@
       __syncthreads();
       if (tid == 0) s_ne = 0;
       __syncthreads();
-      collect([&](float a, uint32_t) { return a >= mid; });
+      collect(full_c, false, [&](float a, uint32_t, float) { return a >= mid; });
       __syncthreads();
       const uint32_t c = s_ne;
       if (c > (uint32_t)FIN8_RS) a_lo = mid;
@@ -472,19 +549,28 @@
       __syncthreads();
       if (tid == 0) s_ne = 0;
       __syncthreads();
-      collect([&](float a, uint32_t) { return a >= t1; });
+      collect(full_c, false, [&](float a, uint32_t, float) { return a >= t1; });
       __syncthreads();
     }
   }
   FIN8_STAMP(2)
-  const uint32_t ne1_all = s_ne;
+  const uint32_t ne_new = uni(s_ne);
+  const uint32_t ne1_all = ne_new + (inc ? nk : 0u);
   const int ne1 = ne1_all < FIN8_RS ? (int)ne1_all : FIN8_RS;
-  rescore(0, ne1);
+  rescore(0, inc ? (int)ne_new : ne1);
+  if (inc) {
+    for (uint32_t i = tid; i < nk; i += blockDim.x) ex[ne_new + i] = p.inc.top[(size_t)q * RARC_MAX_K + i];
+    if (tid == 0) s_ne = ne1_all;
+  }
   __syncthreads();
   FIN8_STAMP(3)
+  clean = clean && p.tighten_thr && !bisected && ne1_all <= (uint32_t)FIN8_RS && npass < (uint32_t)RARC_FIN_INC_PASSES;
+  uint64_t* const carry = clean ? p.inc.top + (size_t)q * RARC_MAX_K : nullptr;
   if (ne1 >= p.k) {
-    const uint64_t kth = select_kth(ne1, p.k);
+    const uint64_t kth = select_kth(ne1, p.k, carry);
     if (tid == 0) s_L = rarc_candscore(kth);
+  } else if (carry && ne1 >= 1) {
+    select_kth(ne1, ne1, carry);
   }
   __syncthreads();
   const float L = s_L;
@@ -498,6 +584,21 @@
       const float cur = __uint_as_float(p.tighten_thr[q]);
       if (cur > -INFINITY && cur < INFINITY) p.tighten_thr[q] = __float_as_uint(cur - (1.0002f * fmaxf(eps - e16, 0.f) + 1e-7f));
     }
+    if (p.inc_mode) {
+      if (clean) {
+        for (int i = tid; i < RARC_MAX_WG; i += blockDim.x) {
+          const uint32_t c = s_cnt[i];
+          p.inc.cons[((size_t)q * RARC_MAX_WG + i) * 4 + npass] = c < p.seg ? c : p.seg;
+        }
+      }
+      if (tid == 0) {
+        p.inc.state[q] = clean ? npass + 1u : RARC_FIN_INC_POISON;
+        if (clean) {
+          p.inc.nk[q] = (uint32_t)(ne1 < p.k ? ne1 : p.k);
+          p.inc.t1[npass * RARC_MAX_QUERIES + q] = t1;
+        }
+      }
+    }
     return;
   }
 
@@ -511,7 +612,19 @@
     const float rt = (float)__builtin_bit_cast(half_t, (uint16_t)(w >> 16));
     return a + fmaxf(eps - hqv * fmaxf(r_max - rt, 0.f), e16) * 1.0001f >= ref;
   };
-  if (ne1_all <= (uint32_t)FIN8_RS && t1 > -INFINITY) collect([&](float a, uint32_t row) { return a < t1 && reaches(a, row, L); });
+  if (inc) {
+    collect(inc_c, false, [&](float a, uint32_t row, float cut) { return a < cut && reaches(a, row, L); });
+    __syncthreads();
+    if (s_ne > (uint32_t)FIN8_RS) {
+      inc = false;
+      __syncthreads();
+      if (tid == 0) { s_ne = 0; s_L = -INFINITY; }
+      __syncthreads();
+      goto full_walk;
+    }
+  } else if (ne1_all <= (uint32_t)FIN8_RS && t1 > -INFINITY) {
+    collect(full_c, false, [&](float a, uint32_t row, float) { return a < t1 && reaches(a, row, L); });
+  }
   __syncthreads();
   FIN8_STAMP(5)
   uint32_t ne_all = s_ne;
@@ -522,7 +635,7 @@
   if (ne_all > (uint32_t)FIN8_RS && ne1_all <= (uint32_t)FIN8_RS && ne1 >= p.k && L > -INFINITY) {
     uint64_t* tmp = (uint64_t*)fsm;
     auto keep_top_k = [&](int n) {
-      const uint64_t kth = select_kth(n, p.k);
+      const uint64_t kth = select_kth(n, p.k, nullptr);
       if (tid == 0) { s_cmp = 0; s_L = rarc_candscore(kth); }
       __syncthreads();
       for (int i = tid; i < n; i += blockDim.x) {
@@ -544,7 +657,7 @@
       if (tid == 0) s_ne = (uint32_t)p.k;
       __syncthreads();
       const float lc = s_L;
-      collect([&](float a, uint32_t row) { return a >= lo && a < hi && reaches(a, row, lc); });
+      collect(full_c, false, [&](float a, uint32_t row, float) { return a >= lo && a < hi && reaches(a, row, lc); });
       __syncthreads();
       const uint32_t cnt = s_ne;
       if (cnt > (uint32_t)FIN8_RS) {
@@ -590,7 +703,7 @@
     }
   } else {
     uint64_t* top = (uint64_t*)fsm;
-    const uint64_t kth = select_kth(ne, kk);
+    const uint64_t kth = select_kth(ne, kk, nullptr);
     if (tid == 0) s_cmp = 0;
     __syncthreads();
     for (int i = tid; i < ne; i += blockDim.x) {
@@ -623,10 +736,10 @@
 }
 
 unsigned long long* g_fin8_dbg = nullptr;
-int rarc_finalize_q8_launch(const void* corpus, const float* rowscale, int fmt, int d_pad, const float* q32,
-                            const float* eps8, int nq, int k, int64_t id_base, const RarcWs& ws, int cap, int n_wg,
-                            int64_t* out_ids, float* out_scores, uint32_t* status, hipStream_t s, int tighten,
-                            const float* qmeta, const float* hq, const float* eps16) {
+int rarc_finalize_q8_launch_inc(const void* corpus, const float* rowscale, int fmt, int d_pad, const float* q32,
+                                const float* eps8, int nq, int k, int64_t id_base, const RarcWs& ws, int cap, int n_wg,
+                                int64_t* out_ids, float* out_scores, uint32_t* status, hipStream_t s, int tighten,
+                                const float* qmeta, const float* hq, const float* eps16, int inc_mode) {
   RARC_REQUIRE(d_pad <= FIN8_MAXD, RARC_E_UNSUPPORTED, "rarc_finalize_q8: d_pad %d > %d", d_pad, FIN8_MAXD);
   Fin8Params p;
   p.corpus = corpus;
@@ -656,6 +769,10 @@
   p.tighten_mode = tighten;
   p.eps16 = eps16;
   p.flag_host = tighten ? nullptr : rarc_launch_extras().flag_host;
+  RARC_REQUIRE(inc_mode >= 0 && inc_mode <= 2 && (inc_mode == 0 || tighten != 2) && (inc_mode != 1 || tighten == 1),
+               RARC_E_INVALID, "rarc_finalize_q8: inc_mode %d with tighten %d", inc_mode, tighten);
+  p.inc_mode = inc_mode;
+  p.inc = inc_mode ? rarc_fin_inc_carve(ws, cap) : RarcFinInc{nullptr, nullptr, nullptr, nullptr, nullptr};
   const size_t rbytes = (size_t)d_pad * (fmt == 2 ? 4 : (fmt ? 1 : 2));
   const int threads = rbytes <= 1536 ? FIN8_THREADS : (rbytes <= 3072 ? FIN8_THREADS / 2 : FIN8_THREADS / 4);
   const size_t lds = (size_t)(threads / 64) * 8 * (rbytes + 16);
@@ -669,6 +786,42 @@
   hipLaunchKernelGGL(rarc_finalize_q8_kernel, dim3(nq), dim3(threads), lds, s, p);
   RARC_HIP_CHECK(hipGetLastError());
   return RARC_OK;
+}
+int rarc_finalize_q8_launch(const void* corpus, const float* rowscale, int fmt, int d_pad, const float* q32,
+                            const float* eps8, int nq, int k, int64_t id_base, const RarcWs& ws, int cap, int n_wg,
+                            int64_t* out_ids, float* out_scores, uint32_t* status, hipStream_t s, int tighten,
+                            const float* qmeta, const float* hq, const float* eps16) {
+  return rarc_finalize_q8_launch_inc(corpus, rowscale, fmt, d_pad, q32, eps8, nq, k, id_base, ws, cap, n_wg, out_ids,
+                                     out_scores, status, s, tighten, qmeta, hq, eps16, 0);
+}
+
+extern "C" int rarc_debug_fin_inc_layout(int cand_cap, int64_t* out6) {
+  RARC_REQUIRE(out6 && cand_cap >= 4096 && cand_cap % RARC_MAX_WG == 0, RARC_E_INVALID,
+               "rarc_debug_fin_inc_layout: null pointer or cand_cap %d", cand_cap);
+  const size_t base = rarc_fin_inc_offset(cand_cap);
+  out6[0] = (int64_t)(base + RARC_FIN_INC_STATE);
+  out6[1] = (int64_t)(base + RARC_FIN_INC_NK);
+  out6[2] = (int64_t)(base + RARC_FIN_INC_T1);
+  out6[3] = (int64_t)(base + RARC_FIN_INC_CONS);
+  out6[4] = (int64_t)(base + RARC_FIN_INC_TOP);
+  out6[5] = (int64_t)(base + RARC_FIN_INC_BYTES);
+  return RARC_OK;
+}
+extern "C" int rarc_debug_finalize_q8(const uint16_t* d_corpus_f16, int d_pad, const void* d_qblock, int nq, int k, int64_t id_base,
+                                      int n_wg, int tighten, int inc_mode, int64_t* d_out_ids, float* d_out_scores,
+                                      uint32_t* d_status, void* d_workspace, size_t workspace_bytes, int cand_cap, void* stream) {
+  RARC_REQUIRE(d_corpus_f16 && d_qblock && d_out_ids && d_out_scores && d_status && d_workspace, RARC_E_INVALID,
+               "rarc_debug_finalize_q8: null pointer");
+  RARC_REQUIRE(d_pad > 0 && d_pad % RARC_DIM_ALIGN == 0 && nq >= 1 && nq <= RARC_MAX_QUERIES && k >= 1 && k <= RARC_MAX_K &&
+                   n_wg >= 1 && n_wg <= RARC_MAX_WG && (tighten == 0 || tighten == 1),
+               RARC_E_INVALID, "rarc_debug_finalize_q8: bad arguments (d_pad=%d nq=%d k=%d n_wg=%d tighten=%d)", d_pad, nq, k, n_wg,
+               tighten);
+  RARC_REQUIRE(cand_cap >= 4096 && cand_cap % RARC_MAX_WG == 0 && workspace_bytes >= rarc_fin_inc_offset(cand_cap) + RARC_FIN_INC_BYTES,
+               RARC_E_WORKSPACE, "rarc_debug_finalize_q8: workspace of %zu bytes too small for cand_cap=%d", workspace_bytes, cand_cap);
+  const RarcWs ws = rarc_ws_carve(d_workspace);
+  const RarcQb qb = rarc_qb_carve(d_qblock, d_pad);
+  return rarc_finalize_q8_launch_inc(d_corpus_f16, nullptr, 0, d_pad, qb.q32, qb.eps8, nq, k, id_base, ws, cand_cap, n_wg, d_out_ids,
+                                     d_out_scores, d_status, (hipStream_t)stream, tighten, nullptr, nullptr, nullptr, inc_mode);
 }
 
 __device__ __forceinline__ float canon_dot_f8(const float* __restrict__ q, const uint8_t* __restrict__ row, int d,
diff --git a/rag-arc_amd/csrc/rarc_api.hip b/rag-arc_amd/csrc/rarc_api.hip
--- a/rag-arc_amd/csrc/rarc_api.hip
+++ b/rag-arc_amd/csrc/rarc_api.hip
@@ -18,6 +18,10 @@
                             const float* eps8, int nq, int k, int64_t id_base, const RarcWs& ws, int cap, int n_wg,
                             int64_t* out_ids, float* out_scores, uint32_t* status, hipStream_t s, int tighten,
                             const float* qmeta, const float* hq, const float* eps16);
+int rarc_finalize_q8_launch_inc(const void* corpus, const float* rowscale, int fmt, int d_pad, const float* q32,
+                                const float* eps8, int nq, int k, int64_t id_base, const RarcWs& ws, int cap, int n_wg,
+                                int64_t* out_ids, float* out_scores, uint32_t* status, hipStream_t s, int tighten,
+                                const float* qmeta, const float* hq, const float* eps16, int inc_mode);
 
 struct Q8Search {
   const void* rows;
@@ -33,11 +37,18 @@
   float* out_scores;
   uint32_t* status;
   hipStream_t s;
+  int passes = 0;
 };
 static int q8_tighten(void* ctx, int n_wg, int mode) {
-  const Q8Search& a = *(const Q8Search*)ctx;
-  return rarc_finalize_q8_launch(a.rows, a.rowscale, a.fin_fmt, a.d_pad, a.q32, a.eps8, a.nq, a.k, a.id_base, *a.ws, a.cap,
-                                 n_wg, a.out_ids, a.out_scores, a.status, a.s, mode, a.qmeta, a.hq, a.eps16);
+  Q8Search& a = *(Q8Search*)ctx;
+  const int inc_mode = mode == 1 ? (a.passes++ == 0 ? 1 : 2) : 0;
+  return rarc_finalize_q8_launch_inc(a.rows, a.rowscale, a.fin_fmt, a.d_pad, a.q32, a.eps8, a.nq, a.k, a.id_base, *a.ws, a.cap,
+                                     n_wg, a.out_ids, a.out_scores, a.status, a.s, mode, a.qmeta, a.hq, a.eps16, inc_mode);
+}
+static int q8_final(const Q8Search& a, int n_wg, bool hybrid) {
+  return rarc_finalize_q8_launch_inc(a.rows, a.rowscale, a.fin_fmt, a.d_pad, a.q32, a.eps8, a.nq, a.k, a.id_base, *a.ws, a.cap,
+                                     n_wg, a.out_ids, a.out_scores, a.status, a.s, 0, a.qmeta, a.hq, hybrid ? a.eps16 : nullptr,
+                                     a.passes > 0 ? 2 : 0);
 }
 int rarc_repair_launch(const void* corpus, const float* rowscale, int fmt, int64_t n_rows, int d_pad,
                        const float* qv, int k, int64_t id_base, int64_t* ids, float* scores, uint32_t* found,
@@ -133,7 +144,7 @@
 
 extern "C" size_t rarc_search_workspace_bytes(int cand_cap) {
   if (cand_cap < 4096) cand_cap = 4096;
-  return RARC_WS_CAND + (size_t)RARC_MAX_QUERIES * (size_t)cand_cap * 8;
+  return rarc_fin_inc_offset(cand_cap) + RARC_FIN_INC_BYTES;
 }
 
 static int check_ws(void* ws, size_t bytes, int cap, const char* who) {
@@ -173,8 +184,7 @@
     rc = rarc_scan_q8_launch(d_corpus_f16, nullptr, 0, n_rows, d_pad, d_qmeta, qb.q16, qb.q8, qb.qinv, qb.eps16,
                              qb.eps8, nq, kprime, bin_lo, bin_hi, ws, cand_cap, &n_wg, s, nullptr, q8_tighten, &a, qb.hq, qb.floor, &hybrid);
     if (rc) return rc;
-    return rarc_finalize_q8_launch(d_corpus_f16, nullptr, 0, d_pad, qb.q32, qb.eps8, nq, k, id_base, ws, cand_cap,
-                                   n_wg, d_out_ids, d_out_scores, d_status, s, 0, d_qmeta, qb.hq, hybrid ? qb.eps16 : nullptr);
+    return q8_final(a, n_wg, hybrid != 0);
   }
   rc = rarc_scan_f16_launch(d_corpus_f16, n_rows, d_pad, qb.q16, nq, kprime, bin_lo, bin_hi, ws, cand_cap, &n_wg, s,
                             qb.floor, qb.eps16);
@@ -231,8 +241,7 @@
   rc = rarc_scan_q8_launch(d_corpus_f16, nullptr, 2, n_rows, d_pad, d_qmeta, qb.q16, qb.q8, qb.qinv, qb.eps16, qb.eps8,
                            nq, kprime, bin_lo, bin_hi, ws, cand_cap, &n_wg, s, d_shadow8, q8_tighten, &a, qb.hq, qb.floor, nullptr);
   if (rc) return rc;
-  return rarc_finalize_q8_launch(d_corpus_f16, nullptr, 0, d_pad, qb.q32, qb.eps8, nq, k, id_base, ws, cand_cap,
-                                 n_wg, d_out_ids, d_out_scores, d_status, s, 0, d_qmeta, qb.hq, hybrid ? qb.eps16 : nullptr);
+  return q8_final(a, n_wg, hybrid != 0);
 }
 
 extern "C" int rarc_search_f32(const float* d_corpus_f32, const uint16_t* d_image_f16, int64_t n_rows, int d_pad,
@@ -264,8 +273,7 @@
   rc = rarc_scan_q8_launch(d_image_f16, nullptr, 0, n_rows, d_pad, d_qmeta, qb.q16, qb.q8, qb.qinv, qb.eps16, qb.eps8,
                            nq, kprime, bin_lo, bin_hi, ws, cand_cap, &n_wg, s, nullptr, q8_tighten, &a, qb.hq, qb.floor, nullptr);
   if (rc) return rc;
-  return rarc_finalize_q8_launch(d_corpus_f32, nullptr, 2, d_pad, qb.q32, qb.eps8, nq, k, id_base, ws, cand_cap, n_wg,
-                                 d_out_ids, d_out_scores, d_status, s, 0, d_qmeta, qb.hq, hybrid ? qb.eps16 : nullptr);
+  return q8_final(a, n_wg, hybrid != 0);
 }
 
 extern "C" int rarc_repair_f32(const float* d_corpus_f32, int64_t n_rows, int d_pad, const void* d_qblock, int q, int k,
@@ -316,8 +324,7 @@
   rc = rarc_scan_q8_launch(d_corpus_f8, d_row_scale, 1, n_rows, d_pad, d_qmeta, qb.q16, qb.q8, qb.qinv, qb.eps16,
                            qb.eps8, nq, kprime, bin_lo, bin_hi, ws, cand_cap, &n_wg, s, nullptr, q8_tighten, &a, qb.hq, qb.floor, nullptr);
   if (rc) return rc;
-  return rarc_finalize_q8_launch(d_corpus_f8, d_row_scale, 1, d_pad, qb.q32, qb.eps8, nq, k, id_base, ws, cand_cap,
-                                 n_wg, d_out_ids, d_out_scores, d_status, s, 0, d_qmeta, qb.hq, hybrid ? qb.eps16 : nullptr);
+  return q8_final(a, n_wg, hybrid != 0);
 }
 
 extern "C" int rarc_repair_f8(const uint8_t* d_corpus_f8, const float* d_row_scale, int64_t n_rows, int d_pad,
diff --git a/rag-arc_amd/csrc/rarc_common.h b/rag-arc_amd/csrc/rarc_common.h
--- a/rag-arc_amd/csrc/rarc_common.h
+++ b/rag-arc_amd/csrc/rarc_common.h
@@ -65,6 +65,36 @@
   return w;
 }
 
+constexpr int RARC_FIN_INC_PASSES = 3;
+constexpr uint32_t RARC_FIN_INC_POISON = 0xffffffffu;
+constexpr size_t RARC_FIN_INC_STATE = 0;
+constexpr size_t RARC_FIN_INC_NK = 1024;
+constexpr size_t RARC_FIN_INC_T1 = 2048;
+constexpr size_t RARC_FIN_INC_CONS = 8192;
+constexpr size_t RARC_FIN_INC_TOP = RARC_FIN_INC_CONS + (size_t)RARC_MAX_QUERIES * RARC_MAX_WG * 4 * 4;
+constexpr size_t RARC_FIN_INC_BYTES = RARC_FIN_INC_TOP + (size_t)RARC_MAX_QUERIES * RARC_MAX_K * 8;
+static_assert(RARC_FIN_INC_T1 + 4 * RARC_MAX_QUERIES * 4 <= RARC_FIN_INC_CONS, "t1 overlaps cons");
+static inline size_t rarc_fin_inc_offset(int cand_cap) {
+  return RARC_WS_CAND + (size_t)RARC_MAX_QUERIES * (size_t)cand_cap * 8;
+}
+struct RarcFinInc {
+  uint32_t* state;
+  uint32_t* nk;
+  float* t1;
+  uint32_t* cons;
+  uint64_t* top;
+};
+static inline RarcFinInc rarc_fin_inc_carve(const RarcWs& ws, int cand_cap) {
+  char* b = (char*)ws.cand + (size_t)RARC_MAX_QUERIES * (size_t)cand_cap * 8;
+  RarcFinInc f;
+  f.state = (uint32_t*)(b + RARC_FIN_INC_STATE);
+  f.nk = (uint32_t*)(b + RARC_FIN_INC_NK);
+  f.t1 = (float*)(b + RARC_FIN_INC_T1);
+  f.cons = (uint32_t*)(b + RARC_FIN_INC_CONS);
+  f.top = (uint64_t*)(b + RARC_FIN_INC_TOP);
+  return f;
+}
+
 
 struct RarcQb {
   float* q32;
diff --git a/rag-arc_amd/hip/binding.py b/rag-arc_amd/hip/binding.py
--- a/rag-arc_amd/hip/binding.py
+++ b/rag-arc_amd/hip/binding.py
@@ -211,6 +211,9 @@
                                         ctypes.POINTER(ctypes.c_uint32), ctypes.POINTER(ctypes.c_uint32), ctypes.POINTER(ctypes.c_uint32)]),
     "rarc_debug_q8_tail_chunks": (c_int, [ctypes.c_uint32] * 7 + [c_void_p, c_void_p]),
     "rarc_debug_q8_tail_counter_offset": (c_int64, [c_int]),
+    "rarc_debug_fin_inc_layout": (c_int, [c_int, c_void_p]),
+    "rarc_debug_finalize_q8": (c_int, [c_void_p, c_int, c_void_p, c_int, c_int, c_int64, c_int, c_int, c_int, c_void_p, c_void_p,
+                                       c_void_p, c_void_p, c_size_t, c_int, c_void_p]),
     "rarc_search_rows_workspace_bytes": (c_size_t, [c_int, c_int]),
     "rarc_search_rows": (c_int, [c_void_p, c_int, c_int64, c_int, c_void_p, c_int, c_void_p, c_int64, c_int, c_int64, c_void_p, c_int,
                                  c_void_p, c_void_p, c_void_p, c_void_p, c_size_t, c_void_p]),
```

After: 9876 queries/s, median of 2. Within noise of the previous version (-0.1%).
